# guanlongzhao/fac-via-ppg

Measured on AMD Instinct MI355X. Metric: 22.05 kHz audio samples/sec end-to-end PPG→wav; real-time factor at batch=1, higher is better.
Workload: dtype f32

## Files before the change

### fac-via-ppg_amd/common/stft.py

```python
import numpy as np
import torch
from scipy.signal import get_window

from common.audio_processing import _center_pad, squared_window
from facppg import lib as _lib


def dft_bases(filter_length, hop_length, win_length, window):
    n = filter_length
    cutoff = n // 2 + 1
    ang = 2.0 * np.pi * np.outer(np.arange(cutoff), np.arange(n)) / n
    fwd = np.vstack([np.cos(ang), -np.sin(ang)])
    wc = np.full(cutoff, 2.0)
    wc[0] = 1.0
    if n % 2 == 0:
        wc[-1] = 1.0
    scale = n / hop_length
    inv = np.vstack([np.cos(ang) * wc[:, None], -np.sin(ang) * wc[:, None]]) / (n * scale)
    fwd32, inv32 = fwd.astype(np.float32), inv.astype(np.float32)
    if window is not None:
        assert filter_length >= win_length
        win = _center_pad(get_window(window, win_length, fftbins=True), n).astype(np.float32)
        fwd32, inv32 = fwd32 * win, inv32 * win
    return fwd32, inv32


class STFT(torch.nn.Module):

    def __init__(self, filter_length=800, hop_length=200, win_length=800, window='hann', mel_basis=None):
        super(STFT, self).__init__()
        self.filter_length = filter_length
        self.hop_length = hop_length
        self.win_length = win_length
        self.window = window
        self.forward_transform = None
        fwd, inv = dft_bases(filter_length, hop_length, win_length, window)
        self.register_buffer('forward_basis', torch.from_numpy(fwd[:, None, :]).float())
        self.register_buffer('inverse_basis', torch.from_numpy(inv[:, None, :]).float())
        wsq = squared_window(window, win_length, filter_length) if window is not None else \
            np.zeros(filter_length)
        self.register_buffer('_win_sq', torch.from_numpy(wsq.astype(np.float32)), persistent=False)
        self._mel_basis_np = mel_basis

    def _handle(self, dev):
        h = self.__dict__.get("_facppg_handle")
        if h is not None and h[1] == dev:
            return h[0]
        self._release()
        L = _lib.load()
        fwd = self.forward_basis.squeeze(1).to(dev).contiguous()
        inv_t = self.inverse_basis.squeeze(1).t().to(dev).contiguous()
        wsq = self._win_sq.to(dev).contiguous()
        mel = None if self._mel_basis_np is None else torch.as_tensor(self._mel_basis_np, dtype=torch.float32).to(dev).contiguous()
        out = _lib.ctypes.c_void_p()
        with torch.cuda.device(dev):
            _lib.check(L.facppg_stft_create(self.filter_length, self.hop_length, _lib.ptr(fwd), _lib.ptr(inv_t), _lib.ptr(wsq),
                                            _lib.ptr(mel), 0 if mel is None else mel.shape[0], dev.index,
                                            _lib.current_stream(dev), _lib.ctypes.byref(out)))
        self.__dict__["_facppg_handle"] = (out, dev)
        return out

    def _release(self):
        h = self.__dict__.pop("_facppg_handle", None)
        if h is not None:
            _lib.load().facppg_stft_destroy(h[0])
        self.__dict__.pop("_facppg_ws", None)

    def __del__(self):
        try:
            self._release()
        except Exception:
            pass

    def __getstate__(self):
        d = dict(self.__dict__)
        d.pop("_facppg_handle", None)
        d.pop("_facppg_ws", None)
        return d

    def _workspace(self, h, dev, B, N):
        nbytes = _lib.load().facppg_stft_workspace_bytes(h, B, N)
        ws = self.__dict__.get("_facppg_ws")
        if ws is None or ws.numel() < nbytes or ws.device != dev:
            ws = torch.empty(nbytes, dtype=torch.uint8, device=dev)
            self.__dict__["_facppg_ws"] = ws
        return ws

    @staticmethod
    def _lengths(lengths, B, N, dev):
        if lengths is None:
            return None
        if torch.is_tensor(lengths):
            lt = lengths.to(device=dev, dtype=torch.int32).contiguous()
            if lt.numel() != B or int(lt.max()) > N:
                raise _lib.FacppgError("lengths must be B sample counts <= N")
            return lt
        if len(lengths) != B or max(int(n) for n in lengths) > N:
            raise _lib.FacppgError("lengths must be B sample counts <= N")
        return _lib.upload([int(n) for n in lengths], torch.int32, dev)

    def transform(self, input_data, lengths=None):
        _lib.require_cuda(input_data, "STFT.transform: input_data")
        x = input_data.float().contiguous()
        B, N = x.shape
        self.num_samples = N
        dev = x.device
        h = self._handle(dev)
        ws = self._workspace(h, dev, B, N)
        F = N // self.hop_length + 1
        cutoff = self.filter_length // 2 + 1
        mag = torch.zeros(B, cutoff, F, device=dev) if lengths is not None else torch.empty(B, cutoff, F, device=dev)
        phase = torch.zeros_like(mag) if lengths is not None else torch.empty_like(mag)
        with torch.cuda.device(dev):
            _lib.check(_lib.load().facppg_stft_transform(h, _lib.ptr(x), _lib.ptr(self._lengths(lengths, B, N, dev)), B, N,
                                                         _lib.ptr(mag), _lib.ptr(phase), _lib.ptr(ws), ws.numel(),
                                                         _lib.current_stream(dev)))
        return mag, phase

    def inverse(self, magnitude, phase):
        _lib.require_cuda(magnitude, "STFT.inverse: magnitude")
        mag = magnitude.float().contiguous()
        ph = phase.to(mag.device).float().contiguous()
        B, _, F = mag.shape
        dev = mag.device
        h = self._handle(dev)
        ws = self._workspace(h, dev, B, (F - 1) * self.hop_length)
        out = torch.empty(B, 1, self.hop_length * (F - 1), device=dev)
        with torch.cuda.device(dev):
            _lib.check(_lib.load().facppg_stft_inverse(h, _lib.ptr(mag), _lib.ptr(ph), B, F, _lib.ptr(out), _lib.ptr(ws),
                                                       ws.numel(), _lib.current_stream(dev)))
        return out

    def forward(self, input_data):
        self.magnitude, self.phase = self.transform(input_data)
        return self.inverse(self.magnitude, self.phase)

    def mel(self, y, lengths=None):
        _lib.require_cuda(y, "mel_spectrogram: y")
# ... 29 lines not shown
```

### fac-via-ppg_amd/csrc/facppg_dsp.hip

```cpp
#include <cstring>
#include <new>

#include "facppg_gemm.h"

using namespace facppg;

struct facppg_stft {
  int fl, hop, cutoff, n_mel, device;
  char* arena;
  float4 *fwd, *inv_t, *melb;
  float* win_sq;
};

namespace {

__global__ void k_frames(const float* __restrict__ x, float* __restrict__ X, const int* __restrict__ n_valid, int N, int fl,
                         int hop, int F, int* __restrict__ f_valid) {
  const int b = blockIdx.z, k = blockIdx.y;
  const int Nb = n_valid ? n_valid[b] : N;
  const int Fb = Nb / hop + 1;
  if (f_valid && blockIdx.x == 0 && k == 0 && threadIdx.x == 0) f_valid[b] = Fb;
  const int f = blockIdx.x * blockDim.x + threadIdx.x;
  if (f >= Fb) return;
  int j = f * hop + k - fl / 2;
// ... 12 lines not shown
  if (phase) phase[o] = atan2f(im, re);
}

__global__ void k_recombine(const float* __restrict__ mag, const float* __restrict__ phase, float* __restrict__ R,
                            const int* __restrict__ f_valid, int cutoff, int F) {
  const int b = blockIdx.z, c = blockIdx.y, f = blockIdx.x * blockDim.x + threadIdx.x;
  if (f >= (f_valid ? f_valid[b] : F)) return;
  const size_t o = ((size_t)b * cutoff + c) * F + f;
  float sn, cs;
  sincosf(phase[o], &sn, &cs);
  R[((size_t)b * 2 * cutoff + c) * F + f] = mag[o] * cs;
  R[((size_t)b * 2 * cutoff + cutoff + c) * F + f] = mag[o] * sn;
}

__global__ void k_spectral_subtract(float* __restrict__ S, const float* __restrict__ bias, float strength,
                                    const int* __restrict__ f_valid, int cutoff, int F) {
  const int b = blockIdx.z, c = blockIdx.y, f = blockIdx.x * blockDim.x + threadIdx.x;
  if (f >= (f_valid ? f_valid[b] : F)) return;
  const size_t ore = ((size_t)b * 2 * cutoff + c) * F + f, oim = ore + (size_t)cutoff * F;
  const float re = S[ore], im = S[oim];
  const float mag = sqrtf(re * re + im * im);
  const float m2 = fmaxf(mag - bias[c] * strength, 0.0f);
  if (mag > 0.0f) {
    const float sc = m2 / mag;
    S[ore] = re * sc; S[oim] = im * sc;
  } else {
    S[ore] = m2; S[oim] = 0.0f;
  }
}

__global__ void k_overlap_add(const float* __restrict__ Zt, const float* __restrict__ win_sq, float* __restrict__ y,
                              const int* __restrict__ f_valid, int fl, int hop, int F, long y_bs) {
  const int b = blockIdx.y;
  const int Fb = f_valid ? f_valid[b] : F;
  const int i = blockIdx.x * blockDim.x + threadIdx.x;
  if (i >= hop * (Fb - 1)) return;
  const int n = i + fl / 2;
  int f_hi = n / hop;
  if (f_hi > Fb - 1) f_hi = Fb - 1;
  int f_lo = (n - fl + hop) / hop;
  if (f_lo < 0) f_lo = 0;
  float acc = 0.0f, ws = 0.0f;
  for (int f = f_lo; f <= f_hi; ++f) {
    const int k = n - f * hop;
    acc += Zt[((size_t)b * F + f) * fl + k];
    ws += win_sq[k];
  }
  if (ws > 1.17549435e-38f) acc /= ws;
  y[(size_t)b * y_bs + i] = acc * ((float)fl / (float)hop);
}

struct Ws {
  int F;
  size_t X, S, Z, fv, sk, sk_bytes, total;
};
Ws ws_layout(const facppg_stft* h, int B, int N) {
  Ws w;
  w.F = N / h->hop + 1;
  size_t off = 0;
  auto take = [&](size_t bytes) { size_t o = off; off += (bytes + 255) / 256 * 256; return o; };
  w.X = take((size_t)B * (h->fl + 2) * w.F * 4);
  w.S = take((size_t)B * (h->fl + 2) * w.F * 4);
  w.Z = take((size_t)B * w.F * h->fl * 4);
  w.fv = take((size_t)B * 4);
  w.sk_bytes = (size_t)4 * B * (h->fl + 2) * w.F * 4;
  w.sk = take(w.sk_bytes);
  w.total = off;
  return w;
}

int run_forward(facppg_stft* h, const float* audio, const int* n_valid, int B, int N, char* ws, const Ws& w, hipStream_t s) {
  float* X = (float*)(ws + w.X);
  float* S = (float*)(ws + w.S);
  int* fv = (int*)(ws + w.fv);
  dim3 g((w.F + 255) / 256, h->fl, B);
  k_frames<<<g, 256, 0, s>>>(audio, X, n_valid, N, h->fl, h->hop, w.F, fv);
  GemmArgs a;
  a.A = h->fwd; a.M = 2 * h->cutoff; a.Cin = h->fl; a.X = X; a.x_bs = (long)h->fl * w.F; a.ldx = w.F; a.N = w.F;
  a.n_valid = fv; a.C = S; a.c_bs = (long)2 * h->cutoff * w.F; a.ldc = w.F; a.B = B;
  a.splitk_ws = (float*)(ws + w.sk); a.splitk_ws_bytes = w.sk_bytes;
  return gemm_launch(a, s);
}

int run_inverse(facppg_stft* h, const float* R, int B, char* ws, const Ws& w, const int* fv, float* out, long out_bs, hipStream_t s) {
  float* Z = (float*)(ws + w.Z);
  GemmArgs a;
  a.A = h->inv_t; a.M = h->fl; a.Cin = 2 * h->cutoff; a.X = R; a.x_bs = (long)2 * h->cutoff * w.F; a.ldx = w.F; a.N = w.F;
  a.n_valid = fv; a.C = Z; a.c_bs = (long)w.F * h->fl; a.ldc = h->fl; a.c_transposed = 1; a.B = B;
  a.splitk_ws = (float*)(ws + w.sk); a.splitk_ws_bytes = w.sk_bytes;
  if (int rc = gemm_launch(a, s)) return rc;
  const int n_out = h->hop * (w.F - 1);
  if (n_out > 0) {
    dim3 g((n_out + 255) / 256, B);
    k_overlap_add<<<g, 256, 0, s>>>(Z, h->win_sq, out, fv, h->fl, h->hop, w.F, out_bs);
  }
  FACPPG_HIP_CHECK(hipGetLastError());
  return FACPPG_OK;
}

int check_common(const facppg_stft* h, const void* a, const void* b, const void* ws, int B, int N, size_t ws_bytes, Ws* w) {
  FACPPG_REQUIRE(h && a && b && ws, FACPPG_EINVAL, "NULL argument");
  FACPPG_REQUIRE(B > 0 && N > h->fl / 2, FACPPG_EINVAL, "need B > 0 and N > filter_length/2 (reflect padding), got B=%d N=%d", B, N);
  *w = ws_layout(h, B, N);
  FACPPG_REQUIRE(ws_bytes >= w->total, FACPPG_EWORKSPACE, "workspace has %zu bytes, need %zu", ws_bytes, w->total);
  return FACPPG_OK;
}

}

extern "C" int facppg_stft_create(int filter_length, int hop_length, const float* fwd_basis_dev, const float* inv_basis_t_dev,
                                  const float* win_sq_dev, const float* mel_basis_dev, int n_mel, int device, void* stream_,
                                  facppg_stft** out) {
  FACPPG_REQUIRE(fwd_basis_dev && inv_basis_t_dev && win_sq_dev && out, FACPPG_EINVAL, "NULL argument");
  FACPPG_REQUIRE(filter_length >= 16 && filter_length % 2 == 0 && hop_length > 0 && hop_length <= filter_length, FACPPG_EINVAL,
                 "bad filter_length/hop_length %d/%d", filter_length, hop_length);
  FACPPG_REQUIRE(!mel_basis_dev || n_mel > 0, FACPPG_EINVAL, "n_mel must be positive with a mel basis");
  hipStream_t s = (hipStream_t)stream_;
  FACPPG_HIP_CHECK(hipSetDevice(device));
  facppg_stft* h = new (std::nothrow) facppg_stft();
  FACPPG_REQUIRE(h, FACPPG_EINVAL, "out of host memory");
  h->fl = filter_length; h->hop = hop_length; h->cutoff = filter_length / 2 + 1; h->n_mel = mel_basis_dev ? n_mel : 0;
  h->device = device;
  const int R = 2 * h->cutoff;
  size_t off = 0;
  auto take = [&](size_t bytes) { size_t o = off; off += (bytes + 255) / 256 * 256; return o; };
  const size_t o_fwd = take(packed_a_float4s(R, h->fl) * 16), o_inv = take(packed_a_float4s(h->fl, R) * 16);
  const size_t o_mel = take(h->n_mel ? packed_a_float4s(h->n_mel, h->cutoff) * 16 : 16), o_win = take((size_t)h->fl * 4);
  if (hipMalloc((void**)&h->arena, off) != hipSuccess) {
    set_error("hipMalloc(%zu) failed", off);
    delete h;
    return FACPPG_EHIP;
  }
  h->fwd = (float4*)(h->arena + o_fwd); h->inv_t = (float4*)(h->arena + o_inv); h->melb = (float4*)(h->arena + o_mel);
  h->win_sq = (float*)(h->arena + o_win);
  int rc = pack_a(fwd_basis_dev, R, h->fl, 1, h->fwd, s);
  if (!rc) rc = pack_a(inv_basis_t_dev, h->fl, R, 1, h->inv_t, s);
  if (!rc && h->n_mel) rc = pack_a(mel_basis_dev, h->n_mel, h->cutoff, 1, h->melb, s);
  if (!rc && hipMemcpyAsync(h->win_sq, win_sq_dev, (size_t)h->fl * 4, hipMemcpyDeviceToDevice, s) != hipSuccess) rc = FACPPG_EHIP;
  if (!rc && hipStreamSynchronize(s) != hipSuccess) rc = FACPPG_EHIP;
  if (rc) {
    (void)hipFree(h->arena);
    delete h;
    return rc;
  }
  *out = h;
  return FACPPG_OK;
}

extern "C" void facppg_stft_destroy(facppg_stft* h) {
  if (!h) return;
  (void)hipFree(h->arena);
  delete h;
}

extern "C" size_t facppg_stft_workspace_bytes(const facppg_stft* h, int B, int N) {
  if (!h || B <= 0 || N <= 0) return 0;
  return ws_layout(h, B, N).total;
}

extern "C" int facppg_stft_transform(facppg_stft* h, const float* audio_dev, const int32_t* n_valid_dev, int B, int N,
                                     float* mag_dev, float* phase_dev, void* ws_, size_t ws_bytes, void* stream_) {
  Ws w;
  if (int rc = check_common(h, audio_dev, mag_dev, ws_, B, N, ws_bytes, &w)) return rc;
  hipStream_t s = (hipStream_t)stream_;
  char* ws = (char*)ws_;
  if (int rc = run_forward(h, audio_dev, n_valid_dev, B, N, ws, w, s)) return rc;
  dim3 g((w.F + 255) / 256, h->cutoff, B);
  k_magphase<<<g, 256, 0, s>>>((float*)(ws + w.S), mag_dev, phase_dev, (int*)(ws + w.fv), h->cutoff, w.F);
  FACPPG_HIP_CHECK(hipGetLastError());
  return FACPPG_OK;
}

extern "C" int facppg_stft_inverse(facppg_stft* h, const float* mag_dev, const float* phase_dev, int B, int F, float* out_dev,
                                   void* ws_, size_t ws_bytes, void* stream_) {
  FACPPG_REQUIRE(h && mag_dev && phase_dev && out_dev && ws_, FACPPG_EINVAL, "NULL argument");
  FACPPG_REQUIRE(B > 0 && F > 1, FACPPG_EINVAL, "need B > 0 and at least 2 frames");
  const int N = (F - 1) * h->hop;
  const Ws w = ws_layout(h, B, N);
  FACPPG_REQUIRE(ws_bytes >= w.total, FACPPG_EWORKSPACE, "workspace has %zu bytes, need %zu", ws_bytes, w.total);
  hipStream_t s = (hipStream_t)stream_;
  char* ws = (char*)ws_;
  float* R = (float*)(ws + w.X);
  dim3 g((F + 255) / 256, h->cutoff, B);
  k_recombine<<<g, 256, 0, s>>>(mag_dev, phase_dev, R, nullptr, h->cutoff, F);
  return run_inverse(h, R, B, ws, w, nullptr, out_dev, (long)h->hop * (F - 1), s);
}

extern "C" int facppg_stft_mel(facppg_stft* h, const float* audio_dev, const int32_t* n_valid_dev, int B, int N, float* mel_dev,
                               void* ws_, size_t ws_bytes, void* stream_) {
  Ws w;
  if (int rc = check_common(h, audio_dev, mel_dev, ws_, B, N, ws_bytes, &w)) return rc;
  FACPPG_REQUIRE(h->n_mel > 0, FACPPG_EINVAL, "handle was created without a mel basis");
  hipStream_t s = (hipStream_t)stream_;
  char* ws = (char*)ws_;
  if (int rc = run_forward(h, audio_dev, n_valid_dev, B, N, ws, w, s)) return rc;
  float* mag = (float*)(ws + w.X);
  int* fv = (int*)(ws + w.fv);
  dim3 g((w.F + 255) / 256, h->cutoff, B);
  k_magphase<<<g, 256, 0, s>>>((float*)(ws + w.S), mag, nullptr, fv, h->cutoff, w.F);
  GemmArgs a;
  a.A = h->melb; a.M = h->n_mel; a.Cin = h->cutoff; a.X = mag; a.x_bs = (long)h->cutoff * w.F; a.ldx = w.F; a.N = w.F;
  a.n_valid = fv; a.act = ACT_LOG_CLAMP; a.C = mel_dev; a.c_bs = (long)h->n_mel * w.F; a.ldc = w.F; a.B = B;
  return gemm_launch(a, s);
}

extern "C" int facppg_denoise(facppg_stft* h, const float* audio_dev, const int32_t* n_valid_dev, const float* bias_spec_dev,
                              float strength, int B, int N, float* out_dev, void* ws_, size_t ws_bytes, void* stream_) {
  Ws w;
  if (int rc = check_common(h, audio_dev, out_dev, ws_, B, N, ws_bytes, &w)) return rc;
  FACPPG_REQUIRE(bias_spec_dev, FACPPG_EINVAL, "bias_spec is NULL");
  hipStream_t s = (hipStream_t)stream_;
  char* ws = (char*)ws_;
  if (int rc = run_forward(h, audio_dev, n_valid_dev, B, N, ws, w, s)) return rc;
  float* S = (float*)(ws + w.S);
  int* fv = (int*)(ws + w.fv);
  dim3 g((w.F + 255) / 256, h->cutoff, B);
  k_spectral_subtract<<<g, 256, 0, s>>>(S, bias_spec_dev, strength, fv, h->cutoff, w.F);
  return run_inverse(h, S, B, ws, w, fv, out_dev, (long)h->hop * (w.F - 1), s);
}
```

### fac-via-ppg_amd/csrc/facppg_gemm.h

```cpp
#pragma once
#include "facppg_common.h"

namespace facppg {

enum GemmAct { ACT_NONE = 0, ACT_RELU = 1, ACT_TANH = 2, ACT_LOG_CLAMP = 3  };

inline int gemm_kpad(int K) { return round_up(K, 64); }
inline size_t packed_a_float4s(int M, int K) { return (size_t)(round_up(M, 32) / 32) * (gemm_kpad(K) / 8 + 1) * 64 + 3 * 64; }

int pack_a(const float* src, int M, int Cin, int taps, float4* dst, hipStream_t s);
int pack_a_strided(const float* src, int M, int Cin, int taps, long sm, long sc, long st, long off, float4* dst, hipStream_t s);

struct GemmArgs {
  const float4* A = nullptr;
  int M = 0;
  int Cin = 0, taps = 1, dil = 1, pad = 0;
  const float* X = nullptr;
  long x_bs = 0;
  int ldx = 0;
  int N = 0;
  int col0 = 0;
  int src_hi = 0;
  const int* skip = nullptr;
  const int* n_valid = nullptr;
  int n_valid_mul = 1;
  int n_valid_add = 0;
  const float* bias = nullptr;
  const float* scale = nullptr;
  const float* shift = nullptr;
  int act = ACT_NONE;
  const uint8_t* mask = nullptr;
  long mask_bs = 0;
  int ldmask = 0;
  const float* res = nullptr;
  long res_bs = 0;
  int ldres = 0;
  float* C = nullptr;
  long c_bs = 0;
  int ldc = 0;
  int c_transposed = 0;
  const float* gate_ts = nullptr;
  long gate_bs = 0;
  int ldgate = 0;
  int B = 1;
  float* splitk_ws = nullptr;
  size_t splitk_ws_bytes = 0;
};

int gemm_launch(const GemmArgs& a, hipStream_t s);

}
```

### fac-via-ppg_amd/csrc/facppg_gemm.hip

```cpp
#include "facppg_gemm.h"

namespace facppg {
namespace {

constexpr int TN = 64, KCH = 64;

__global__ void k_pack_a(const float* __restrict__ src, float4* __restrict__ dst, int M, int Cin, int taps, int KG, long sm,
                         long sc, long st, long off) {
  const int idx = blockIdx.x * blockDim.x + threadIdx.x;
  const int MB = (M + 31) / 32;
  if (idx >= MB * (KG + 1) * 64) return;
  const int lane = idx & 63, g = (idx >> 6) % (KG + 1), mb = (idx >> 6) / (KG + 1);
  const int m = mb * 32 + (lane & 31), K = Cin * taps;
  float v[4];
  for (int s = 0; s < 4; ++s) {
    const int k = 8 * g + 4 * (lane >> 5) + s;
    const int tap = k / Cin, c = k - tap * Cin;
    v[s] = (m < M && k < K && g < KG) ? src[off + m * sm + c * sc + tap * st] : 0.0f;
  }
  dst[idx] = make_float4(v[0], v[1], v[2], v[3]);
}

struct KArgs {
  GemmArgs g;
  int KG;
  int sk;
};

__device__ __forceinline__ void gemm_epilogue(const GemmArgs& p, int b, int m, int n, float v) {
  if (p.bias) v += p.bias[m];
  if (p.scale) v = v * p.scale[m] + p.shift[m];
  if (p.act == ACT_RELU) v = fmaxf(v, 0.0f);
  else if (p.act == ACT_TANH) v = tanhf(v);
  else if (p.act == ACT_LOG_CLAMP) v = logf(fmaxf(v, 1e-5f));
  if (p.mask) v = v * (float)p.mask[(size_t)b * p.mask_bs + (size_t)m * p.ldmask + n] * 2.0f;
  if (p.res) v += p.res[(size_t)b * p.res_bs + (size_t)m * p.ldres + n];
  if (p.gate_ts) {
    const float T = p.gate_ts[(size_t)b * p.gate_bs + (size_t)m * p.ldgate + n];
    const float S = p.gate_ts[(size_t)b * p.gate_bs + (size_t)(p.M + m) * p.ldgate + n];
    p.C[(size_t)b * p.c_bs + (size_t)m * p.ldc + n] = v * S * (1.0f - T * T);
    p.C[(size_t)b * p.c_bs + (size_t)(p.M + m) * p.ldc + n] = v * T * S * (1.0f - S);
  } else if (p.c_transposed) p.C[(size_t)b * p.c_bs + (size_t)n * p.ldc + m] = v;
  else p.C[(size_t)b * p.c_bs + (size_t)m * p.ldc + n] = v;
}

__global__ __launch_bounds__(256) void k_gemm(KArgs ka) {
  const GemmArgs& p = ka.g;
  __shared__ __attribute__((aligned(16))) float smem[2 * KCH * TN];
  const int tid = threadIdx.x, lane = tid & 63, w = tid >> 6, li = lane & 31, kh = lane >> 5;
  const int b = blockIdx.z / ka.sk, ks = blockIdx.z % ka.sk, n0 = p.col0 + blockIdx.x * TN;
  const int Nb = p.n_valid ? min(p.N, p.n_valid[b] * p.n_valid_mul + p.n_valid_add) : p.N;
  if (n0 >= Nb) return;
  if (p.skip && *p.skip) return;
// ... 4 lines not shown
  const int K = p.Cin * p.taps;
  const int nch_all = ka.KG / 8;
  const int c_lo = ks * nch_all / ka.sk, c_hi = (ks + 1) * nch_all / ka.sk;

  f32x16 acc[2];
#pragma unroll
  for (int r = 0; r < 16; ++r) { acc[0][r] = 0.0f; acc[1][r] = 0.0f; }

  const float* xb = p.X + (size_t)b * p.x_bs;
  const int col = n0 + lane;
  float stg[16];
  auto stage_load = [&](int c) {
#pragma unroll
    for (int j = 0; j < 16; ++j) {
      const int kk = c * KCH + w * 16 + j;
      const int tap = kk / p.Cin, ch = kk - tap * p.Cin;
      const int sc = col + (tap - p.pad) * p.dil;
      stg[j] = (kk < K && sc >= 0 && sc < Ns) ? xb[(size_t)ch * p.ldx + sc] : 0.0f;
    }
  };
  auto stage_write = [&](int buf) {
    float* dst = smem + buf * (KCH * TN) + (w * 16) * TN + lane;
#pragma unroll
    for (int j = 0; j < 16; ++j) dst[j * TN] = stg[j];
  };

  const float4* ap = p.A + (size_t)(active ? mb : 0) * (ka.KG + 1) * 64 + lane;
  constexpr int RING = 4;
  float4 ar[RING];
  stage_load(c_lo);
#pragma unroll
  for (int i = 0; i < RING - 1; ++i) ar[i] = ap[(size_t)(c_lo * 8 + i) * 64];
  stage_write(c_lo & 1);
  __syncthreads();
  for (int c = c_lo; c < c_hi; ++c) {
    stage_load(c + 1 < c_hi ? c + 1 : c);
    const float* lb = smem + (c & 1) * (KCH * TN) + (4 * kh) * TN + li;
    const int G = c * 8;
#pragma unroll
    for (int g = 0; g < 8; ++g) {
      ar[(g + RING - 1) % RING] = ap[(size_t)(G + g + RING - 1) * 64];
      __builtin_amdgcn_sched_barrier(0);
      const float4 a0 = ar[g % RING];
#pragma unroll
      for (int s = 0; s < 4; ++s) {
        const float av = s == 0 ? a0.x : s == 1 ? a0.y : s == 2 ? a0.z : a0.w;
        acc[0] = mfma32x32x2(av, lb[(8 * g + s) * TN], acc[0]);
        acc[1] = mfma32x32x2(av, lb[(8 * g + s) * TN + 32], acc[1]);
      }
    }
    stage_write((c + 1) & 1);
    __syncthreads();
  }
  if (!active) return;
#pragma unroll
  for (int cb = 0; cb < 2; ++cb) {
    const int n = n0 + cb * 32 + li;
    if (n >= Nb) continue;
#pragma unroll
    for (int r = 0; r < 16; ++r) {
      const int m = mb * 32 + 8 * (r >> 2) + (r & 3) + 4 * kh;
      if (m >= p.M) continue;
      if (ka.sk > 1) p.splitk_ws[(((size_t)ks * p.B + b) * p.M + m) * p.N + n] = acc[cb][r];
      else gemm_epilogue(p, b, m, n, acc[cb][r]);
    }
  }
}

__global__ void k_gemm_reduce(KArgs ka) {
  const GemmArgs& p = ka.g;
  const int n = p.col0 + blockIdx.x * blockDim.x + threadIdx.x, m = blockIdx.y, b = blockIdx.z;
  const int Nb = p.n_valid ? min(p.N, p.n_valid[b] * p.n_valid_mul + p.n_valid_add) : p.N;
  if (n >= Nb) return;
  if (p.skip && *p.skip) return;
  float v = 0.0f;
  for (int ks = 0; ks < ka.sk; ++ks) v += p.splitk_ws[(((size_t)ks * p.B + b) * p.M + m) * p.N + n];
  gemm_epilogue(p, b, m, n, v);
}

}

int pack_a_strided(const float* src, int M, int Cin, int taps, long sm, long sc, long st, long off, float4* dst, hipStream_t s) {
  const int KG = gemm_kpad(Cin * taps) / 8;
  const int total = (round_up(M, 32) / 32) * (KG + 1) * 64;
  k_pack_a<<<(total + 255) / 256, 256, 0, s>>>(src, dst, M, Cin, taps, KG, sm, sc, st, off);
  FACPPG_HIP_CHECK(hipGetLastError());
  return FACPPG_OK;
}

int pack_a(const float* src, int M, int Cin, int taps, float4* dst, hipStream_t s) {
  return pack_a_strided(src, M, Cin, taps, (long)Cin * taps, taps, 1, 0, dst, s);
}

int gemm_launch(const GemmArgs& a, hipStream_t s) {
  FACPPG_REQUIRE(a.A && a.X && a.C && a.M > 0 && a.N > 0 && a.Cin > 0 && a.taps > 0 && a.B > 0 && a.col0 >= 0 && a.col0 < a.N, FACPPG_EINVAL,
                 "gemm_launch: bad arguments");
  KArgs ka;
  ka.g = a;
  ka.KG = gemm_kpad(a.Cin * a.taps) / 8;
  ka.sk = 1;
  dim3 grid((a.N - a.col0 + TN - 1) / TN, (round_up(a.M, 32) / 32 + 3) / 4, a.B);
  const int nch = ka.KG / 8;
  if (a.splitk_ws && nch >= 8) {
    const int sk = nch / 4 < 16 ? nch / 4 : 16;
    const size_t need = (size_t)sk * a.B * a.M * a.N * sizeof(float);
    FACPPG_REQUIRE(need <= a.splitk_ws_bytes, FACPPG_EWORKSPACE, "gemm_launch: split-K buffer has %zu bytes, needs %zu",
                   a.splitk_ws_bytes, need);
    ka.sk = sk;
  }
  grid.z = a.B * ka.sk;
  k_gemm<<<grid, 256, 0, s>>>(ka);
  if (ka.sk > 1) k_gemm_reduce<<<dim3((a.N - a.col0 + 255) / 256, a.M, a.B), 256, 0, s>>>(ka);
  FACPPG_HIP_CHECK(hipGetLastError());
  return FACPPG_OK;
}

}
```

### fac-via-ppg_amd/csrc/facppg_taco.hip

```cpp

#include <algorithm>
#include <cstdlib>
#include <cstring>
#include <mutex>
#include <new>

#include "facppg_gemm.h"

using namespace facppg;

struct facppg_taco {
  facppg_taco_config c;
  int device;
  int coop_limit;
  int wall_khz;
  char* arena;
  float4 *pre0, *pre1, *conv[8], *wih;
  float *conv_b[8], *conv_scale[8], *conv_shift[8];
  float *whh_t[2], *lstm_b;
  float4* mem_w;
  float *dp0_t, *dp1_t, *att_t, *att_b, *dec_t, *dec_b, *q_t, *proj_t, *proj_b;
  float *loc_conv, *loc_dense, *v;
  float *att_coop[5], *dec_coop[5];
  int coop_U[5], coop_nwg[5];
// ... 1332 lines not shown
      forced_att_slice<NTC>(att_slice, xrow, p.E + p.A, p.U, p.A, unit0, L.in_att + p.P, L.part, c_state, out, (unsigned)(tf + 1), tid);
    }
    __syncthreads();
  };
  att_step(0);
  long long tk = clock64();
#define PROF(slot)                                                        \
  if (p.prof && leader && b == 0 && tid == 0) {                           \
    const long long now = clock64();                                      \
    p.prof[slot] += now - tk;                                             \
    tk = now;                                                             \
  }
  for (int t = 0; t < T; ++t) {
    unsigned long long* xt = xb + (size_t)t * fw;
    int lo, hi;
    attn_window_range(p.window, t, len, &lo, &hi);
    attn_features<NTC>(p, L, lo, min(64, hi - lo + 1), tid);
    __syncthreads();
    attn_energy_pre<NTC>(p, L, pm, lo, min(64, hi - lo + 1), tid, stash);
    PROF(0)
    coop_gather<NTC>(xt, (unsigned)(t + 1), p.A, ah, L.in_dec, tid);
    PROF(1)
    dec_attention<NTC, 0, true>(p, L, mem, pm, len, t, b, tid, leader, true, NoQueryRegs().w, stash);
    if (leader)
      for (int i = tid; i < p.E; i += NTC) xpub(xt + p.A + i, L.in_proj[p.D + i], (unsigned)(t + 1));
    PROF(2)
    if (t + 1 < T) att_step(t + 1);
    PROF(3)
  }
#undef PROF
}

__global__ void k_forced_inputs(const float* __restrict__ tgt, float* __restrict__ x, size_t rows, int T) {
  const size_t i = (size_t)blockIdx.x * blockDim.x + threadIdx.x;
  if (i >= rows * T) return;
  const int t = (int)(i % T);
  x[i] = t ? tgt[i - 1] : 0.0f;
}
__global__ void k_forced_outputs(const float* __restrict__ mg, float* __restrict__ mel, float* __restrict__ gate, int B, int NF, int T) {
  const size_t i = (size_t)blockIdx.x * blockDim.x + threadIdx.x;
  if (i >= (size_t)B * (NF + 1) * T) return;
  const int t = (int)(i % T), r = (int)(i / T % (NF + 1)), b = (int)(i / T / (NF + 1));
  if (r < NF) mel[((size_t)b * NF + r) * T + t] = mg[i];
  else gate[(size_t)b * T + t] = mg[i];
}
__global__ void k_random_mask_forced_utt(uint8_t* __restrict__ out, const uint64_t* __restrict__ seeds, int B, int P, int T) {
  const size_t i = (size_t)blockIdx.x * blockDim.x + threadIdx.x;
  if (i >= (size_t)2 * B * P * T) return;
  const int t = (int)(i % T), u = (int)(i / T % P), b = (int)(i / T / P % B), j = (int)(i / T / P / B);
  out[i] = mask_bit(seeds[b] ^ 0xD1B54A32D192ED03ull, ((uint64_t)t << 32) | (uint32_t)(j * P + u));
}

struct TWs {
  size_t a0, a1, xproj, mem_cm, mask, xchg, splitk, splitk_bytes, total;
};
TWs tws_layout(const facppg_taco_config& c, int B, int Tin) {
  TWs w;
  size_t off = 0;
  auto take = [&](size_t bytes) { size_t o = off; off += (bytes + 255) / 256 * 256; return o; };
  const size_t E = c.encoder_embedding_dim > c.symbols_embedding_dim ? c.encoder_embedding_dim : c.symbols_embedding_dim;
  w.a0 = take((size_t)B * E * Tin * 4);
  w.a1 = take((size_t)B * E * Tin * 4);
  w.xproj = take((size_t)B * Tin * 4 * c.encoder_embedding_dim * 4);
  w.mem_cm = take((size_t)B * c.encoder_embedding_dim * Tin * 4);
  w.mask = take((size_t)2 * B * c.symbols_embedding_dim * Tin);
  w.xchg = take((size_t)B * 2 * 2 * (c.encoder_embedding_dim / 2) * 8);
  const size_t mx = c.encoder_embedding_dim > c.symbols_embedding_dim ? c.encoder_embedding_dim : c.symbols_embedding_dim;
  w.splitk_bytes = (size_t)16 * B * mx * Tin * 4;
  w.splitk = take(w.splitk_bytes);
  w.total = off;
  return w;
}

}

static int taco_check(const facppg_taco_config* c) {
  FACPPG_REQUIRE(c, FACPPG_EINVAL, "config is NULL");
  FACPPG_REQUIRE(c->n_symbols > 0 && c->symbols_embedding_dim > 0 && c->encoder_embedding_dim > 0 && c->encoder_embedding_dim % 2 == 0,
                 FACPPG_EINVAL, "bad encoder dims");
  FACPPG_REQUIRE(c->symbols_embedding_dim == c->encoder_embedding_dim, FACPPG_EUNSUPPORTED,
                 "symbols_embedding_dim must equal encoder_embedding_dim (prenet feeds the conv bank)");
  FACPPG_REQUIRE(c->encoder_n_convolutions >= 0 && c->encoder_n_convolutions <= 8 && c->postnet_n_convolutions >= 2 &&
                     c->postnet_n_convolutions <= 8 && c->encoder_kernel_size % 2 == 1 && c->postnet_kernel_size % 2 == 1,
                 FACPPG_EUNSUPPORTED, "conv stack sizes out of range");
  FACPPG_REQUIRE(c->attention_rnn_dim == c->decoder_rnn_dim && c->attention_rnn_dim % 4 == 0 && 4 * c->attention_rnn_dim <= 4096,
                 FACPPG_EUNSUPPORTED, "attention_rnn_dim must equal decoder_rnn_dim, be a multiple of 4 and <= 1024");
  FACPPG_REQUIRE(c->attention_location_n_filters >= 1 && c->attention_location_n_filters <= 32 && c->attention_dim >= 1 &&
                     c->attention_dim <= 256,
                 FACPPG_EUNSUPPORTED, "attention_location_n_filters must be <= 32 and attention_dim <= 256 (one MFMA pass each)");
  FACPPG_REQUIRE(c->encoder_embedding_dim <= 768 && c->prenet_dim <= NTC && c->attention_dim <= NTC && c->n_acoustic_feat_dims < NTC &&
                     (2 * c->encoder_embedding_dim) % 4 == 0,
                 FACPPG_EUNSUPPORTED, "decoder dims exceed the 512-thread cooperative workgroup");
  FACPPG_REQUIRE(c->attention_location_kernel_size % 2 == 1 && c->attention_location_n_filters > 0, FACPPG_EUNSUPPORTED,
                 "attention_location_kernel_size must be odd");
  return FACPPG_OK;
}

static size_t taco_count(const facppg_taco_config* c) {
  const size_t S = c->symbols_embedding_dim, E = c->encoder_embedding_dim, H = E / 2, K = c->encoder_kernel_size;
  const size_t P = c->prenet_dim, A = c->attention_rnn_dim, D = c->decoder_rnn_dim, AD = c->attention_dim, NF = c->n_acoustic_feat_dims;
  size_t n = S * c->n_symbols + S * S;
  n += (size_t)c->encoder_n_convolutions * (E * E * K + 5 * E);
  n += 2 * (4 * H * E + 4 * H * H + 8 * H);
  n += P * NF + P * P;
  n += 4 * A * (P + E) + 4 * A * A + 8 * A;
  n += AD * A + AD * E + AD + (size_t)c->attention_location_n_filters * 2 * c->attention_location_kernel_size +
       AD * c->attention_location_n_filters;
  n += 4 * D * (A + E) + 4 * D * D + 8 * D;
  n += NF * (D + E) + NF + (D + E) + 1;
  const size_t PE = c->postnet_embedding_dim, PK = c->postnet_kernel_size;
  for (int j = 0; j < c->postnet_n_convolutions; ++j) {
    const size_t ci = j == 0 ? NF : PE, co = j == c->postnet_n_convolutions - 1 ? NF : PE;
    n += co * ci * PK + 5 * co;
  }
  return n;
}

extern "C" size_t facppg_taco_weight_count(const facppg_taco_config* c) {
  if (taco_check(c) != FACPPG_OK) return 0;
// ... 182 lines not shown
    const int n = (D + E + 1) * Pp;
    k_fold_prenet<<<(n + 255) / 256, 256, 0, s>>>(h->proj_t, h->proj_b, h->dp0_t, h->w1p_t, h->b1p, D + E, NF, NFp, Pp);
    if (!rc) rc = pack_a_strided(h->proj_t, NF + 1, D + E, 1, 1, NFp, 0, 0, h->tf_proj, s);
  }
  for (int j = 0; j < c.postnet_n_convolutions; ++j) {
    const int ci = j == 0 ? NF : PE, co = j == c.postnet_n_convolutions - 1 ? NF : PE;
    h->post[j] = F4(o.post[j]); h->post_b[j] = F(o.post_b[j]); h->post_scale[j] = F(o.post_sc[j]); h->post_shift[j] = F(o.post_sh[j]);
    if (!rc) rc = pack_a(src, co, ci, PK, h->post[j], s); src += (size_t)co * ci * PK;
    cpy(h->post_b[j], src, co); src += co;
    bn(src, co, h->post_scale[j], h->post_shift[j]);
  }
  hipok(hipGetLastError());
  hipok(hipStreamSynchronize(s));
  if (!rc && (size_t)(src - wsrc) != n_floats) { set_error("internal: consumed %zu of %zu weights", (size_t)(src - wsrc), n_floats); rc = FACPPG_EINVAL; }
  if (rc) return rc;
  guard.h = nullptr;
  *out = h;
  return FACPPG_OK;
}

extern "C" void facppg_taco_destroy(facppg_taco* h) {
  if (!h) return;
  (void)hipFree(h->arena);
  delete h;
}

extern "C" size_t facppg_taco_workspace_bytes(const facppg_taco* h, int B, int Tin) {
  if (!h || B <= 0 || Tin <= 0) return 0;
  return tws_layout(h->c, B, Tin).total;
}

static int taco_encode_impl(const facppg_taco* h, const float* ppg_dev, const int32_t* lengths_dev, const uint8_t* masks_dev,
                            uint64_t seed, int B, int Tin, float* memory_dev, float* pm_dev, void* ws_, size_t ws_bytes,
                            void* stream_, bool padded_batch) {
  FACPPG_REQUIRE(h && ppg_dev && memory_dev && pm_dev && ws_, FACPPG_EINVAL, "NULL argument");
  FACPPG_REQUIRE(B > 0 && Tin > 0 && B <= 65535, FACPPG_EINVAL, "bad B/Tin");
  const facppg_taco_config& c = h->c;
  const TWs w = tws_layout(c, B, Tin);
  FACPPG_REQUIRE(ws_bytes >= w.total, FACPPG_EWORKSPACE, "workspace has %zu bytes, need %zu", ws_bytes, w.total);
  hipStream_t s = (hipStream_t)stream_;
  char* ws = (char*)ws_;
  float* a0 = (float*)(ws + w.a0);
  float* a1 = (float*)(ws + w.a1);
  float* xproj = (float*)(ws + w.xproj);
  float* mem_cm = (float*)(ws + w.mem_cm);
  const int S = c.symbols_embedding_dim, E = c.encoder_embedding_dim, H = E / 2;
  const uint8_t* masks = masks_dev;
  if (!masks) {
    uint8_t* m = (uint8_t*)(ws + w.mask);
    const size_t n = (size_t)2 * B * S * Tin;
    k_random_mask<<<(unsigned)((n + 255) / 256), 256, 0, s>>>(m, n, seed);
    masks = m;
  }
  GemmArgs g;
  g.B = B; g.N = Tin; g.n_valid = padded_batch ? nullptr : lengths_dev;
  g.splitk_ws = (float*)(ws + w.splitk); g.splitk_ws_bytes = w.splitk_bytes;
  g.A = h->pre0; g.M = S; g.Cin = c.n_symbols; g.X = ppg_dev; g.x_bs = (long)c.n_symbols * Tin; g.ldx = Tin; g.act = ACT_RELU;
  g.mask = masks; g.mask_bs = (long)S * Tin; g.ldmask = Tin; g.C = a0; g.c_bs = (long)S * Tin; g.ldc = Tin;
  if (int rc = gemm_launch(g, s)) return rc;
  g.A = h->pre1; g.Cin = S; g.X = a0; g.x_bs = (long)S * Tin; g.mask = masks + (size_t)B * S * Tin; g.C = a1;
  if (int rc = gemm_launch(g, s)) return rc;
  float* cur = a1;
  float* nxt = a0;
  g.mask = nullptr;
  for (int j = 0; j < c.encoder_n_convolutions; ++j) {
    g.A = h->conv[j]; g.M = E; g.Cin = E; g.taps = c.encoder_kernel_size; g.pad = (c.encoder_kernel_size - 1) / 2; g.X = cur;
    g.x_bs = (long)E * Tin; g.bias = h->conv_b[j]; g.scale = h->conv_scale[j]; g.shift = h->conv_shift[j]; g.C = nxt;
    g.c_bs = (long)E * Tin;
    if (int rc = gemm_launch(g, s)) return rc;
    float* t = cur; cur = nxt; nxt = t;
  }
  GemmArgs p;
  p.splitk_ws = g.splitk_ws; p.splitk_ws_bytes = g.splitk_ws_bytes;
  p.B = B; p.N = Tin; p.n_valid = lengths_dev; p.A = h->wih; p.M = 8 * H; p.Cin = E; p.X = cur; p.x_bs = (long)E * Tin; p.ldx = Tin;
  p.bias = h->lstm_b; p.C = xproj; p.c_bs = (long)Tin * 8 * H; p.ldc = 8 * H; p.c_transposed = 1;
  if (int rc = gemm_launch(p, s)) return rc;
  const char* bilstm_mode = getenv("FACPPG_BILSTM_MODE");
  const bool no_coop = bilstm_mode && !strcmp(bilstm_mode, "single");
  const bool fit32 = (long)B * 2 * ((H + 31) / 32) <= h->coop_limit && (H + 3) / 4 <= 96 && !(bilstm_mode && !strcmp(bilstm_mode, "wide"));
  const bool fit64 = (long)B * 2 * ((H + 63) / 64) <= h->coop_limit && (H + 1) / 2 <= 152;
  if (!no_coop && (fit32 || fit64)) {
    unsigned long long* xchg = (unsigned long long*)(ws + w.xchg);
    FACPPG_HIP_CHECK(hipMemsetAsync(xchg, 0, (size_t)B * 2 * 2 * H * 8, s));
    const float *w0 = h->whh_t[0], *w1 = h->whh_t[1];
    const float* xp = xproj;
    int Tin_ = Tin, H_ = H;
    void* args[] = {(void*)&xp, (void*)&w0, (void*)&w1, (void*)&lengths_dev, (void*)&Tin_, (void*)&H_, (void*)&xchg,
                    (void*)&memory_dev, (void*)&mem_cm};
    if (fit32) FACPPG_HIP_CHECK(launch_coop((const void*)k_bilstm_coop<32, 96>, dim3((H + 31) / 32, 2, B), dim3(NTC), args, 0, s));
    else FACPPG_HIP_CHECK(launch_coop((const void*)k_bilstm_coop<64, 152>, dim3((H + 63) / 64, 2, B), dim3(NTC), args, 0, s));
  } else {
    const int KS = NT / H < H ? NT / H : H;
    const size_t smem = (size_t)(2 * H + (KS > 0 ? KS : 1) * 4 * H) * 4;
    k_bilstm<<<dim3(2, B), NT, smem, s>>>(xproj, h->whh_t[0], h->whh_t[1], lengths_dev, Tin, H, memory_dev, mem_cm);
  }
  GemmArgs m;
  m.splitk_ws = g.splitk_ws; m.splitk_ws_bytes = g.splitk_ws_bytes;
  m.B = B; m.N = Tin; m.n_valid = lengths_dev; m.A = h->mem_w; m.M = c.attention_dim; m.Cin = E; m.X = mem_cm; m.x_bs = (long)E * Tin;
  m.ldx = Tin; m.C = pm_dev; m.c_bs = (long)Tin * c.attention_dim; m.ldc = Tin;
  if (int rc = gemm_launch(m, s)) return rc;
  FACPPG_HIP_CHECK(hipGetLastError());
  return FACPPG_OK;
}

extern "C" int facppg_taco_encode(const facppg_taco* h, const float* ppg_dev, const int32_t* lengths_dev, const uint8_t* masks_dev,
                                  uint64_t seed, int B, int Tin, float* memory_dev, float* pm_dev, void* ws_, size_t ws_bytes,
                                  void* stream_) {
  return taco_encode_impl(h, ppg_dev, lengths_dev, masks_dev, seed, B, Tin, memory_dev, pm_dev, ws_, ws_bytes, stream_, false);
}

extern "C" int facppg_taco_encode_padded(const facppg_taco* h, const float* ppg_dev, const int32_t* lengths_dev,
                                         const int32_t* lengths_host, const uint8_t* masks_dev, uint64_t seed, int B, int Tin,
                                         float* memory_dev, float* pm_dev, void* ws_, size_t ws_bytes, void* stream_) {
  FACPPG_REQUIRE(h && memory_dev && pm_dev, FACPPG_EINVAL, "NULL argument");
  FACPPG_REQUIRE(B > 0 && Tin > 0, FACPPG_EINVAL, "bad B/Tin");
  FACPPG_REQUIRE((lengths_dev == nullptr) == (lengths_host == nullptr), FACPPG_EINVAL, "lengths_dev and lengths_host go together");
  for (int b = 0; lengths_host && b < B; ++b) {
    FACPPG_REQUIRE(lengths_host[b] >= 1 && lengths_host[b] <= Tin, FACPPG_EINVAL, "lengths[%d] = %d is outside [1, Tin = %d]", b,
                   lengths_host[b], Tin);
    FACPPG_REQUIRE(b == 0 || lengths_host[b] <= lengths_host[b - 1], FACPPG_EINVAL,
                   "lengths must be sorted in descending order (pack_padded_sequence, model.py:226): lengths[%d] = %d > lengths[%d] = %d",
                   b, lengths_host[b], b - 1, lengths_host[b - 1]);
  }
  hipStream_t s = (hipStream_t)stream_;
  FACPPG_HIP_CHECK(hipMemsetAsync(memory_dev, 0, (size_t)B * Tin * h->c.encoder_embedding_dim * 4, s));
  FACPPG_HIP_CHECK(hipMemsetAsync(pm_dev, 0, (size_t)B * Tin * h->c.attention_dim * 4, s));
  return taco_encode_impl(h, ppg_dev, lengths_dev, masks_dev, seed, B, Tin, memory_dev, pm_dev, ws_, ws_bytes, stream_, true);
}

namespace {
struct DecWs { size_t mask, xchg, prof, xsplit, total; };
DecWs dec_ws(const facppg_taco_config& c, int B, int max_steps) {
  DecWs w;
  size_t off = 0;
  auto take = [&](size_t bytes) { size_t o = off; off += (bytes + 255) / 256 * 256; return o; };
  w.mask = take((size_t)max_steps * 2 * B * c.prenet_dim);
  w.xchg = take((size_t)B * 2 * c.attention_rnn_dim * 8);
  w.prof = take(32 * 8);
  w.xsplit = take((size_t)B * (c.n_acoustic_feat_dims + 1 + 2 * c.prenet_dim + c.attention_rnn_dim + c.encoder_embedding_dim + c.decoder_rnn_dim + 8) * 8);
  w.total = off;
  return w;
}
}

extern "C" int facppg_taco_draw_dropout(const facppg_taco* h, const uint64_t* seeds_dev, int B, int Tin, int max_steps,
                                        uint8_t* enc_masks_dev, uint8_t* dec_masks_dev, void* stream_) {
  FACPPG_REQUIRE(h && seeds_dev, FACPPG_EINVAL, "NULL argument");
  FACPPG_REQUIRE(B > 0 && Tin > 0 && max_steps > 0, FACPPG_EINVAL, "bad B/Tin/max_steps");
  hipStream_t s = (hipStream_t)stream_;
  const int S = h->c.symbols_embedding_dim, P = h->c.prenet_dim;
  if (enc_masks_dev) {
    const size_t n = (size_t)2 * B * S * Tin;
// ... 98 lines not shown
                   : NU == 3 ? (const void*)k_decoder_split<3> : (const void*)k_decoder_split<4>;
    FACPPG_HIP_CHECK(hipFuncSetAttribute(fn, hipFuncAttributeMaxDynamicSharedMemorySize, (int)ssm));
    void* args[] = {(void*)&a};
    const int groups = (B + NU - 1) / NU;
    a.nwk = h->split_nwk;
    unsigned long long* words = opts ? (unsigned long long*)opts->frame_words_dev : nullptr;
    a.melx = (B == 1 && words && opts->frame_words_frames >= max_steps) ? words : nullptr;
    a.dbg_flags = getenv("FACPPG_DECODER_NO_ROWS") ? 1 : 0;
    FACPPG_HIP_CHECK(launch_coop(fn, dim3(h->split_nwk + NU, groups), dim3(NTC), args, ssm, s));
    launch_mode = 2; launch_wgs = (h->split_nwk + NU) * groups;
    if (a.prof) {
      long long pr[32];
      FACPPG_HIP_CHECK(hipMemcpyAsync(pr, a.prof, sizeof(pr), hipMemcpyDeviceToHost, s));
      FACPPG_HIP_CHECK(hipStreamSynchronize(s));
      fprintf(stderr, "[facppg split decoder prof (main), shader cycles] location features %lld energy_pre %lld entering row %lld query weights requested %lld wait_gate %lld wait_ah %lld attention %lld | att: query %lld energy %lld softmax %lld update %lld context %lld\n",
              pr[6], pr[7], pr[14], pr[2], pr[0], pr[3], pr[5], pr[8], pr[10], pr[11], pr[12], pr[13]);
      fprintf(stderr, "[facppg split decoder prof (worker 0), shader cycles] proj+prenet1 %lld | gather gate,X1 %lld | prenet2 %lld | gather X2 %lld | "
              "att LSTM %lld | gather AH %lld | gather CTX %lld | dec LSTM + gather DH %lld | barrier %lld\n",
              pr[16], pr[17], pr[18], pr[19], pr[20], pr[21], pr[22], pr[23], pr[24]);
    }
  } else
  if (coop) {
    FACPPG_HIP_CHECK(hipMemsetAsync(ws + w.xchg, 0, w.total - w.xchg, s));
    const void* fn = (const void*)k_decoder_coop;
    FACPPG_HIP_CHECK(hipFuncSetAttribute(fn, hipFuncAttributeMaxDynamicSharedMemorySize, (int)smem));
    for (int b0 = 0; b0 < B; b0 += chunk) {
      const int nb = B - b0 < chunk ? B - b0 : chunk;
      int cv = variant;
      if (!force_u)
        for (int v = 0; v < variant; ++v)
          if ((long)nb * h->coop_nwg[v] <= wg_limit) { cv = v; break; }
      a.b0 = b0; a.att_coop = h->att_coop[cv]; a.dec_coop = h->dec_coop[cv]; a.U = h->coop_U[cv];
      void* args[] = {(void*)&a};
      FACPPG_HIP_CHECK(launch_coop(fn, dim3(h->coop_nwg[cv], nb), dim3(NTC), args, smem, s));
      launch_mode = 1; launch_wgs = h->coop_nwg[cv] * nb;
    }
    if (a.prof) {
      long long pr[16];
      FACPPG_HIP_CHECK(hipMemcpyAsync(pr, a.prof, sizeof(pr), hipMemcpyDeviceToHost, s));
      FACPPG_HIP_CHECK(hipStreamSynchronize(s));
      fprintf(stderr, "[facppg decoder prof, shader cycles] project %lld prenet %lld att_slice %lld sync1 %lld gather %lld attention %lld dec_slice %lld sync2 %lld | att: query %lld feat %lld energy %lld softmax %lld update %lld context %lld\n",
              pr[0], pr[1], pr[2], pr[3], pr[4], pr[5], pr[6], pr[7], pr[8], pr[9], pr[10], pr[11], pr[12], pr[13]);
    }
  } else {
    FACPPG_HIP_CHECK(hipFuncSetAttribute((const void*)k_decoder, hipFuncAttributeMaxDynamicSharedMemorySize, (int)smem));
    k_decoder<<<B, NT, smem, s>>>(a);
  }
  FACPPG_HIP_CHECK(hipGetLastError());
  if (opts) { opts->mode = launch_mode; opts->workgroups = launch_wgs; opts->streamed = a.melx != nullptr; }
  return FACPPG_OK;
}

namespace {
struct ForcedWs { size_t x0, p1, p2, xa, hc, mg, mask, xchg, prof, splitk, splitk_bytes, total; };
ForcedWs forced_ws(const facppg_taco_config& c, int B, int T) {
  ForcedWs w;
  size_t off = 0;
  auto take = [&](size_t bytes) { size_t o = off; off += (bytes + 255) / 256 * 256; return o; };
  const size_t BT = (size_t)B * T;
  w.x0 = take(BT * c.n_acoustic_feat_dims * 4);
  w.p1 = take(BT * c.prenet_dim * 4);
  w.p2 = take(BT * c.prenet_dim * 4);
  w.xa = take(BT * 4 * c.attention_rnn_dim * 4);
  w.hc = take(BT * (c.decoder_rnn_dim + c.encoder_embedding_dim) * 4);
  w.mg = take(BT * (c.n_acoustic_feat_dims + 1) * 4);
  w.mask = take(2 * BT * c.prenet_dim);
  w.xchg = take(BT * (c.attention_rnn_dim + c.encoder_embedding_dim + c.decoder_rnn_dim) * 8);
  w.prof = take(32 * 8);
  w.splitk_bytes = 16 * BT * (c.n_acoustic_feat_dims + 1) * 4;
  w.splitk = take(w.splitk_bytes);
  w.total = off;
  return w;
}
}

extern "C" size_t facppg_taco_decode_forced_workspace_bytes(const facppg_taco* h, int B, int T_out) {
  if (!h || B <= 0 || T_out <= 0) return 0;
  return forced_ws(h->c, B, T_out).total;
}

extern "C" int facppg_taco_draw_dropout_forced(const facppg_taco* h, const uint64_t* seeds_dev, int B, int T_out,
                                               uint8_t* dec_masks_dev, void* stream_) {
  FACPPG_REQUIRE(h && seeds_dev && dec_masks_dev, FACPPG_EINVAL, "NULL argument");
  FACPPG_REQUIRE(B > 0 && T_out > 0, FACPPG_EINVAL, "bad B/T_out");
  const size_t n = (size_t)2 * B * h->c.prenet_dim * T_out;
  k_random_mask_forced_utt<<<(unsigned)((n + 255) / 256), 256, 0, (hipStream_t)stream_>>>(dec_masks_dev, seeds_dev, B, h->c.prenet_dim, T_out);
  FACPPG_HIP_CHECK(hipGetLastError());
  return FACPPG_OK;
}

extern "C" int facppg_taco_decode_forced(const facppg_taco* h, const float* memory_dev, const float* pm_dev, const int32_t* lengths_dev,
                                         const float* targets_dev, const uint8_t* masks_dev, uint64_t seed, int B, int Tin, int T_out,
                                         float* mel_dev, float* gate_dev, float* align_dev, void* ws_, size_t ws_bytes,
                                         facppg_taco_decode_opts* opts, void* stream_) {
  FACPPG_REQUIRE(h && memory_dev && pm_dev && targets_dev && mel_dev && gate_dev && ws_, FACPPG_EINVAL, "NULL argument");
  FACPPG_REQUIRE(B > 0 && Tin > 0 && T_out > 0 && B <= 65535, FACPPG_EINVAL, "bad B/Tin/T_out");
  FACPPG_REQUIRE(!opts || opts->max_workgroups >= 0, FACPPG_EINVAL, "negative max_workgroups");
  FACPPG_REQUIRE(Tin <= 8192, FACPPG_EUNSUPPORTED, "Tin > 8192 does not fit the decoder's LDS state");
  const facppg_taco_config& c = h->c;
  hipStream_t s = (hipStream_t)stream_;
  const ForcedWs w = forced_ws(c, B, T_out);
  FACPPG_REQUIRE(ws_bytes >= w.total, FACPPG_EWORKSPACE, "teacher-forced decode workspace has %zu bytes, need %zu", ws_bytes, w.total);
  char* ws = (char*)ws_;
  const int P = c.prenet_dim, E = c.encoder_embedding_dim, A = c.attention_rnn_dim, D = c.decoder_rnn_dim, NF = c.n_acoustic_feat_dims;
  const int T = T_out, G = 4 * A, KP = D + E;
  float *x0 = (float*)(ws + w.x0), *p1 = (float*)(ws + w.p1), *p2 = (float*)(ws + w.p2), *xa = (float*)(ws + w.xa);
  float *hc = (float*)(ws + w.hc), *mg = (float*)(ws + w.mg);
  const uint8_t* masks = masks_dev;
  const size_t nmask = (size_t)2 * B * P * T;
  if (!masks) {
    k_random_mask<<<(unsigned)((nmask + 255) / 256), 256, 0, s>>>((uint8_t*)(ws + w.mask), nmask, seed ^ 0xD1B54A32D192ED03ull);
    masks = (const uint8_t*)(ws + w.mask);
  }
  {
    const size_t n = (size_t)B * NF * T;
    k_forced_inputs<<<(unsigned)((n + 255) / 256), 256, 0, s>>>(targets_dev, x0, (size_t)B * NF, T);
  }
  GemmArgs g;
  g.B = B; g.N = T; g.A = h->tf_dp0; g.M = P; g.Cin = NF; g.X = x0; g.x_bs = (long)NF * T; g.ldx = T; g.act = ACT_RELU;
  g.mask = masks; g.mask_bs = (long)P * T; g.ldmask = T; g.C = p1; g.c_bs = (long)P * T; g.ldc = T;
  if (int rc = gemm_launch(g, s)) return rc;
  g.A = h->tf_dp1; g.Cin = P; g.X = p1; g.x_bs = (long)P * T; g.mask = masks + (size_t)B * P * T; g.C = p2;
  if (int rc = gemm_launch(g, s)) return rc;
  GemmArgs x;
  x.B = B; x.N = T; x.A = h->tf_attx; x.M = G; x.Cin = P; x.X = p2; x.x_bs = (long)P * T; x.ldx = T; x.bias = h->att_b;
  x.C = xa; x.c_bs = (long)T * G; x.ldc = G; x.c_transposed = 1;
  if (int rc = gemm_launch(x, s)) return rc;
  DecArgs a = {};
  a.dec_b = h->dec_b; a.q_t = h->q_t; a.loc_conv = h->loc_conv; a.loc_dense = h->loc_dense; a.v = h->v;
  a.memory = memory_dev; a.pm = pm_dev; a.lengths = lengths_dev; a.align = align_dev;
  a.B = B; a.Tin = Tin; a.E = E; a.P = P; a.A = A; a.D = D; a.AD = c.attention_dim; a.NF = NF;
  a.NFIL = c.attention_location_n_filters; a.KSZ = c.attention_location_kernel_size; a.window = c.attention_window_size;
  a.max_steps = T; a.gate_thr = c.gate_threshold;
  const size_t smem = (round_up((int)dec_lds_floats(a.P, a.E, a.A, a.D, a.NF, a.AD, a.NFIL, a.KSZ, Tin), 4) + (size_t)8 * NTC * 4) * 4;
  FACPPG_REQUIRE(smem <= 160 * 1024 - 1024, FACPPG_EUNSUPPORTED, "decoder state (%zu bytes) exceeds LDS", smem);
  const int max_wgs = opts ? opts->max_workgroups : 0;
  const int wg_limit = max_wgs > 0 && max_wgs < h->coop_limit ? max_wgs : h->coop_limit;
  FACPPG_REQUIRE(wg_limit >= 2 * h->coop_nwg[4], FACPPG_EUNSUPPORTED, "the teacher-forced decoder needs %d co-resident workgroups, %d allowed",
                 2 * h->coop_nwg[4], wg_limit);
  const char* force_u = getenv("FACPPG_DECODER_COOP_U");
  auto pick = [&](int nb, int* vc, int* vd) {
    for (int c2 = 0; c2 < 5; ++c2) {
      if (force_u && atoi(force_u) != h->coop_U[c2]) continue;
      for (int d2 = c2; d2 <= (force_u ? c2 : std::min(c2 + 1, 4)); ++d2)
        if ((long)nb * (h->coop_nwg[c2] + h->coop_nwg[d2]) <= wg_limit) { *vc = c2; *vd = d2; return true; }
    }
    return false;
  };
  const bool regw = !force_u && !getenv("FACPPG_FORCED_NO_REGW") && (long)B * (h->split_nwk + h->coop_nwg[0]) <= wg_limit &&
                    E + A <= SKP * SKR_FA && A <= h->split_nwk * SU;
  int vc = 4, vd = 4, chunk = B;
  if (regw) { vc = vd = 0; }
  else if (!pick(B, &vc, &vd)) {
    FACPPG_REQUIRE(!force_u, FACPPG_EUNSUPPORTED, "FACPPG_DECODER_COOP_U=%s does not fit B = %d", force_u, B);
    vc = vd = 4; chunk = wg_limit / (2 * h->coop_nwg[4]);
  }
  unsigned long long* xw = (unsigned long long*)(ws + w.xchg);
  FACPPG_HIP_CHECK(hipMemsetAsync(xw, 0, w.prof + 32 * 8 - w.xchg, s));
  a.prof = getenv("FACPPG_DECODER_PROF") ? (long long*)(ws + w.prof) : nullptr;
  const void* fn = regw ? (const void*)k_decoder_forced<true> : (const void*)k_decoder_forced<false>;
  FACPPG_HIP_CHECK(hipFuncSetAttribute(fn, hipFuncAttributeMaxDynamicSharedMemorySize, (int)smem));
  a.att_w4 = h->att_w4;
  int launch_wgs = 0;
  for (int b0 = 0; b0 < B; b0 += chunk) {
    const int nb = B - b0 < chunk ? B - b0 : chunk;
    int cv = vc, dv = vd;
    if (nb < chunk && !force_u && !regw) pick(nb, &cv, &dv);
    a.b0 = b0; a.att_coop = h->att_coop[cv]; a.dec_coop = h->dec_coop[dv]; a.U = h->coop_U[cv];
    const float* xa_c = xa;
    int NA = regw ? h->split_nwk : h->coop_nwg[cv], UD = h->coop_U[dv];
    void* args[] = {(void*)&a, (void*)&xa_c, (void*)&hc, (void*)&xw, (void*)&NA, (void*)&UD};
    FACPPG_HIP_CHECK(launch_coop(fn, dim3(NA + h->coop_nwg[dv], nb), dim3(NTC), args, smem, s));
    launch_wgs = (NA + h->coop_nwg[dv]) * nb;
  }
  if (a.prof) {
    long long pr[16];
    FACPPG_HIP_CHECK(hipMemcpyAsync(pr, a.prof, sizeof(pr), hipMemcpyDeviceToHost, s));
    FACPPG_HIP_CHECK(hipStreamSynchronize(s));
    fprintf(stderr, "[facppg teacher-forced decoder prof (chain workgroup 0), shader cycles] features+energy_pre %lld gather_ah %lld attention %lld att_slice %lld | att: query %lld feat %lld energy %lld softmax %lld update %lld context %lld\n",
            pr[0], pr[1], pr[2], pr[3], pr[8], pr[9], pr[10], pr[11], pr[12], pr[13]);
  }
  GemmArgs q;
  q.splitk_ws = (float*)(ws + w.splitk); q.splitk_ws_bytes = w.splitk_bytes;
  q.B = B; q.N = T; q.A = h->tf_proj; q.M = NF + 1; q.Cin = KP; q.X = hc; q.x_bs = (long)KP * T; q.ldx = T; q.bias = h->proj_b;
  q.C = mg; q.c_bs = (long)(NF + 1) * T; q.ldc = T;
  if (int rc = gemm_launch(q, s)) return rc;
  {
    const size_t n = (size_t)B * (NF + 1) * T;
    k_forced_outputs<<<(unsigned)((n + 255) / 256), 256, 0, s>>>(mg, mel_dev, gate_dev, B, NF, T);
  }
  FACPPG_HIP_CHECK(hipGetLastError());
  if (opts) { opts->mode = 1; opts->workgroups = launch_wgs; opts->streamed = 0; }
  return FACPPG_OK;
}

__global__ void k_forced_state(const unsigned long long* __restrict__ xw, float* __restrict__ ah, float* __restrict__ dh, size_t BT,
                               int A, int E, int D) {
  const size_t i = (size_t)blockIdx.x * blockDim.x + threadIdx.x;
  if (i >= BT * (A + D)) return;
  const size_t r = i / (A + D);
  const int k = (int)(i % (A + D));
  const float v = __uint_as_float((unsigned)xw[r * (A + E + D) + (k < A ? k : k + E)]);
  if (k < A) ah[r * A + k] = v;
  else dh[r * D + k - A] = v;
}

extern "C" int facppg_taco_decode_forced_state(const facppg_taco* h, const void* ws_, size_t ws_bytes, int B, int T_out, float* ah_dev,
                                               float* dh_dev, uint8_t* masks_dev, void* stream_) {
  FACPPG_REQUIRE(h && ws_ && ah_dev && dh_dev, FACPPG_EINVAL, "NULL argument");
  FACPPG_REQUIRE(B > 0 && T_out > 0, FACPPG_EINVAL, "bad B/T_out");
  const facppg_taco_config& c = h->c;
  const ForcedWs w = forced_ws(c, B, T_out);
  FACPPG_REQUIRE(ws_bytes >= w.total, FACPPG_EWORKSPACE, "teacher-forced decode workspace has %zu bytes, need %zu", ws_bytes, w.total);
  hipStream_t s = (hipStream_t)stream_;
  const char* ws = (const char*)ws_;
  const size_t BT = (size_t)B * T_out, n = BT * (c.attention_rnn_dim + c.decoder_rnn_dim);
  k_forced_state<<<(unsigned)((n + 255) / 256), 256, 0, s>>>((const unsigned long long*)(ws + w.xchg), ah_dev, dh_dev, BT,
                                                             c.attention_rnn_dim, c.encoder_embedding_dim, c.decoder_rnn_dim);
  FACPPG_HIP_CHECK(hipGetLastError());
  if (masks_dev) FACPPG_HIP_CHECK(hipMemcpyAsync(masks_dev, ws + w.mask, 2 * BT * c.prenet_dim, hipMemcpyDeviceToDevice, s));
  return FACPPG_OK;
}

extern "C" int facppg_taco_encode_state(const facppg_taco* h, const void* ws_, size_t ws_bytes, int B, int Tin, uint8_t* masks_dev,
                                        void* stream_) {
  FACPPG_REQUIRE(h && ws_ && masks_dev, FACPPG_EINVAL, "NULL argument");
  FACPPG_REQUIRE(B > 0 && Tin > 0, FACPPG_EINVAL, "bad B/Tin");
  const TWs w = tws_layout(h->c, B, Tin);
  FACPPG_REQUIRE(ws_bytes >= w.total, FACPPG_EWORKSPACE, "encoder workspace has %zu bytes, need %zu", ws_bytes, w.total);
  FACPPG_HIP_CHECK(hipMemcpyAsync(masks_dev, (const char*)ws_ + w.mask, (size_t)2 * B * h->c.symbols_embedding_dim * Tin,
                                  hipMemcpyDeviceToDevice, (hipStream_t)stream_));
  return FACPPG_OK;
}

extern "C" int facppg_taco_postnet(const facppg_taco* h, const float* mel_dev, const int32_t* out_lengths_dev, int B, int T, int ld,
                                   float* mel_post_dev, void* ws_, size_t ws_bytes, void* stream_) {
  FACPPG_REQUIRE(h && mel_dev && mel_post_dev && ws_, FACPPG_EINVAL, "NULL argument");
  FACPPG_REQUIRE(B > 0 && T > 0 && ld >= T, FACPPG_EINVAL, "bad B/T/ld");
  const facppg_taco_config& c = h->c;
  const int PE = c.postnet_embedding_dim, NF = c.n_acoustic_feat_dims, n = c.postnet_n_convolutions;
  const size_t need = facppg_taco_postnet_workspace_bytes(h, B, T);
  FACPPG_REQUIRE(ws_bytes >= need, FACPPG_EWORKSPACE, "workspace has %zu bytes, need %zu", ws_bytes, need);
  hipStream_t s = (hipStream_t)stream_;
  float* buf[2] = {(float*)ws_, (float*)ws_ + (size_t)B * PE * T};
  float* skws = (float*)ws_ + (size_t)2 * B * PE * T;
  const size_t skws_bytes = need - (size_t)2 * B * PE * T * 4;
  const float* cur = mel_dev;
  long cur_bs = (long)NF * ld;
  int cur_ld = ld;
  for (int j = 0; j < n; ++j) {
    const int ci = j == 0 ? NF : PE, co = j == n - 1 ? NF : PE;
    GemmArgs g;
    g.splitk_ws = skws; g.splitk_ws_bytes = skws_bytes;
    g.B = B; g.N = T; g.n_valid = out_lengths_dev; g.A = h->post[j]; g.M = co; g.Cin = ci; g.taps = c.postnet_kernel_size;
    g.pad = (c.postnet_kernel_size - 1) / 2; g.X = cur; g.x_bs = cur_bs; g.ldx = cur_ld; g.bias = h->post_b[j];
    g.scale = h->post_scale[j]; g.shift = h->post_shift[j];
    if (j < n - 1) {
      g.act = ACT_TANH; g.C = buf[j & 1]; g.c_bs = (long)PE * T; g.ldc = T;
    } else {
      g.res = mel_dev; g.res_bs = (long)NF * ld; g.ldres = ld; g.C = mel_post_dev; g.c_bs = (long)NF * ld; g.ldc = ld;
    }
    if (int rc = gemm_launch(g, s)) return rc;
    cur = g.C; cur_bs = g.c_bs; cur_ld = g.ldc;
  }
  return FACPPG_OK;
}

extern "C" size_t facppg_taco_postnet_workspace_bytes(const facppg_taco* h, int B, int T) {
  if (!h || B <= 0 || T <= 0) return 0;
  const size_t sk = (size_t)16 * B * h->c.postnet_embedding_dim * T * 4;
  return (size_t)2 * B * h->c.postnet_embedding_dim * T * 4 + sk;
}

namespace {
__global__ __launch_bounds__(256) void k_collect_frames(const unsigned long long* __restrict__ melx, const int* __restrict__ out_len,
                                                        int NF, int fa, int fb, float* __restrict__ dst, int ld, int* void_flag,
                                                        const int* prev_flag, unsigned long long limit) {
  if (prev_flag && __hip_atomic_load(prev_flag, __ATOMIC_RELAXED, __HIP_MEMORY_SCOPE_AGENT)) {
    if (void_flag) __hip_atomic_store(void_flag, 1, __ATOMIC_RELAXED, __HIP_MEMORY_SCOPE_AGENT);
    return;
  }
  const int n = (fb - fa) * NF;
  for (int i = blockIdx.x * blockDim.x + threadIdx.x; i < n; i += gridDim.x * blockDim.x) {
    const int f = fa + i / NF, row = i - (f - fa) * NF;
    const unsigned long long* w = melx + (size_t)f * NF + row;
    unsigned long long v, t0 = 0;
    unsigned spins = 0;
    for (;;) {
      v = __hip_atomic_load(w, __ATOMIC_RELAXED, __HIP_MEMORY_SCOPE_AGENT);
      if ((unsigned)(v >> 32) == (unsigned)(f + 1)) break;
      const int ol = __hip_atomic_load(out_len, __ATOMIC_RELAXED, __HIP_MEMORY_SCOPE_AGENT);
      if (ol > 0 && f >= ol) {
        if (void_flag) __hip_atomic_store(void_flag, 1, __ATOMIC_RELAXED, __HIP_MEMORY_SCOPE_AGENT);
        return;
      }
      __builtin_amdgcn_s_sleep(32);
      if ((++spins & 255u) == 0 && limit) {
        const unsigned long long now = wall_clock64();
        if (!t0) t0 = now;
        else if (now - t0 > limit) {
          if (void_flag) __hip_atomic_store(void_flag, 1, __ATOMIC_RELAXED, __HIP_MEMORY_SCOPE_AGENT);
          return;
        }
      }
    }
    dst[(size_t)row * ld + f] = __uint_as_float((unsigned)v);
  }
}
}

extern "C" int facppg_taco_collect_frames(const facppg_taco* h, const void* words_dev, const int32_t* out_length_dev, int frame_a,
                                          int frame_b, float* mel_dev, int ld, int32_t* void_flag_dev, const int32_t* prev_flag_dev,
                                          void* stream_) {
  FACPPG_REQUIRE(h && words_dev && out_length_dev && mel_dev, FACPPG_EINVAL, "NULL argument");
  FACPPG_REQUIRE(frame_a >= 0 && frame_b > frame_a && frame_b <= ld, FACPPG_EINVAL, "frames [%d, %d) with ld %d", frame_a, frame_b, ld);
  const int n = (frame_b - frame_a) * h->c.n_acoustic_feat_dims;
  const char* wait_env = getenv("FACPPG_STREAM_WAIT_MS");
  const double wait_ms = wait_env ? strtod(wait_env, nullptr) : 100.0;
  const unsigned long long limit = void_flag_dev && wait_ms > 0 && h->wall_khz > 0 ? (unsigned long long)(wait_ms * h->wall_khz) : 0ull;
  k_collect_frames<<<(n + 255) / 256 < 8 ? (n + 255) / 256 : 8, 256, 0, (hipStream_t)stream_>>>(
      (const unsigned long long*)words_dev, out_length_dev, h->c.n_acoustic_feat_dims, frame_a, frame_b, mel_dev, ld, void_flag_dev,
      prev_flag_dev, limit);
  FACPPG_HIP_CHECK(hipGetLastError());
  return FACPPG_OK;
}

extern "C" size_t facppg_taco_postnet_stream_workspace_bytes(const facppg_taco* h, int max_frames) {
  if (!h || max_frames <= 0) return 0;
  const size_t PE = h->c.postnet_embedding_dim, n = h->c.postnet_n_convolutions;
  return (n - 1) * PE * max_frames * 4 + (size_t)16 * PE * max_frames * 4;
}

extern "C" int facppg_taco_postnet_range(const facppg_taco* h, const float* mel_dev, int ld, int f_prev, int f_new, int final_T,
                                         float* mel_post_dev, int ld_post, void* ws_, size_t ws_bytes, int max_frames,
                                         const int32_t* skip_dev, void* stream_) {
  FACPPG_REQUIRE(h && mel_dev && mel_post_dev && ws_, FACPPG_EINVAL, "NULL argument");
  const facppg_taco_config& c = h->c;
  const int PE = c.postnet_embedding_dim, NF = c.n_acoustic_feat_dims, n = c.postnet_n_convolutions, pad = (c.postnet_kernel_size - 1) / 2;
  FACPPG_REQUIRE(f_prev >= 0 && f_new >= f_prev && f_new <= max_frames && max_frames <= ld && final_T <= max_frames, FACPPG_EINVAL,
                 "bad frame range [%d, %d) / final %d / max %d", f_prev, f_new, final_T, max_frames);
  FACPPG_REQUIRE(final_T == 0 || final_T == f_new, FACPPG_EINVAL, "a final call covers exactly the utterance's frames");
  const size_t need = facppg_taco_postnet_stream_workspace_bytes(h, max_frames);
  FACPPG_REQUIRE(ws_bytes >= need, FACPPG_EWORKSPACE, "workspace has %zu bytes, need %zu", ws_bytes, need);
  hipStream_t s = (hipStream_t)stream_;
  float* bufs = (float*)ws_;
  float* skws = bufs + (size_t)(n - 1) * PE * max_frames;
  const size_t skws_bytes = (size_t)16 * PE * max_frames * 4;
  int src_hi = f_new;
  for (int j = 0; j < n; ++j) {
    const int lag = pad * (j + 1);
    const int lo = f_prev - lag > 0 ? f_prev - lag : 0;
    const int hi = final_T > 0 ? final_T : f_new - lag;
    if (hi > lo) {
      const int ci = j == 0 ? NF : PE, co = j == n - 1 ? NF : PE;
      GemmArgs g;
      g.splitk_ws = skws; g.splitk_ws_bytes = skws_bytes;
      g.B = 1; g.N = hi; g.col0 = lo; g.src_hi = src_hi; g.skip = skip_dev;
      g.A = h->post[j]; g.M = co; g.Cin = ci; g.taps = c.postnet_kernel_size; g.pad = pad;
      g.X = j == 0 ? mel_dev : bufs + (size_t)(j - 1) * PE * max_frames; g.ldx = j == 0 ? ld : max_frames;
      g.bias = h->post_b[j]; g.scale = h->post_scale[j]; g.shift = h->post_shift[j];
      if (j < n - 1) { g.act = ACT_TANH; g.C = bufs + (size_t)j * PE * max_frames; g.ldc = max_frames; }
      else { g.res = mel_dev; g.ldres = ld; g.C = mel_post_dev; g.ldc = ld_post; }
      if (int rc = gemm_launch(g, s)) return rc;
    }
    src_hi = hi > 0 ? hi : 0;
    if (src_hi == 0) break;
  }
  return FACPPG_OK;
}

extern "C" size_t facppg_taco_decode_workspace_bytes(const facppg_taco* h, int B, int max_steps) {
  if (!h || B <= 0 || max_steps <= 0) return 0;
  return dec_ws(h->c, B, max_steps).total;
}
```

### fac-via-ppg_amd/csrc/facppg_tdnn.hip

```cpp
#include <cmath>
#include <new>
#include <vector>

#include "facppg_gemm.h"

using namespace facppg;

struct facppg_tdnn {
  int device = 0;
  int n_layers = 0, final_op = 0, in_dim = 0, out_dim = 0, left = 0, right = 0, max_dim = 0;
  std::vector<facppg_tdnn_layer> layers;
  std::vector<float4*> A;
  std::vector<float*> bias;
  float* arena = nullptr;
};

namespace {

__global__ void k_tdnn_input(const float* __restrict__ feats, float* __restrict__ x0, int T, int D, int L, int Tp) {
  const int j = blockIdx.x * blockDim.x + threadIdx.x, c = blockIdx.y;
  if (j >= Tp) return;
  const int t = min(max(j - L, 0), T - 1);
  x0[(size_t)c * Tp + j] = feats[(size_t)t * D + c];
}

__global__ void k_tdnn_renorm(float* __restrict__ x, int C, int Tp, float target_rms) {
  const int j = blockIdx.x * blockDim.x + threadIdx.x;
  if (j >= Tp) return;
  float ss = 0.0f;
  for (int c = 0; c < C; ++c) { const float v = x[(size_t)c * Tp + j]; ss = fmaf(v, v, ss); }
  const float floor_ = 1.3552527156068805e-20f;
  const float scale = 1.0f / sqrtf(fmaxf(ss / ((float)C * target_rms * target_rms), floor_));
  for (int c = 0; c < C; ++c) x[(size_t)c * Tp + j] *= scale;
}

__global__ void k_tdnn_output(const float* __restrict__ y, int M, int Tp, int T, int final_op, float* __restrict__ out) {
  const int t = blockIdx.x * blockDim.x + threadIdx.x;
  if (t >= T) return;
  float mx = -INFINITY, sum = 0.0f;
  if (final_op != 0) {
    for (int m = 0; m < M; ++m) mx = fmaxf(mx, y[(size_t)m * Tp + t]);
    for (int m = 0; m < M; ++m) sum += expf(y[(size_t)m * Tp + t] - mx);
  }
  const float lse = logf(sum);
  for (int m = 0; m < M; ++m) {
    const float v = y[(size_t)m * Tp + t];
    out[(size_t)t * M + m] = final_op == 0 ? v : final_op == 1 ? expf(v - mx) / sum : v - mx - lse;
  }
}

struct TdnnWs { size_t x[2], splitk, splitk_bytes, total; int Tp; };
TdnnWs tdnn_ws(const facppg_tdnn* h, int T) {
  TdnnWs w;
  w.Tp = h->left + T + h->right;
  size_t off = 0;
  auto take = [&](size_t bytes) { size_t o = off; off += (bytes + 255) / 256 * 256; return o; };
  w.x[0] = take((size_t)h->max_dim * w.Tp * 4);
  w.x[1] = take((size_t)h->max_dim * w.Tp * 4);
  w.splitk_bytes = (size_t)16 * h->max_dim * w.Tp * 4;
  w.splitk = take(w.splitk_bytes);
  w.total = off;
  return w;
}

}

extern "C" size_t facppg_tdnn_weight_count(const facppg_tdnn_layer* layers, int n_layers) {
  if (!layers || n_layers <= 0) return 0;
  size_t n = 0;
  for (int i = 0; i < n_layers; ++i) {
    const facppg_tdnn_layer& l = layers[i];
    if (l.out_dim <= 0 || l.in_dim <= 0 || l.taps <= 0 || l.dil <= 0) return 0;
    n += (size_t)l.out_dim * l.taps * l.in_dim + l.out_dim;
  }
  return n;
}

extern "C" int facppg_tdnn_create(const facppg_tdnn_layer* layers, int n_layers, int final_op, const float* weights_dev,
                                  size_t n_weights, int device, void* stream_, facppg_tdnn** out) {
  FACPPG_REQUIRE(layers && weights_dev && out && n_layers > 0, FACPPG_EINVAL, "NULL argument");
  FACPPG_REQUIRE(final_op >= 0 && final_op <= 2, FACPPG_EINVAL, "final_op must be 0 (none), 1 (softmax) or 2 (log-softmax)");
  FACPPG_REQUIRE(n_weights == facppg_tdnn_weight_count(layers, n_layers) && n_weights > 0, FACPPG_EINVAL,
                 "weight blob has %zu values, the layer table needs %zu", n_weights, facppg_tdnn_weight_count(layers, n_layers));
  hipStream_t s = (hipStream_t)stream_;
  facppg_tdnn* h = new (std::nothrow) facppg_tdnn;
  FACPPG_REQUIRE(h, FACPPG_EHIP, "out of host memory");
  h->device = device; h->n_layers = n_layers; h->final_op = final_op;
  h->layers.assign(layers, layers + n_layers);
  h->in_dim = layers[0].in_dim; h->out_dim = layers[n_layers - 1].out_dim; h->max_dim = h->in_dim;
  size_t a_f4 = 0, b_f = 0;
  for (int i = 0; i < n_layers; ++i) {
    const facppg_tdnn_layer& l = layers[i];
    if (i > 0 && l.in_dim != layers[i - 1].out_dim) {
      set_error("layer %d reads %d channels, layer %d writes %d", i, l.in_dim, i - 1, layers[i - 1].out_dim);
      delete h;
      return FACPPG_EINVAL;
    }
    h->left += l.first < 0 ? -l.first : 0;
    const int hi = l.first + (l.taps - 1) * l.dil;
    h->right += hi > 0 ? hi : 0;
    if (l.first > 0 || hi < 0) {
      set_error("layer %d: a splice that excludes the current frame's side (first %d, last %d) is not supported", i, l.first, hi);
      delete h;
      return FACPPG_EUNSUPPORTED;
    }
    h->max_dim = l.out_dim > h->max_dim ? l.out_dim : h->max_dim;
    a_f4 += packed_a_float4s(l.out_dim, l.in_dim * l.taps);
    b_f += (size_t)round_up(l.out_dim, 64);
  }
  if (hipMalloc(&h->arena, a_f4 * 16 + b_f * 4) != hipSuccess) {
    set_error("hipMalloc of %zu bytes of packed TDNN weights failed", a_f4 * 16 + b_f * 4);
// ... 6 lines not shown
  for (int i = 0; i < n_layers; ++i) {
    const facppg_tdnn_layer& l = layers[i];
    const int K = l.taps * l.in_dim;
    const int rc = pack_a_strided(src, l.out_dim, l.in_dim, l.taps, K, 1, l.in_dim, 0, ap, s);
    if (rc != FACPPG_OK || hipMemcpyAsync(bp, src + (size_t)l.out_dim * K, (size_t)l.out_dim * 4, hipMemcpyDeviceToDevice, s) != hipSuccess) {
      if (rc == FACPPG_OK) set_error("copy of the layer-%d bias failed", i);
      (void)hipFree(h->arena);
      delete h;
      return FACPPG_EHIP;
    }
    h->A.push_back(ap);
    h->bias.push_back(bp);
    ap += packed_a_float4s(l.out_dim, K);
    bp += round_up(l.out_dim, 64);
    src += (size_t)l.out_dim * K + l.out_dim;
  }
  if (hipStreamSynchronize(s) != hipSuccess) {
    set_error("packing the TDNN weights failed");
    (void)hipFree(h->arena);
    delete h;
    return FACPPG_EHIP;
  }
  *out = h;
  return FACPPG_OK;
}

extern "C" void facppg_tdnn_destroy(facppg_tdnn* h) {
  if (!h) return;
  if (h->arena) (void)hipFree(h->arena);
  delete h;
}

extern "C" int facppg_tdnn_context(const facppg_tdnn* h, int* left, int* right) {
  FACPPG_REQUIRE(h && left && right, FACPPG_EINVAL, "NULL argument");
  *left = h->left; *right = h->right;
  return FACPPG_OK;
}

extern "C" size_t facppg_tdnn_workspace_bytes(const facppg_tdnn* h, int T) {
  if (!h || T <= 0) return 0;
  return tdnn_ws(h, T).total;
}

extern "C" int facppg_tdnn_forward(facppg_tdnn* h, const float* feats_dev, int T, float* out_dev, void* ws_, size_t ws_bytes,
                                   void* stream_) {
  FACPPG_REQUIRE(h && feats_dev && out_dev && ws_, FACPPG_EINVAL, "NULL argument");
  FACPPG_REQUIRE(T > 0, FACPPG_EINVAL, "T must be positive (got %d)", T);
  const TdnnWs w = tdnn_ws(h, T);
  FACPPG_REQUIRE(ws_bytes >= w.total, FACPPG_EWORKSPACE, "workspace has %zu bytes, need %zu", ws_bytes, w.total);
  hipStream_t s = (hipStream_t)stream_;
  char* ws = (char*)ws_;
  float* x[2] = {(float*)(ws + w.x[0]), (float*)(ws + w.x[1])};
  const int Tp = w.Tp;
  k_tdnn_input<<<dim3((Tp + 255) / 256, h->in_dim), 256, 0, s>>>(feats_dev, x[0], T, h->in_dim, h->left, Tp);
  int cur = 0;
  for (int i = 0; i < h->n_layers; ++i) {
    const facppg_tdnn_layer& l = h->layers[i];
    GemmArgs g;
    g.A = h->A[i]; g.M = l.out_dim; g.Cin = l.in_dim; g.taps = l.taps; g.dil = l.dil; g.pad = 0;
    g.X = x[cur]; g.ldx = Tp; g.N = Tp; g.bias = h->bias[i]; g.act = l.relu ? ACT_RELU : ACT_NONE;
    g.C = x[cur ^ 1]; g.ldc = Tp; g.B = 1;
    g.splitk_ws = (float*)(ws + w.splitk); g.splitk_ws_bytes = w.splitk_bytes;
    const int rc = gemm_launch(g, s);
    if (rc != FACPPG_OK) return rc;
    cur ^= 1;
    if (l.renorm_target_rms > 0.0f) k_tdnn_renorm<<<(Tp + 255) / 256, 256, 0, s>>>(x[cur], l.out_dim, Tp, l.renorm_target_rms);
  }
  k_tdnn_output<<<(T + 63) / 64, 64, 0, s>>>(x[cur], h->out_dim, Tp, T, h->final_op, out_dev);
  FACPPG_HIP_CHECK(hipGetLastError());
  return FACPPG_OK;
}
```

### fac-via-ppg_amd/csrc/facppg_wg.hip

```cpp
#include <algorithm>
#include <cmath>
#include <cstdlib>
#include <cstring>
#include <new>
#include <type_traits>
#include <vector>

#include "facppg_gemm.h"
#include "facppg_wg_internal.h"

namespace facppg {

thread_local char g_err[512] = "";
void set_error(const char* fmt, ...) {
  va_list ap;
  va_start(ap, fmt);
  vsnprintf(g_err, sizeof(g_err), fmt, ap);
  va_end(ap);
}

namespace {

constexpr int TN = 64;
constexpr int HALO = 128;
// ... 171 lines not shown
}

__global__ void k_fold_first(const float* __restrict__ in_w,
                             const float* __restrict__ start_w,
                             const float* __restrict__ start_b,
                             float* __restrict__ F0, int hh) {
  const int idx = blockIdx.x * blockDim.x + threadIdx.x;
  if (idx >= 2 * C * 64) return;
  const int o = idx >> 6, kk = idx & 63, tap = kk >> 3, ch = kk & 7;
  double v = 0.0;
  if (tap < 3 && ch <= hh)
    for (int c = 0; c < C; ++c) v += (double)in_w[((size_t)o * C + c) * 3 + tap] * (double)(ch < hh ? start_w[c * hh + ch] : start_b[c]);
  F0[idx] = (float)v;
}

__global__ void k_copy_rows(const float* __restrict__ src, float* __restrict__ dst, int n) {
  const int i = blockIdx.x * blockDim.x + threadIdx.x;
  if (i < n) dst[i] = src[i];
}

__global__ __launch_bounds__(1024) void k_group_offsets(const int* __restrict__ t_valid, int B, int* __restrict__ off) {
  __shared__ int part[1024];
  const int t = threadIdx.x, per = (B + 1023) / 1024, b0 = t * per, b1 = min(B, b0 + per);
  int sum = 0;
  for (int b = b0; b < b1; ++b) sum += (t_valid[b] + 3) / 4;
  part[t] = sum;
  __syncthreads();
  for (int d = 1; d < 1024; d <<= 1) {
    const int v = t >= d ? part[t - d] : 0;
    __syncthreads();
    part[t] += v;
    __syncthreads();
  }
  int run = part[t] - sum;
  for (int b = b0; b < b1; ++b) { off[b] = run; run += (t_valid[b] + 3) / 4; }
  if (t == 1023) off[B] = part[1023];
}

__global__ void k_group_table(const int* __restrict__ t_valid, const int* __restrict__ off, int B, int4* __restrict__ table, int n) {
  const int g = blockIdx.x * blockDim.x + threadIdx.x;
  if (g >= n) return;
  int4 e = make_int4(0, 0, 0, 0);
  if (g < off[B]) {
    int lo = 0, hi = B - 1;
    while (lo < hi) {
      const int mid = (lo + hi + 1) >> 1;
      if (off[mid] <= g) lo = mid; else hi = mid - 1;
    }
    const int q = 4 * (g - off[lo]);
    e = make_int4(lo, q, t_valid[lo] - q, 0);
  }
  table[g] = e;
}

struct WnArgs {
  const float* h_in;
  float* h_out;
  const float* spect;
  float* skip;
  const float4* w1;
  const float* b1;
  const float4* w2;
  const float* b2;
  const int* t_valid;
  int T, hop8, Lp, Lr, dil, first;
  float* save_ts;
  const float* melp;
  const float4* wc;
  int P, Tr, Tqp, ntq, nt, nch, ngc, kc, xcd_map;
  int hop, ksize;
  int flat_cols;
  const int4* groups;
  const float* xa;
  const float* we;
  const float* endb;
  int nconv;
  const float4* seed;
  int seed_nt;
};

typedef float f4u __attribute__((ext_vector_type(4), aligned(4)));

template <int NRB>
__device__ __forceinline__ void load_a(float4 (&a)[4], const float4* __restrict__ p, int rb_stride, int g) {
#pragma unroll
  for (int rb = 0; rb < NRB; ++rb) a[rb] = p[rb * rb_stride + g * 64];
}

template <int NCB, bool K4 = false>
__device__ __forceinline__ void load_b(float (&bv)[4][NCB], const float* lb, int g) {
  if constexpr (K4) {
#pragma unroll
    for (int cb = 0; cb < NCB; ++cb) {
      const float4 v = *reinterpret_cast<const float4*>(lb + ((2 * g) * (32 * NCB) + 32 * cb) * 4);
      bv[0][cb] = v.x; bv[1][cb] = v.y; bv[2][cb] = v.z; bv[3][cb] = v.w;
    }
  } else {
#pragma unroll
    for (int s = 0; s < 4; ++s)
#pragma unroll
      for (int cb = 0; cb < NCB; ++cb) bv[s][cb] = lb[(8 * g + s) * (32 * NCB) + 32 * cb];
  }
}

__device__ __forceinline__ int k4_index(int k, int col, int tnt) { return ((k >> 2) * tnt + col) * 4 + (k & 3); }

template <int NRB, int NCB>
__device__ __forceinline__ void mfma_group(f32x16 (&acc)[4][NCB], const float4 (&a)[4], const float (&bv)[4][NCB]) {
#pragma unroll
  for (int s = 0; s < 4; ++s) {
#pragma unroll
    for (int rb = 0; rb < NRB; ++rb) {
      const float av = s == 0 ? a[rb].x : s == 1 ? a[rb].y : s == 2 ? a[rb].z : a[rb].w;
#pragma unroll
      for (int cb = 0; cb < NCB; ++cb) acc[rb][cb] = mfma32x32x2(av, bv[s][cb], acc[rb][cb]);
    }
  }
}

__device__ __forceinline__ int pm_chunks(const WnArgs& p, int ph) {
  const int nj = (p.ksize - 1 - 8 * ph) / p.hop + 1;
  return min(p.nch, p.nconv + (nj * NMEL + KCH - 1) / KCH);
}

template <bool LAST, int NCB, bool SAVE = false, bool PM = false, bool EF = false>
__global__ __launch_bounds__(256, 2) void k_wn_layer(WnArgs p) {
  static_assert(!EF || PM, "folded flow edges exist on the phase-major layout only");
  extern __shared__ __attribute__((aligned(16))) float smem[];
  constexpr int TNt = 32 * NCB;
  constexpr int RPL = 64 / TNt;
  constexpr int NSTG = 16 / RPL;
// ... 358 lines not shown
#pragma unroll
  for (int rb = 0; rb < NRB2; ++rb) {
    const bool is_res = !LAST && rb < 2;
    const int chb = w * 64 + (rb & 1) * 32 + 4 * kh;
#pragma unroll
    for (int cb = 0; cb < NCB; ++cb) {
      const int col = cb * 32 + li;
      if (col < nvalid) {
#pragma unroll
        for (int r = 0; r < 16; ++r) {
          const int ch = chb + 8 * (r >> 2) + (r & 3);
          if (is_res) {
            const size_t o = ((size_t)b * C + ch) * p.Lp + in_off + col;
            p.h_out[o] = acc[rb][cb][r];
          } else {
            const size_t o = ((size_t)b * C + ch) * p.Lr + sk_off + col;
            p.skip[o] = (p.first ? 0.0f : p.skip[o]) + acc[rb][cb][r];
          }
        }
      }
    }
  }
}

#ifdef FACPPG_WN8_PROF
__device__ unsigned long long g_wn8_prof[12];
#define WN8_STAMP_DECL long long wn8_t = clock64()
#define WN8_STAMP(i)                                                                           \
  do {                                                                                         \
    const long long now__ = clock64();                                                         \
    if (blockIdx.x == 0 && threadIdx.x == 0) { atomicAdd(&g_wn8_prof[i], (unsigned long long)(now__ - wn8_t)); if ((i) == 5) atomicAdd(&g_wn8_prof[6], 1ull); } \
    wn8_t = now__;                                                                             \
  } while (0)
#else
#define WN8_STAMP_DECL
#define WN8_STAMP(i)
#endif

typedef float f32x4s __attribute__((ext_vector_type(4)));
#define FACPPG_AS1 __attribute__((address_space(1)))
typedef float f32x4s __attribute__((ext_vector_type(4)));
__device__ __forceinline__ float4 gld(const float4* q) {
  const f32x4s v = *(const FACPPG_AS1 f32x4s*)q;
  return make_float4(v.x, v.y, v.z, v.w);
}
__device__ __forceinline__ f4u gld(const f4u* q) { return *(const FACPPG_AS1 f4u*)q; }
__device__ __forceinline__ float gld(const float* q) { return *(const FACPPG_AS1 float*)q; }
__device__ __forceinline__ void store_f4(float* g, const float4 v) {
  const f32x4s x = {v.x, v.y, v.z, v.w};
  *(FACPPG_AS1 f32x4s*)g = x;
}
__device__ __forceinline__ void store_f1(float* g, const float v) { *(__attribute__((address_space(1))) float*)g = v; }

template <bool LAST, int NCB, bool EF, bool SEED = false>
__device__ __forceinline__ void wn_layer8_tile(const WnArgs& p, const int lin, float* __restrict__ smem) {
  static_assert(!SEED || NCB == 1, "seeded tiles: 32 frames");
  constexpr int TNt = 32 * NCB;
  WN8_STAMP_DECL;
  const int tid = threadIdx.x, lane = tid & 63, w8 = tid >> 6, wq = w8 >> 1, sub = w8 & 1;
  const int li = lane & 31, kh = lane >> 5;
  const int chb = wq * 64 + sub * 32;
  int b, nvalid, ph, in_off, sk_off, tap0, tap1, tap2, lane_q;
  int tile;
  {
    if (p.xcd_map == 1) { const int r = lin >> 3; ph = (r / p.nt) * 8 + (lin & 7); tile = r % p.nt; }
    else { ph = lin / p.nt; tile = lin % p.nt; }
    if (ph >= p.P) return;
    int qcol;
    if (p.groups) {
      const int4 e = p.groups[tile * (TNt / 4) + lane % (TNt / 4)];
      if (__builtin_amdgcn_readfirstlane(e.z) <= 0) return;
      b = e.x; qcol = e.y; nvalid = e.z;
    } else if (p.flat_cols > 0) {
      const int c0 = tile * TNt + (lane % (TNt / 4)) * 4;
      const int cl = min(c0, p.flat_cols - 4);
      b = cl / p.T; qcol = cl - b * p.T; nvalid = p.flat_cols - c0;
    } else {
      b = tile / p.ntq;
      const int q0 = (tile % p.ntq) * TNt, Tb = p.t_valid ? p.t_valid[b] : p.T;
      if (q0 >= Tb) return;
      qcol = q0 + (lane % (TNt / 4)) * 4; nvalid = Tb - qcol;
    }
    in_off = ph * p.Tqp + HQ + qcol;
    sk_off = ph * p.Tr + qcol;
    lane_q = HQ + qcol;
    {
      const int pm = ph - p.dil, qm = pm >= 0 ? pm / p.P : -((p.P - 1 - pm) / p.P);
      const int pq = ph + p.dil, qp = pq / p.P;
      tap0 = (pm - qm * p.P) * p.Tqp + qm;
      tap1 = ph * p.Tqp;
      tap2 = (pq - qp * p.P) * p.Tqp + qp;
    }
  }
  f32x16 acc[2][NCB];
  const float4* wave_a = p.w1 + (wq * 4 + sub) * 64 + lane;
  const float4* wave_c = p.wc + (size_t)ph * p.ngc * 1024 + (wq * 4 + sub) * 64 + lane;
  const int nch = SEED ? p.nconv : pm_chunks(p, ph);
  const int ncc = SEED ? 0 : nch - p.nconv;
  constexpr int F4R = TNt / 4, RPL4 = 64 / F4R, NSTG4 = 8 / RPL4;
  const int srow4 = lane / F4R, scol4 = (lane % F4R) * 4;
  const bool folded_first = EF && p.nconv == 1;
  const float* hb4 = folded_first ? p.xa + (size_t)b * 8 * p.Lp : p.h_in + (size_t)b * C * p.Lp;
  const float* sb4 = p.melp + (size_t)b * NMEL * p.Tqp + in_off - ph * p.Tqp;
  float4 stg[NSTG4];
  auto stage_load = [&](int c) __attribute__((always_inline)) {
    const bool conv = c >= ncc;
// ... 43 lines not shown
#pragma unroll
        for (int cb = 0; cb < NCB; ++cb) acc[rb][cb] = mfma32x32x2(av, bv[s][cb], acc[rb][cb]);
      }
  };
  constexpr int RING = 4;
  float4 ar[RING][2];
  stage_load(0);
#pragma unroll
  for (int i = 0; i < RING - 1; ++i) load_a1(ar[i], i);
  const float4* seedp = SEED ? p.seed + ((((size_t)ph * p.seed_nt + tile) * 8 + w8) * 8) * 64 + lane : nullptr;
#pragma unroll
  for (int rb = 0; rb < 2; ++rb) {
#pragma unroll
    for (int q = 0; q < 4; ++q) {
      const float4 bv = SEED ? gld(seedp + (rb * 4 + q) * 64) : gld(reinterpret_cast<const float4*>(p.b1 + rb * C + chb + 4 * kh + 8 * q));
      acc[rb][0][4 * q + 0] = bv.x; acc[rb][0][4 * q + 1] = bv.y; acc[rb][0][4 * q + 2] = bv.z; acc[rb][0][4 * q + 3] = bv.w;
    }
#pragma unroll
    for (int cb = 1; cb < NCB; ++cb) acc[rb][cb] = acc[rb][0];
  }
  stage_write(0);
  __syncthreads();
  WN8_STAMP(0);
  for (int c = 0; c < nch; ++c) {
    stage_load(c + 1 < nch ? c + 1 : c);
    const float* lb = smem + (c & 1) * (KCH * TNt) + (kh * TNt + li) * 4;
#pragma unroll
    for (int g = 0; g < 8; ++g) {
      load_a1(ar[(g + RING - 1) % RING], c * 8 + g + RING - 1);
      __builtin_amdgcn_sched_barrier(0);
      float bq[4][NCB];
      load_b<NCB, true>(bq, lb, g);
      mfma2(ar[g % RING], bq, 2);
    }
    stage_write((c + 1) & 1);
    __syncthreads();
  }
  WN8_STAMP(1);
#pragma unroll
  for (int cb = 0; cb < NCB; ++cb)
#pragma unroll
    for (int r = 0; r < 16; ++r)
      smem[k4_index(chb + 8 * (r >> 2) + (r & 3) + 4 * kh, cb * 32 + li, TNt)] = gate_tanh_sigmoid(acc[0][cb][r], acc[1][cb][r]);
  __syncthreads();
  WN8_STAMP(2);
  constexpr int NRB2 = EF ? (LAST ? 0 : 1) : LAST ? 1 : 2;
  constexpr bool ROWS256 = LAST || EF;
  constexpr bool ESPLIT = EF && NCB == 1;
  float4 es0, es1;
  if constexpr (ESPLIT) {
    const float4* wimg = reinterpret_cast<const float4*>(p.we) + w8 * 128 + lane * 2;
    es0 = gld(wimg); es1 = gld(wimg + 1);
  }
  constexpr bool HPRE = !LAST && NCB == 1;
  float4 hpre[HPRE ? 32 / RPL4 : 1];
  if constexpr (HPRE) {
    if (nvalid >= 4) {
      const float* rb0 = p.h_in + (size_t)b * C * p.Lp + in_off;
#pragma unroll
      for (int i = 0; i < 32 / RPL4; ++i) hpre[i] = gld(reinterpret_cast<const float4*>(rb0 + (size_t)(chb + i * RPL4 + srow4) * p.Lp));
    }
  }
#pragma unroll
  for (int rb = 0; rb < NRB2; ++rb) {
#pragma unroll
    for (int q = 0; q < 4; ++q) {
      const float4 bv = gld(reinterpret_cast<const float4*>(p.b2 + (ROWS256 ? 0 : rb * C) + chb + 4 * kh + 8 * q));
      acc[rb][0][4 * q + 0] = bv.x; acc[rb][0][4 * q + 1] = bv.y; acc[rb][0][4 * q + 2] = bv.z; acc[rb][0][4 * q + 3] = bv.w;
    }
#pragma unroll
    for (int cb = 1; cb < NCB; ++cb) acc[rb][cb] = acc[rb][0];
  }
  if constexpr (NRB2 > 0) {
    const float4* ap2 = p.w2 + (size_t)(ROWS256 ? wq * 2 + sub : wq * 4 + sub) * NG2 * 64 + lane;
    const float* lb = smem + (kh * TNt + li) * 4;
    auto load_a2 = [&](float4 (&a)[2], int g) __attribute__((always_inline)) {
      a[0] = gld(ap2 + g * 64);
      if constexpr (!ROWS256) a[1] = gld(ap2 + (size_t)2 * NG2 * 64 + g * 64);
    };
#pragma unroll
    for (int i = 0; i < RING - 1; ++i) load_a2(ar[i], i);
    for (int c = 0; c < NG2 / 8; ++c) {
#pragma unroll
      for (int g = 0; g < 8; ++g) {
        load_a2(ar[(g + RING - 1) % RING], c * 8 + g + RING - 1);
        __builtin_amdgcn_sched_barrier(0);
        float bq[4][NCB];
        load_b<NCB, true>(bq, lb, c * 8 + g);
        mfma2(ar[g % RING], bq, NRB2);
      }
    }
  }
  WN8_STAMP(3);
  if constexpr (ESPLIT) {
    const int pl = lane & 15, kq = lane >> 4;
    const float av[8] = {es0.x, es0.y, es0.z, es0.w, es1.x, es1.y, es1.z, es1.w};
#pragma unroll
    for (int blk = 0; blk < TNt / 16; ++blk) {
      const float* gb = smem + (16 * blk + pl) * 4 + kq + (8 * w8) * TNt * 4;
      f32x4 e = {0.f, 0.f, 0.f, 0.f};
#pragma unroll
      for (int g = 0; g < 8; ++g) e = mfma16x16x4(av[g], gb[g * TNt * 4], e);
      if (kq < 2) {
        float* part = smem + C * TNt + (w8 * 8 + 4 * kq) * TNt + 16 * blk + pl;
#pragma unroll
        for (int r = 0; r < 4; ++r) part[r * TNt] = e[r];
      }
    }
  } else if constexpr (EF) {
    if (w8 < TNt / 16) {
      const int pl = lane & 15, kq = lane >> 4;
      const float4* wimg = reinterpret_cast<const float4*>(p.we) + lane * 2;
      const float* gb = smem + (16 * w8 + pl) * 4 + kq;
      float4 a0[8], a1[8];
#pragma unroll
      for (int sl = 0; sl < 8; ++sl) { a0[sl] = gld(wimg + sl * 128); a1[sl] = gld(wimg + sl * 128 + 1); }
      f32x4 tot = {0.f, 0.f, 0.f, 0.f};
#pragma unroll
      for (int sl = 0; sl < 8; ++sl) {
        const float av[8] = {a0[sl].x, a0[sl].y, a0[sl].z, a0[sl].w, a1[sl].x, a1[sl].y, a1[sl].z, a1[sl].w};
        f32x4 e = {0.f, 0.f, 0.f, 0.f};
#pragma unroll
        for (int g = 0; g < 8; ++g) e = mfma16x16x4(av[g], gb[(8 * sl + g) * TNt * 4], e);
        if (sl == 0) tot = e;
        else { tot[0] += e[0]; tot[1] += e[1]; tot[2] += e[2]; tot[3] += e[3]; }
      }
      if (kq < 2) {
        float* endl = smem + C * TNt + (4 * kq) * TNt + 16 * w8 + pl;
#pragma unroll
        for (int r = 0; r < 4; ++r) endl[r * TNt] = tot[r];
      }
    }
  }
  __syncthreads();
  WN8_STAMP(4);
  if constexpr (EF) {
    const int row = w8 * RPL4 + srow4;
    if (row < 8 && nvalid > 0) {
      float4 v4 = *reinterpret_cast<const float4*>(smem + C * TNt + row * TNt + scol4);
      if constexpr (ESPLIT) {
#pragma unroll
        for (int sl = 1; sl < 8; ++sl) {
          const float4 x = *reinterpret_cast<const float4*>(smem + C * TNt + (sl * 8 + row) * TNt + scol4);
          v4.x += x.x; v4.y += x.y; v4.z += x.z; v4.w += x.w;
        }
      }
      float* g = p.skip + ((size_t)b * 8 + row) * p.Lr + sk_off;
      const float bias = p.endb[row];
      const float vv[4] = {v4.x, v4.y, v4.z, v4.w};
      if (nvalid >= 4) {
        float4 x = make_float4(bias, bias, bias, bias);
        if (!p.first) x = *reinterpret_cast<const float4*>(g);
        store_f4(g, make_float4(x.x + vv[0], x.y + vv[1], x.z + vv[2], x.w + vv[3]));
      } else {
        for (int k = 0; k < nvalid; ++k) store_f1(g + k, (p.first ? bias : g[k]) + vv[k]);
      }
    }
  }
  float* slab = smem + w8 * (32 * TNt);
#pragma unroll
  for (int half = 0; half < NRB2; ++half) {
    const bool is_res = EF || (!LAST && half == 0);
#pragma unroll
    for (int cb = 0; cb < NCB; ++cb)
#pragma unroll
      for (int r = 0; r < 16; ++r) slab[(8 * (r >> 2) + (r & 3) + 4 * kh) * TNt + cb * 32 + li] = acc[half][cb][r];
    const int nv = nvalid;
    if (nv <= 0) continue;
    float* gbase = is_res ? p.h_out + (size_t)b * C * p.Lp + in_off : p.skip + (size_t)b * C * p.Lr + sk_off;
    const float* rbase = is_res ? p.h_in + (size_t)b * C * p.Lp + in_off : gbase;
    const int pitch = is_res ? p.Lp : p.Lr;
    const bool add = is_res || !p.first;
#pragma unroll
    for (int i = 0; i < 32 / RPL4; ++i) {
      const int row = i * RPL4 + srow4;
      const size_t o = (size_t)(chb + row) * pitch;
      float4 v = *reinterpret_cast<const float4*>(slab + row * TNt + scol4);
      if (nv >= 4) {
        if (add) {
          float4 x;
          if (HPRE && is_res) x = hpre[i];
          else x = gld(reinterpret_cast<const float4*>(rbase + o));
          v.x += x.x; v.y += x.y; v.z += x.z; v.w += x.w;
        }
        store_f4(gbase + o, v);
      } else {
        const float vv[4] = {v.x, v.y, v.z, v.w};
        for (int k = 0; k < nv; ++k) store_f1(gbase + o + k, vv[k] + (add ? gld(rbase + o + k) : 0.0f));
      }
    }
  }
  WN8_STAMP(5);
}

template <bool LAST, int NCB, bool EF = false, bool SEED = false>
__global__ __launch_bounds__(512, NCB == 4 ? 2 : 4) void k_wn_layer8(WnArgs p) {
  extern __shared__ __attribute__((aligned(16))) float smem[];
  wn_layer8_tile<LAST, NCB, EF, SEED>(p, (int)blockIdx.x, smem);
}


struct WnLayerPtrs {
  const float4* w1;
  const float4* wc;
  const float* b1;
  const float4* w2;
  const float* b2;
  const float* we;
};
// ... 231 lines not shown
          acc[rbl] = mfma16x16x4(s == 0 ? a4.x : s == 1 ? a4.y : s == 2 ? a4.z : a4.w, bq[s], acc[rbl]);
        }
    }
    stage_write((c + 1) & 1);
    __syncthreads();
  }
#pragma unroll
  for (int rbl = 0; rbl < 2; ++rbl)
#pragma unroll
    for (int r = 0; r < 4; ++r)
      smem[(((2 * w8 + rbl) * 4 + 2 * (r & 1) + (kq & 1)) * TN16 + pl) * 4 + 2 * (kq >> 1) + ((r >> 1) & 1)] = gate_tanh_sigmoid(acc[rbl][r], acc[rbl + 2][r]);
  __syncthreads();
  constexpr int NB2 = EF ? (LAST ? 0 : 2) : LAST ? 2 : 4;
  constexpr bool ROWS256 = LAST || EF;
  float4 hpre[2];
  if constexpr (!LAST) {
    if (nvalid - (lane & 3) * 4 >= 4) {
#pragma unroll
      for (int it = 0; it < 2; ++it)
        hpre[it] = *reinterpret_cast<const float4*>(p.h_in + ((size_t)b * C + chb + it * 16 + (lane >> 2)) * p.Lp + in_off + (lane & 3) * 4);
    }
  }
#pragma unroll
  for (int rbl = 0; rbl < NB2; ++rbl) {
    const float4 bv = *reinterpret_cast<const float4*>(p.b2 + (ROWS256 ? 0 : (rbl >> 1) * C) + chb + (rbl & 1) * 16 + 4 * kq);
    acc[rbl][0] = bv.x; acc[rbl][1] = bv.y; acc[rbl][2] = bv.z; acc[rbl][3] = bv.w;
  }
  if constexpr (NB2 > 0) {
    const float4* ap2 = p.w2 + (w8 * NB2) * 64 + lane;
    const float* lb = smem + (kq * TN16 + pl) * 4;
    auto load_a2 = [&](float4 (&a)[4], int g) __attribute__((always_inline)) {
#pragma unroll
      for (int rbl = 0; rbl < NB2; ++rbl) a[rbl] = ap2[(size_t)g * (NB2 * 8 * 64) + rbl * 64];
    };
#pragma unroll
    for (int i = 0; i < RING - 1; ++i) load_a2(ar[i], i);
    for (int c = 0; c < C / 64; ++c) {
#pragma unroll
      for (int g = 0; g < 4; ++g) {
        load_a2(ar[(g + RING - 1) % RING], c * 4 + g + RING - 1);
        __builtin_amdgcn_sched_barrier(0);
        const float4 b4 = *reinterpret_cast<const float4*>(lb + (4 * c + g) * (4 * TN16 * 4));
        const float bq[4] = {b4.x, b4.y, b4.z, b4.w};
#pragma unroll
        for (int s = 0; s < 4; ++s)
#pragma unroll
          for (int rbl = 0; rbl < NB2; ++rbl) {
            const float4& a4 = ar[g % RING][rbl];
            acc[rbl] = mfma16x16x4(s == 0 ? a4.x : s == 1 ? a4.y : s == 2 ? a4.z : a4.w, bq[s], acc[rbl]);
          }
      }
    }
  }
  if constexpr (EF) {
    const float4* wimg = reinterpret_cast<const float4*>(p.we) + w8 * 128 + lane * 2;
    const float4 a0 = wimg[0], a1 = wimg[1];
    const float av[8] = {a0.x, a0.y, a0.z, a0.w, a1.x, a1.y, a1.z, a1.w};
    f32x4 e = {0.f, 0.f, 0.f, 0.f};
#pragma unroll
    for (int g = 0; g < 8; ++g)
      e = mfma16x16x4(av[g], smem[(((2 * w8 + (g >> 2)) * 4 + 2 * (kq & 1) + (g & 1)) * TN16 + pl) * 4 + 2 * ((g & 3) >> 1) + (kq >> 1)], e);
    if (kq < 2) {
      float* part = smem + C * TN16 + (w8 * 8 + 4 * kq) * TN16 + pl;
#pragma unroll
      for (int r = 0; r < 4; ++r) part[r * TN16] = e[r];
    }
  }
  __syncthreads();
  if constexpr (EF) {
    if (tid < 32) {
      const int row = tid >> 2, c4 = (tid & 3) * 4, nv = nvalid - c4;
      if (nv > 0) {
        const float* part = smem + C * TN16 + row * TN16 + c4;
        float4 t = *reinterpret_cast<const float4*>(part);
#pragma unroll
        for (int sl = 1; sl < 8; ++sl) {
          const float4 x = *reinterpret_cast<const float4*>(part + sl * 8 * TN16);
          t.x += x.x; t.y += x.y; t.z += x.z; t.w += x.w;
        }
        float* g = p.skip + ((size_t)b * 8 + row) * p.Lr + sk_off + c4;
        const float bias = p.endb[row];
        const float vv[4] = {t.x, t.y, t.z, t.w};
        if (nv >= 4) {
          float4 x = make_float4(bias, bias, bias, bias);
          if (!p.first) x = *reinterpret_cast<const float4*>(g);
          *reinterpret_cast<float4*>(g) = make_float4(x.x + vv[0], x.y + vv[1], x.z + vv[2], x.w + vv[3]);
        } else {
          for (int k = 0; k < nv; ++k) g[k] = (p.first ? bias : g[k]) + vv[k];
        }
      }
    }
  }
  float* slab = smem + w8 * (32 * TN16);
  const int erow = lane >> 2, ecol = (lane & 3) * 4;
#pragma unroll
  for (int half = 0; half < NB2 / 2; ++half) {
    const bool is_res = EF || (!LAST && half == 0);
#pragma unroll
    for (int rbl = 0; rbl < 2; ++rbl)
#pragma unroll
      for (int r = 0; r < 4; ++r) slab[(16 * rbl + 4 * kq + r) * TN16 + pl] = acc[half * 2 + rbl][r];
    const int nv = nvalid - ecol;
    if (nv <= 0) continue;
    float* gbase = is_res ? p.h_out + (size_t)b * C * p.Lp + in_off + ecol : p.skip + (size_t)b * C * p.Lr + sk_off + ecol;
    const float* rbase = is_res ? p.h_in + (size_t)b * C * p.Lp + in_off + ecol : gbase;
    const int pitch = is_res ? p.Lp : p.Lr;
    const bool add = is_res || !p.first;
#pragma unroll
    for (int it = 0; it < 2; ++it) {
      const int row = it * 16 + erow;
      const size_t o = (size_t)(chb + row) * pitch;
      float4 v = *reinterpret_cast<const float4*>(slab + row * TN16 + ecol);
      if (nv >= 4) {
        if (add) {
          float4 x;
          if (!LAST && is_res) x = hpre[it];
          else x = *reinterpret_cast<const float4*>(rbase + o);
          v.x += x.x; v.y += x.y; v.z += x.z; v.w += x.w;
        }
        *reinterpret_cast<float4*>(gbase + o) = v;
      } else {
        const float vv[4] = {v.x, v.y, v.z, v.w};
        for (int k = 0; k < nv; ++k) gbase[o + k] = vv[k] + (add ? rbase[o + k] : 0.0f);
      }
    }
  }
}

template <bool LAST, bool EF = false>
__global__ __launch_bounds__(512, 4) void k_wn_layer16(WnArgs p) {
  extern __shared__ __attribute__((aligned(16))) float smem[];
  int ph, tile;
  {
    const int lin = blockIdx.x;
    if (p.xcd_map == 1) { const int r = lin >> 3; ph = (r / p.nt) * 8 + (lin & 7); tile = r % p.nt; }
    else { ph = lin / p.nt; tile = lin % p.nt; }
    if (ph >= p.P) return;
  }
  wn_layer16_tile<LAST, EF>(p, ph, tile / p.ntq, (tile % p.ntq) * TN16, smem);
}

template <bool LAST>
__global__ __launch_bounds__(512, 4) void k_wn_layer_mixed(WnArgs p32, WnArgs p16, int n32) {
// ... 56 lines not shown
  for (int r = 0; r < 10; ++r) {
    const uint64_t p0 = (uint64_t)0xD2511F53u * c0, p1 = (uint64_t)0xCD9E8D57u * c2;
    const uint32_t n0 = (uint32_t)(p1 >> 32) ^ c1 ^ k0, n2 = (uint32_t)(p0 >> 32) ^ c3 ^ k1;
    c1 = (uint32_t)p1; c3 = (uint32_t)p0; c0 = n0; c2 = n2;
    k0 += 0x9E3779B9u; k1 += 0xBB67AE85u;
  }
  out[0] = c0; out[1] = c1; out[2] = c2; out[3] = c3;
}

__device__ __forceinline__ void normal4(const uint32_t (&r)[4], float (&o)[4]) {
#pragma unroll
  for (int h = 0; h < 2; ++h) {
    const float u1 = ((float)(r[2 * h] >> 8) + 0.5f) * (1.0f / 16777216.0f);
    const float u2 = ((float)(r[2 * h + 1] >> 8) + 0.5f) * (1.0f / 16777216.0f);
    const float rad = sqrtf(-2.0f * logf(u1));
    float sn, cs;
    sincosf(6.28318530717958647692f * u2, &sn, &cs);
    o[2 * h] = rad * cs; o[2 * h + 1] = rad * sn;
  }
}

__global__ void k_noise(float* __restrict__ z, size_t n, uint64_t seed) {
  const size_t i = (size_t)blockIdx.x * blockDim.x + threadIdx.x;
  if (4 * i >= n) return;
  uint32_t r[4];
  philox4x32_10((uint32_t)i, (uint32_t)(i >> 32), 0u, 0u, (uint32_t)seed, (uint32_t)(seed >> 32), r);
  float o[4];
  normal4(r, o);
  for (int j = 0; j < 4; ++j)
    if (4 * i + j < n) z[4 * i + j] = o[j];
}

__global__ void k_noise_utt(float* __restrict__ z, const uint64_t* __restrict__ seeds, int B, int L, int n_first, int n_early,
                            int n_seg) {
  const int l4 = blockIdx.x * blockDim.x + threadIdx.x, b = blockIdx.y;
  if (4 * l4 >= L) return;
  const uint64_t seed = seeds[b];
  size_t seg_off = 0;
  for (int sg = 0; sg < n_seg; ++sg) {
    const int nch = sg == 0 ? n_first : n_early;
    for (int ch = 0; ch < nch; ++ch) {
      uint32_t r[4];
      philox4x32_10((uint32_t)l4, (uint32_t)ch, (uint32_t)sg, 0x7A5Eu, (uint32_t)seed, (uint32_t)(seed >> 32), r);
      float o[4];
      normal4(r, o);
      float* dst = z + seg_off + ((size_t)b * nch + ch) * L + 4 * l4;
      for (int j = 0; j < 4; ++j)
        if (4 * l4 + j < L) dst[j] = o[j];
    }
    seg_off += (size_t)B * nch * L;
  }
}

struct EdgeArgs {
  const float* skip;
  const float* aud_in;
  float* aud_out;
  float* h_out;
  float* final_audio;
  const float* z0;
  const float* z_early;
  const float* end_w;
  const float* end_b;
  const float* winv;
  const float* start_w;
  const float* start_b;
  const int* t_valid;
  float sigma;
  int T, hop8, Lp, Lr, L, n_early, final_flow;
  int swap, swap_next;
  int La;
  int P, Tr, Tqp;
  int folded;
  float* xa_out;
};

template <int HN>
__device__ __forceinline__ void write_xa(const EdgeArgs& p, int b, int h_off, const float* a0) {
  float* dst = p.xa_out + (size_t)b * 8 * p.Lp + h_off;
#pragma unroll
  for (int j = 0; j < 8; ++j) dst[(size_t)j * p.Lp] = j < HN ? a0[j] : j == HN ? 1.0f : 0.0f;
}

__device__ __forceinline__ bool edge_pos(const EdgeArgs& p, int b, int x, int& pos, int& h_off, int& sk_off) {
  const int Tb = p.t_valid ? p.t_valid[b] : p.T;
  if (p.P > 0) {
    const int ph = blockIdx.z;
    if (x >= Tb) return false;
    pos = x * p.P + ph; h_off = ph * p.Tqp + HQ + x; sk_off = ph * p.Tr + x;
  } else {
    if (x >= Tb * p.hop8) return false;
    pos = x; h_off = HALO + x; sk_off = x;
  }
  return true;
}

template <int HN>
__device__ __forceinline__ void start_conv(const EdgeArgs& p, int b, int h_off, const float* a0, int ch0 = 0, int nch = C) {
  float* dst = p.h_out + (size_t)b * C * p.Lp + h_off;
  for (int ch = ch0; ch < ch0 + nch; ++ch) {
    float v = p.start_b[ch];
#pragma unroll
    for (int j = 0; j < HN; ++j) v = fmaf(p.start_w[ch * HN + j], a0[j], v);
    dst[(size_t)ch * p.Lp] = v;
  }
}

template <int HN, bool QS = false>
__global__ __launch_bounds__(256) void k_begin(EdgeArgs p) {
  const int b = blockIdx.y;
  const int pl = QS ? (int)(threadIdx.x & 63) : (int)threadIdx.x, wq = QS ? (int)(threadIdx.x >> 6) : 0;
  int pos, h_off, sk_off;
  if (!edge_pos(p, b, blockIdx.x * (QS ? 64 : 256) + pl, pos, h_off, sk_off)) return;
  float a[2 * HN];
#pragma unroll
  for (int j = 0; j < 2 * HN; ++j) {
    a[j] = p.sigma * p.z0[((size_t)b * 2 * HN + j) * p.L + pos];
    if (wq == 0) p.aud_out[((size_t)b * 8 + j) * p.La + pos] = a[j];
  }
  if constexpr (QS) start_conv<HN>(p, b, h_off, a + (p.swap_next ? HN : 0), 64 * wq, 64);
  else start_conv<HN>(p, b, h_off, a + (p.swap_next ? HN : 0));
  if (p.folded && wq == 0) write_xa<HN>(p, b, h_off, a + (p.swap_next ? HN : 0));
}

template <int H, bool EARLY, bool QS>
__global__ __launch_bounds__(256) void k_flow_end(EdgeArgs p) {
  constexpr int CC = 2 * H;
  __shared__ float red[QS ? 4 : 1][CC][QS ? 64 : 1];
  const int b = blockIdx.y, pl = QS ? (threadIdx.x & 63) : threadIdx.x, qtr = QS ? (threadIdx.x >> 6) : 0;
  constexpr int CQ = QS ? C / 4 : C;
  int pos = 0, h_off = 0, sk_off = 0;
  const bool valid = edge_pos(p, b, blockIdx.x * (QS ? 64 : 256) + pl, pos, h_off, sk_off);
  float o[CC];
  const float* sk = p.skip + (size_t)b * C * p.Lr + sk_off;
  auto quarter = [&](int q, float (&acc)[CC]) __attribute__((always_inline)) {
#pragma unroll
    for (int j = 0; j < CC; ++j) acc[j] = 0.0f;
    for (int c0 = q * 64; c0 < q * 64 + 64; c0 += 16) {
      float v[16];
#pragma unroll
      for (int u = 0; u < 16; ++u) v[u] = sk[(size_t)(c0 + u) * p.Lr];
#pragma unroll
      for (int u = 0; u < 16; ++u)
#pragma unroll
        for (int j = 0; j < CC; ++j) acc[j] = fmaf(p.end_w[j * C + c0 + u], v[u], acc[j]);
    }
  };
  if (p.folded) {
    if (!valid) return;
#pragma unroll
    for (int j = 0; j < CC; ++j) o[j] = p.skip[((size_t)b * 8 + j) * p.Lr + sk_off];
  } else if constexpr (QS) {
#pragma unroll
    for (int j = 0; j < CC; ++j) o[j] = 0.0f;
    if (valid) quarter(qtr, o);
#pragma unroll
    for (int j = 0; j < CC; ++j) red[qtr][j][pl] = o[j];
    __syncthreads();
    if (!valid) return;
#pragma unroll
    for (int j = 0; j < CC; ++j) o[j] = p.end_b[j] + red[0][j][pl] + red[1][j][pl] + red[2][j][pl] + red[3][j][pl];
  } else {
    if (!valid) return;
#pragma unroll
    for (int j = 0; j < CC; ++j) o[j] = p.end_b[j];
    for (int q = 0; q < 4; ++q) {
      float acc[CC];
      quarter(q, acc);
#pragma unroll
      for (int j = 0; j < CC; ++j) o[j] += acc[j];
    }
  }
  float a[CC];
#pragma unroll
  for (int j = 0; j < CC; ++j) a[j] = p.aud_in[((size_t)b * 8 + j) * p.La + pos];
  {
    const int tr = p.swap ? 0 : H;
#pragma unroll
    for (int j = 0; j < H; ++j) a[tr + j] = (a[tr + j] - o[j]) / expf(o[H + j]);
  }
  constexpr int CN = EARLY ? CC + 2 : CC;
  float y[CN];
  if (EARLY) {
#pragma unroll
    for (int j = 0; j < 2; ++j) y[j] = p.sigma * p.z_early[((size_t)b * 2 + j) * p.L + pos];
  }
#pragma unroll
  for (int i = 0; i < CC; ++i) {
    float v = 0.0f;
#pragma unroll
    for (int j = 0; j < CC; ++j) v = fmaf(p.winv[i * CC + j], a[j], v);
    y[(EARLY ? 2 : 0) + i] = v;
  }
  if (p.final_flow) {
    if (qtr == 0) {
      float* dst = p.final_audio + (size_t)b * p.T * p.hop8 * 8 + (size_t)pos * CN;
#pragma unroll
      for (int j = 0; j < CN; ++j) dst[j] = y[j];
    }
  } else {
    if (qtr == 0) {
#pragma unroll
      for (int j = 0; j < CN; ++j) p.aud_out[((size_t)b * 8 + j) * p.La + pos] = y[j];
    }
    start_conv<CN / 2>(p, b, h_off, y + (p.swap_next ? CN / 2 : 0), qtr * CQ, CQ);
    if (p.folded && qtr == 0) write_xa<CN / 2>(p, b, h_off, y + (p.swap_next ? CN / 2 : 0));
  }
}


template <int H, bool EARLY>
__global__ __launch_bounds__(256) void k_flow_end4(EdgeArgs p) {
  constexpr int CC = 2 * H, CN = EARLY ? CC + 2 : CC, HN = CN / 2;
  const int b = blockIdx.y, ph = blockIdx.z, x0 = 4 * (blockIdx.x * blockDim.x + threadIdx.x);
  const int Tb = p.t_valid ? p.t_valid[b] : p.T;
  if (x0 >= Tb) return;
  const int nv = min(4, Tb - x0);
  const int h_off = ph * p.Tqp + HQ + x0, sk_off = ph * p.Tr + x0;
  const float* sk = p.skip + (size_t)b * C * p.Lr + sk_off;
  float o[4][CC];
#pragma unroll
  for (int e = 0; e < 4; ++e)
#pragma unroll
    for (int j = 0; j < CC; ++j) o[e][j] = p.end_b[j];
  if (p.folded) {
#pragma unroll
    for (int j = 0; j < CC; ++j) {
      const float4 v = *reinterpret_cast<const float4*>(p.skip + ((size_t)b * 8 + j) * p.Lr + sk_off);
      o[0][j] = v.x; o[1][j] = v.y; o[2][j] = v.z; o[3][j] = v.w;
    }
  }
  for (int q = 0; q < (p.folded ? 0 : 4); ++q) {
    float acc[4][CC];
#pragma unroll
    for (int e = 0; e < 4; ++e)
#pragma unroll
      for (int j = 0; j < CC; ++j) acc[e][j] = 0.0f;
    for (int c0 = q * 64; c0 < q * 64 + 64; c0 += 8) {
      float4 v[8];
#pragma unroll
      for (int u = 0; u < 8; ++u) v[u] = *reinterpret_cast<const float4*>(sk + (size_t)(c0 + u) * p.Lr);
#pragma unroll
      for (int u = 0; u < 8; ++u)
#pragma unroll
        for (int j = 0; j < CC; ++j) {
          const float wv = p.end_w[j * C + c0 + u];
          acc[0][j] = fmaf(wv, v[u].x, acc[0][j]); acc[1][j] = fmaf(wv, v[u].y, acc[1][j]);
          acc[2][j] = fmaf(wv, v[u].z, acc[2][j]); acc[3][j] = fmaf(wv, v[u].w, acc[3][j]);
        }
    }
#pragma unroll
    for (int e = 0; e < 4; ++e)
#pragma unroll
      for (int j = 0; j < CC; ++j) o[e][j] += acc[e][j];
  }
  float y[4][CN];
#pragma unroll
  for (int e = 0; e < 4; ++e) {
    const int pos = (x0 + (e < nv ? e : 0)) * p.P + ph;
    float a[CC];
#pragma unroll
    for (int j = 0; j < CC; ++j) a[j] = p.aud_in[((size_t)b * 8 + j) * p.La + pos];
    const int tr = p.swap ? 0 : H;
#pragma unroll
    for (int j = 0; j < H; ++j) a[tr + j] = (a[tr + j] - o[e][j]) / expf(o[e][H + j]);
    if (EARLY) {
#pragma unroll
      for (int j = 0; j < 2; ++j) y[e][j] = p.sigma * p.z_early[((size_t)b * 2 + j) * p.L + pos];
    }
#pragma unroll
    for (int i = 0; i < CC; ++i) {
      float v = 0.0f;
#pragma unroll
      for (int j = 0; j < CC; ++j) v = fmaf(p.winv[i * CC + j], a[j], v);
      y[e][(EARLY ? 2 : 0) + i] = v;
    }
    if (e < nv) {
      if (p.final_flow) {
        float* dst = p.final_audio + (size_t)b * p.T * p.hop8 * 8 + (size_t)pos * CN;
#pragma unroll
        for (int j = 0; j < CN; ++j) dst[j] = y[e][j];
      } else {
#pragma unroll
        for (int j = 0; j < CN; ++j) p.aud_out[((size_t)b * 8 + j) * p.La + pos] = y[e][j];
      }
    }
  }
  if (p.final_flow) return;
  const int a0 = p.swap_next ? HN : 0;
  float* dst = p.h_out + (size_t)b * C * p.Lp + h_off;
  for (int ch = 0; ch < C; ++ch) {
    float v[4];
#pragma unroll
    for (int e = 0; e < 4; ++e) {
      v[e] = p.start_b[ch];
#pragma unroll
      for (int j = 0; j < HN; ++j) v[e] = fmaf(p.start_w[ch * HN + j], y[e][a0 + j], v[e]);
    }
    float* d = dst + (size_t)ch * p.Lp;
    if (nv == 4) *reinterpret_cast<float4*>(d) = make_float4(v[0], v[1], v[2], v[3]);
    else for (int e = 0; e < nv; ++e) d[e] = v[e];
  }
  if (p.folded) {
    float* xd = p.xa_out + (size_t)b * 8 * p.Lp + h_off;
#pragma unroll
    for (int j = 0; j < 8; ++j) {
      float v[4];
#pragma unroll
      for (int e = 0; e < 4; ++e) v[e] = j < HN ? y[e][a0 + j] : j == HN ? 1.0f : 0.0f;
      float* d = xd + (size_t)j * p.Lp;
      if (nv == 4) *reinterpret_cast<float4*>(d) = make_float4(v[0], v[1], v[2], v[3]);
      else for (int e = 0; e < nv; ++e) d[e] = v[e];
    }
  }
}

struct FwdArgs {
  const float* skip;
  const float* aud_in;
  float* aud_out;
  float* h_out;
  const float* audio;
  float* z_out;
  float* log_s_out;
  const float* end_w;
  const float* end_b;
  const float* w_next;
  const float* start_w;
  const float* start_b;
// ... 553 lines not shown
  }
  auto launch_cost = [](long tiles, int full, int half) {
    const long rem = tiles % 512;
    return (tiles / 512) * full + (rem == 0 ? 0 : rem <= 256 ? half : full);
  };
  const bool uniform = !T_valid_dev && T % 4 == 0;
  const long cols = (long)B * T;
  const long tiles_w = uniform ? (long)w.P * ((cols + 63) / 64) : (long)w.P * B * ((T + 63) / 64);
  const long tiles_n = uniform ? (long)w.P * ((cols + 31) / 32) : (long)w.P * B * ((T + 31) / 32);
  const long tiles_16 = (long)w.P * B * ((T + 15) / 16);
  const long cost_w = launch_cost(tiles_w, 331, 185), cost_n = launch_cost(tiles_n, 181, 94);
  const long cost_16 = launch_cost(tiles_16, FACPPG_COST16_FULL, FACPPG_COST16_HALF);
  int tn = cost_16 < cost_w && cost_16 < cost_n ? TN16 : cost_n < cost_w ? 32 : TN;
  if (const char* tile_env = getenv("FACPPG_WN_TILE")) {
    const int v = atoi(tile_env);
    FACPPG_REQUIRE(v == 16 || v == 32 || v == 64 || (v == 128 && fold), FACPPG_EINVAL,
                   "FACPPG_WN_TILE=%s: expected 16, 32, 64 or (with folded flow edges) 128", tile_env);
    tn = v;
  }
  if (seeds) {
    FACPPG_REQUIRE(B == 1 && !T_valid_dev && fold, FACPPG_EUNSUPPORTED, "seeded inference: one utterance, folded flow edges");
    FACPPG_REQUIRE(seeded_frames % 32 == 0 && seeded_frames > 0, FACPPG_EUNSUPPORTED,
                   "seeded inference: %d seeded frames, expected a positive multiple of 32", seeded_frames);
    tn = 32;
  }
  const int n32 = seeds && seeded_frames < T ? seeded_frames / 32 : 0;
  const int n16 = n32 ? (T - seeded_frames + TN16 - 1) / TN16 : 0;
  const bool tile16 = tn == TN16, narrow = tn == 32, wide128 = tn == 128;
  WnArgs a;
  memset(&a, 0, sizeof(a));
  a.melp = melp; a.skip = skip; a.t_valid = T_valid_dev; a.T = T; a.hop8 = w.P; a.Lp = w.P * w.Tqp; a.Lr = w.P * w.Tr;
  a.P = w.P; a.Tr = w.Tr; a.Tqp = w.Tqp; a.ntq = (T + tn - 1) / tn; a.nt = a.ntq * B;
  const char* no_flat = getenv("FACPPG_WN_NO_FLAT");
  if (!T_valid_dev && T % 4 == 0 && !no_flat && !tile16) { a.flat_cols = B * T; a.nt = (B * T + tn - 1) / tn; }
  if (T_valid_dev && B > 1 && !no_flat && !tile16) {
    int* goff = (int*)(ws + w.goff);
    int4* gtab = (int4*)(ws + w.gtab);
    k_group_offsets<<<1, 1024, 0, s>>>(T_valid_dev, B, goff);
    k_group_table<<<(w.ngroups + 255) / 256, 256, 0, s>>>(T_valid_dev, goff, B, gtab, w.ngroups);
    a.groups = gtab; a.nt = w.ngroups * 4 / tn;
  }
  a.ngc = h->kcp / 8; a.kc = h->kc; a.hop = c.hop_length; a.ksize = c.upsample_kernel;
  a.xa = xa;
  const char* no_xcd = getenv("FACPPG_WN_NO_XCD_MAP");
  a.xcd_map = ((w.P % 8 == 0) && !no_xcd) ? 1 : 0;
  if (n32) a.nt = n32 + n16;
  const unsigned lgrid = (unsigned)(w.P * a.nt);
  const char* w8env = getenv("FACPPG_WN_8W");
  const int w8mode = seeds ? 1 : w8env ? atoi(w8env) : 1;
  a.seed_nt = w.Tr / 32;
  h->last_tile = tn; h->last_tiles = (int)lgrid;
  h->last_waves = (wide128 || tile16 || (narrow && w8mode != 0) || (!narrow && w8mode == 2)) ? 8 : 4;
  h->ev_layers = c.wn_layers;
  for (int k = nf - 1; k >= 0; --k) {
    if (flow_events && flow_events[k]) FACPPG_HIP_CHECK(hipStreamWaitEvent(s, (hipEvent_t)flow_events[k], 0));
    for (int i = 0; i < c.wn_layers; ++i) {
      a.h_in = hbuf[hi]; a.h_out = hbuf[hi ^ 1];
      a.w1 = h->w1pm[k][i]; a.wc = h->wcpm[k][i]; a.b1 = h->b1pm[k][i]; a.w2 = h->w2[k][i]; a.b2 = h->b2[k][i];
      if (tile16) { a.w1 = h->w1_16[k][i]; a.wc = h->wc_16[k][i]; a.w2 = h->w2_16[k][i]; }
      a.dil = 1 << i; a.first = (i == 0);
      const bool last = i == c.wn_layers - 1;
      a.nconv = NCHH;
      if (fold) {
        a.we = h->we[k][i]; a.endb = h->endb[k];
        a.w2 = tile16 ? h->w2r_16[k][i] : h->w2r[k][i];
        if (i == 0) { a.nconv = 1; a.w1 = tile16 ? h->w1f_16[k] : h->w1f[k]; }
      }
      a.nch = a.nconv + h->kcp / KCH;
      if (h->profiling && i == 0) FACPPG_HIP_CHECK(hipEventRecord(h->ev[h->ev_used++], s));
#define WN_LAUNCH(KERNEL_LAST, KERNEL_MID, THREADS, LDS)              \
  do {                                                                 \
    if (last) KERNEL_LAST<<<lgrid, THREADS, LDS, s>>>(a);              \
    else KERNEL_MID<<<lgrid, THREADS, LDS, s>>>(a);                    \
  } while (0)
      if (fold) {
        if (wide128) WN_LAUNCH((k_wn_layer8<true, 4, true>), (k_wn_layer8<false, 4, true>), 512, 131072 + 4096);
        else if (tile16) WN_LAUNCH((k_wn_layer16<true, true>), (k_wn_layer16<false, true>), 512, 16384 + 4096);
        else if (narrow) {
          if (seeds) {
            a.seed = seeds + (size_t)(k * c.wn_layers + i) * w.P * a.seed_nt * 8 * 8 * 64;
            if (n32) {
              WnArgs a16 = a;
              a16.w1 = i == 0 ? h->w1f_16[k] : h->w1_16[k][i]; a16.wc = h->wc_16[k][i]; a16.w2 = last ? h->w2_16[k][i] : h->w2r_16[k][i];
              a16.flat_cols = 0; a16.groups = nullptr;
              if (last) k_wn_layer_mixed<true><<<lgrid, 512, 32768 + 8 * 1024, s>>>(a, a16, n32);
              else k_wn_layer_mixed<false><<<lgrid, 512, 32768 + 8 * 1024, s>>>(a, a16, n32);
            } else WN_LAUNCH((k_wn_layer8<true, 1, true, true>), (k_wn_layer8<false, 1, true, true>), 512, 32768 + 8 * 1024);
          } else if (w8mode == 0) WN_LAUNCH((k_wn_layer<true, 1, false, true, true>), (k_wn_layer<false, 1, false, true, true>), 256, 32768 + 1024);
          else WN_LAUNCH((k_wn_layer8<true, 1, true>), (k_wn_layer8<false, 1, true>), 512, 32768 + 8 * 1024);
        } else if (w8mode == 2) WN_LAUNCH((k_wn_layer8<true, 2, true>), (k_wn_layer8<false, 2, true>), 512, 65536 + 2048);
        else WN_LAUNCH((k_wn_layer<true, 2, false, true, true>), (k_wn_layer<false, 2, false, true, true>), 256, 65536 + 2048);
      } else {
        if (tile16) WN_LAUNCH((k_wn_layer16<true>), (k_wn_layer16<false>), 512, 16384);
        else if (narrow) {
          if (w8mode == 0) WN_LAUNCH((k_wn_layer<true, 1, false, true>), (k_wn_layer<false, 1, false, true>), 256, 32768);
          else WN_LAUNCH((k_wn_layer8<true, 1>), (k_wn_layer8<false, 1>), 512, 32768);
        } else if (w8mode == 2) WN_LAUNCH((k_wn_layer8<true, 2>), (k_wn_layer8<false, 2>), 512, 65536);
        else WN_LAUNCH((k_wn_layer<true, 2, false, true>), (k_wn_layer<false, 2, false, true>), 256, 65536);
      }
#undef WN_LAUNCH
      if (!last) hi ^= 1;
      if (h->profiling && last) FACPPG_HIP_CHECK(hipEventRecord(h->ev[h->ev_used++], s));
    }
    e.aud_in = aud[ai]; e.aud_out = aud[ai ^ 1]; e.h_out = hbuf[hi];
    e.end_w = h->end_w[k]; e.end_b = h->end_b[k]; e.winv = h->winv[k];
    e.final_flow = (k == 0);
    e.swap = c.alternate_halves && (k & 1);
    e.swap_next = c.alternate_halves && k > 0 && ((k - 1) & 1);
    e.z_early = nullptr;
    if (h->early[k]) { e.z_early = z + z_off; z_off += (size_t)B * c.n_early_size * w.L; }
    if (k > 0) { e.start_w = h->start_w[k - 1]; e.start_b = h->start_b[k - 1]; }
    const int cn = 2 * h->n_half[k] + (h->early[k] ? 2 : 0);
    if (k > 0) FACPPG_REQUIRE(cn == 2 * h->n_half[k - 1], FACPPG_EUNSUPPORTED, "flow %d channel mismatch", k);
    else FACPPG_REQUIRE(cn == 8, FACPPG_EUNSUPPORTED, "final flow must yield n_group channels");
    switch (h->n_half[k]) {
      case 1: launch_flow_end<1>(h->early[k], fqs, fgrid, s, e); break;
      case 2: launch_flow_end<2>(h->early[k], fqs, fgrid, s, e); break;
      case 3: launch_flow_end<3>(h->early[k], fqs, fgrid, s, e); break;
      case 4: launch_flow_end<4>(h->early[k], fqs, fgrid, s, e); break;
      default: FACPPG_REQUIRE(false, FACPPG_EUNSUPPORTED, "n_half %d", h->n_half[k]);
    }
    ai ^= 1;
  }
  FACPPG_HIP_CHECK(hipGetLastError());
  return FACPPG_OK;
}

extern "C" int facppg_wg_infer(facppg_wg* h, const float* mel_dev, const int32_t* T_valid_dev, const float* z_dev,
                               uint64_t seed, float sigma, int B, int T, float* audio_dev, void* ws_, size_t ws_bytes,
                               void* stream_) {
  WG_REQUIRE_FP32(h, "facppg_wg_infer");
  FACPPG_REQUIRE(h && mel_dev && audio_dev && ws_, FACPPG_EINVAL, "NULL argument");
  FACPPG_REQUIRE(B > 0 && T > 0, FACPPG_EINVAL, "B and T must be positive (got %d, %d)", B, T);
  const facppg_wg_config& c = h->cfg;
  const WsLayout w = ws_layout(c, B, T);
  {
    const size_t need = facppg_wg_workspace_bytes(h, B, T);
    FACPPG_REQUIRE(ws_bytes >= need, FACPPG_EWORKSPACE, "workspace has %zu bytes, need %zu", ws_bytes, need);
  }
  FACPPG_REQUIRE(B <= 65535, FACPPG_EINVAL, "B too large");
  {
    int tot = h->n_rem[c.n_flows - 1];
    for (int k = 0; k < c.n_flows; ++k) tot += h->early[k] ? c.n_early_size : 0;
    FACPPG_REQUIRE(tot == 8, FACPPG_EUNSUPPORTED, "noise channel count %d != n_group", tot);
  }
  const char* unfolded = getenv("FACPPG_WG_UNFOLDED");
  if (!unfolded || atoi(unfolded) == 0)
    return wg_infer_pm(h, mel_dev, T_valid_dev, z_dev, seed, sigma, B, T, audio_dev, (char*)ws_, (hipStream_t)stream_);
  hipStream_t s = (hipStream_t)stream_;
  char* ws = (char*)ws_;
  float* hbuf[2] = {(float*)(ws + w.h0), (float*)(ws + w.h1)};
  float* spect = (float*)(ws + w.spect);
  float* skip = (float*)(ws + w.skip);
  float* aud[2] = {(float*)(ws + w.aud0), (float*)(ws + w.aud1)};
  float* zbuf = (float*)(ws + w.z);
  const int hop8 = c.hop_length / 8;
  const int nf = c.n_flows;

  FACPPG_HIP_CHECK(hipMemsetAsync(ws + w.h0, 0, (size_t)B * C * w.Lp * 4 * 2, s));
  if (w.Lr != w.L || T_valid_dev) FACPPG_HIP_CHECK(hipMemsetAsync(spect, 0, (size_t)B * NCOND * w.Lr * 4, s));

  const float* z = z_dev;
  const size_t zn = (size_t)B * 8 * w.L;
  if (!z) {
    k_noise<<<(unsigned)((zn / 4 + 255) / 256 + 1), 256, 0, s>>>(zbuf, zn, seed);
    z = zbuf;
  }
  {
    dim3 g((T + UP_QB - 1) / UP_QB, c.n_mel_channels, B);
    const size_t sm = (size_t)c.n_mel_channels * (UP_QB + UP_MAXJ) * 4;
    k_upsample<<<g, 256, sm, s>>>(mel_dev, h->up_w, h->up_b, spect, T_valid_dev, T, c.n_mel_channels, c.hop_length,
                                  c.upsample_kernel, w.Lr, T * c.hop_length);
  }
// ... 521 lines not shown
```

### fac-via-ppg_amd/waveglow/glow.py

```python
import os

import torch

from facppg import lib as _lib


def fused_add_tanh_sigmoid_multiply(input_a, input_b, n_channels):
    n = int(n_channels[0])
    in_act = input_a + input_b
    return torch.tanh(in_act[:, :n, :]) * torch.sigmoid(in_act[:, n:, :])


def _sum_segment(t):
    if t.dim() == 0 or t.is_contiguous():
        return 1, 0, t.numel()
    if t.dim() == 3 and t.stride(2) == 1 and t.stride(1) == t.size(2):
        return t.size(0), t.stride(0), t.size(1) * t.size(2)
    return None


class _GlowLossFunction(torch.autograd.Function):

    @staticmethod
    def forward(ctx, sigma, n_log_s, z, *rest):
        L = _lib.load()
        dev = z.device
        log_s, log_det = rest[:n_log_s], rest[n_log_s:]
        tensors = [z] + list(log_s)
        segs = (_lib.SumSegment * len(tensors))()
        for i, t in enumerate(tensors):
            outer, stride, inner = _sum_segment(t)
            segs[i] = _lib.SumSegment(t.data_ptr(), stride, outer, inner, 1 if i == 0 else 0)
        ws = torch.empty(len(tensors) * 64, dtype=torch.float64, device=dev)
        sums = torch.empty(len(tensors), dtype=torch.float32, device=dev)
        with torch.cuda.device(dev):
            _lib.check(L.facppg_segment_sums(segs, len(tensors), _lib.ptr(ws), ws.numel() * 8, _lib.ptr(sums), _lib.current_stream(dev)))
        n = z.numel()
        total = sums[0] * (0.5 / (sigma * sigma)) - sums[1:].sum()
        if log_det:
            total = total - torch.stack([t.reshape(()) for t in log_det]).sum()
        ctx.save_for_backward(z)
        ctx.sigma, ctx.n = float(sigma), n
        ctx.shapes = [t.shape for t in rest]
        return total / n

    @staticmethod
    def backward(ctx, g):
        (z,) = ctx.saved_tensors
        c = g / ctx.n
        neg = -c
        return (None, None, z * (c * (1.0 / (ctx.sigma * ctx.sigma)))) + tuple(neg.expand(sh) for sh in ctx.shapes)


# ... 923 lines not shown
        best = None
        for frames, full, half in self._ROUND_COSTS:
            cols = sum(-(-int(n) // 4) * 4 for n in lengths)
            tiles = P * -(-cols // frames)
            rem = tiles % 512
            cost = (tiles // 512) * full + (0 if rem == 0 else half if rem <= 256 else full)
            if best is None or cost < best[0]:
                best = (cost, tiles / 512.0 * full, tiles)
        return 1.0 - best[1] / best[0] if best[0] and best[2] > 512 else 0.0

    def _infer_two_groups(self, spect, sigma, zt, lengths, seed, utterance_seeds):
        dev, hop, g8 = spect.device, self.upsample.stride[0], self.n_group
        B, _, T = spect.shape
        order = sorted(range(B), key=lambda i: (-int(lengths[i]), i))
        side = _infer_side_stream(dev)
        cur = torch.cuda.current_stream(dev)
        out = torch.zeros(B, T * hop, dtype=torch.float32, device=dev)
        Lfull = T * hop // g8
        segs = None
        if zt is not None:
            chans = [self.n_remaining_channels] + [self.n_early_size] * ((g8 - self.n_remaining_channels) // self.n_early_size)
            segs, off = [], 0
            for c in chans:
                segs.append(zt[off:off + B * c * Lfull].view(B, c, Lfull))
                off += B * c * Lfull
        sel = _lib.upload(order[0::2] + order[1::2] + [int(lengths[i]) for i in order[0::2] + order[1::2]], torch.int64, dev)
        parts, n0 = [], len(order[0::2])
        for gi, idx in enumerate((order[0::2], order[1::2])):
            it = sel[:n0] if gi == 0 else sel[n0:B]
            lt = (sel[B:B + n0] if gi == 0 else sel[B + n0:]).to(torch.int32)
            Tg = max(int(lengths[i]) for i in idx)
            mel_g = spect.index_select(0, it)[:, :, :Tg].contiguous()
            if utterance_seeds is not None:
                z_g = self.draw_noise([utterance_seeds[i] for i in idx], Tg, dev)
            elif segs is not None:
                z_g = torch.cat([sg.index_select(0, it)[:, :, :Tg * hop // g8].reshape(-1) for sg in segs])
            else:
                z_g = None
            a = torch.zeros(len(idx), Tg * hop, dtype=torch.float32, device=dev)
            ws = self._infer_workspace(len(idx), Tg, dev, gi)
            parts.append((it, lt, Tg, mel_g, z_g, a, ws))
        side.wait_stream(cur)
        for gi, (it, lt, Tg, mel_g, z_g, a, ws) in enumerate(parts):
            with torch.cuda.stream(side if gi else cur):
                self._infer_launch(mel_g, lt, z_g, (seed + 0x9E3779B97F4A7C15 * gi) & 0x7FFFFFFFFFFFFFFF, sigma, a, ws)
        cur.wait_stream(side)
        for it, lt, Tg, mel_g, z_g, a, ws in parts:
            out[:, :Tg * hop].index_copy_(0, it, a)
        return out

    def _infer_workspace(self, B, T, dev, slot, handle=None):
        nbytes = _lib.load().facppg_wg_workspace_bytes(handle if handle is not None else self._handle(dev), B, T)
        wss = self.__dict__.setdefault("_facppg_ws", {})
        ws = wss.get(slot)
        if ws is None or ws.numel() < nbytes or ws.device != dev:
            ws = torch.empty(nbytes, dtype=torch.uint8, device=dev)
            wss[slot] = ws
        return ws

    def _infer_launch(self, spect, lt, zt, seed, sigma, audio, ws, handle=None):
        dev = spect.device
        B, _, T = spect.shape
        with torch.cuda.device(dev):
            _lib.check(_lib.load().facppg_wg_infer(handle if handle is not None else self._handle(dev), _lib.ptr(spect), _lib.ptr(lt), _lib.ptr(zt),
                                                   seed & 0xFFFFFFFFFFFFFFFF, float(sigma), B, T, _lib.ptr(audio),
                                                   _lib.ptr(ws), ws.numel(), _lib.current_stream(dev)))

    def seed_layout(self, T, device):
        c = _lib.ctypes
        tqp, mg, nb = c.c_int(), c.c_int(), c.c_size_t()
        _lib.check(_lib.load().facppg_wg_seed_layout(self._handle(device), int(T), c.byref(tqp), c.byref(mg), c.byref(nb)))
        return tqp.value, mg.value, nb.value

    def mel_pad(self, mel, handle=None):
        dev = mel.device
        T = mel.shape[2]
        tqp, _, _ = self.seed_layout(T, dev)
        out = torch.empty(mel.shape[1], tqp, dtype=torch.float32, device=dev)
        m = mel[0]
        with torch.cuda.device(dev):
            _lib.check(_lib.load().facppg_wg_mel_pad(self._handle(dev), _lib.ptr(m), T, m.stride(0), _lib.ptr(out), _lib.current_stream(dev)))
        return out

    def cond_seed(self, melp, T, frame0, nframes, seeds, block_tiles=1, layers_per_workgroup=4, skip=None, handle=None, flows=None,
                  max_workgroups=0, counter=None):
        dev = melp.device
        f0, nf = flows if flows is not None else (0, 0)
        with torch.cuda.device(dev):
            _lib.check(_lib.load().facppg_wg_cond_seed(handle if handle is not None else self._handle(dev), _lib.ptr(melp), int(T), int(frame0),
                                                       int(nframes), int(block_tiles), int(layers_per_workgroup), int(f0), int(nf), _lib.ptr(seeds),
                                                       seeds.numel() * seeds.element_size(), _lib.ptr(skip), int(max_workgroups), _lib.ptr(counter),
                                                       _lib.current_stream(dev)))

    def infer_seeded(self, melp, T, seeds, seeded_frames, sigma=1.0, z=None, seed=None, handle=None, T_layout=None, flow_events=None):
        T_layout = T if T_layout is None else int(T_layout)
        dev = melp.device
        hop = self.upsample.stride[0]
        zt = None
        if z is not None:
            if isinstance(z, (list, tuple)):
                z = torch.cat([t.to(dev).float().reshape(-1) for t in z])
            zt = z.to(dev).float().contiguous()
            if zt.numel() != self.n_group * (T * hop // self.n_group):
                raise _lib.FacppgError("z has %d values, expected n_group*L = %d" % (zt.numel(), self.n_group * (T * hop // self.n_group)))
        if seed is None:
            seed = int(torch.empty((), dtype=torch.int64).random_().item())
        h = handle if handle is not None else self._handle(dev)
        ws = self._infer_workspace(1, T_layout, dev, 0, h)
        audio = torch.empty(1, T * hop, dtype=torch.float32, device=dev)
        evs = None
# ... 137 lines not shown
```

Measured before the change: 4.344 million.

## Fuse split-K reduction into GEMM via tickets and fuse WaveGlow flow edge into last WN layer

Adds an optional in-launch split-K reduction where the last-arriving block per tile, found through atomic tickets, sums the partials, replacing the separate reduce kernel. It is gated by the FACPPG_GEMM_REDUCE=inlaunch environment variable, so it is off by default. Separately, WaveGlow's flow-end coupling kernel is fused into the last WN layer launch for batch-1 folded configurations, which is on by default, to remove one launch per flow. It also makes Python workspaces per-thread and merges memsets in the Tacotron encoder. The changes add code complexity and a need for atomic ordering correctness.

```diff
diff --git a/fac-via-ppg_amd/common/stft.py b/fac-via-ppg_amd/common/stft.py
--- a/fac-via-ppg_amd/common/stft.py
+++ b/fac-via-ppg_amd/common/stft.py
@@ -1,3 +1,5 @@
+import threading
+
 import numpy as np
 import torch
 from scipy.signal import get_window
@@ -80,10 +82,12 @@
 
     def _workspace(self, h, dev, B, N):
         nbytes = _lib.load().facppg_stft_workspace_bytes(h, B, N)
-        ws = self.__dict__.get("_facppg_ws")
+        wss = self.__dict__.setdefault("_facppg_ws", {})
+        key = threading.get_ident()
+        ws = wss.get(key)
         if ws is None or ws.numel() < nbytes or ws.device != dev:
             ws = torch.empty(nbytes, dtype=torch.uint8, device=dev)
-            self.__dict__["_facppg_ws"] = ws
+            wss[key] = ws
         return ws
 
     @staticmethod
diff --git a/fac-via-ppg_amd/csrc/facppg_dsp.hip b/fac-via-ppg_amd/csrc/facppg_dsp.hip
--- a/fac-via-ppg_amd/csrc/facppg_dsp.hip
+++ b/fac-via-ppg_amd/csrc/facppg_dsp.hip
@@ -88,7 +88,7 @@
 
 struct Ws {
   int F;
-  size_t X, S, Z, fv, sk, sk_bytes, total;
+  size_t X, S, Z, fv, tk, tk_bytes, sk, sk_bytes, total;
 };
 Ws ws_layout(const facppg_stft* h, int B, int N) {
   Ws w;
@@ -99,13 +99,15 @@
   w.S = take((size_t)B * (h->fl + 2) * w.F * 4);
   w.Z = take((size_t)B * w.F * h->fl * 4);
   w.fv = take((size_t)B * 4);
+  w.tk_bytes = (gemm_ticket_words(B, h->fl + 2, w.F) + gemm_ticket_words(B, h->fl, w.F)) * sizeof(unsigned);
+  w.tk = take(w.tk_bytes);
   w.sk_bytes = (size_t)4 * B * (h->fl + 2) * w.F * 4;
   w.sk = take(w.sk_bytes);
   w.total = off;
   return w;
 }
 
-int run_forward(facppg_stft* h, const float* audio, const int* n_valid, int B, int N, char* ws, const Ws& w, hipStream_t s) {
+int run_forward(facppg_stft* h, const float* audio, const int* n_valid, int B, int N, char* ws, const Ws& w, GemmTickets& tk, hipStream_t s) {
   float* X = (float*)(ws + w.X);
   float* S = (float*)(ws + w.S);
   int* fv = (int*)(ws + w.fv);
@@ -115,15 +117,17 @@
   a.A = h->fwd; a.M = 2 * h->cutoff; a.Cin = h->fl; a.X = X; a.x_bs = (long)h->fl * w.F; a.ldx = w.F; a.N = w.F;
   a.n_valid = fv; a.C = S; a.c_bs = (long)2 * h->cutoff * w.F; a.ldc = w.F; a.B = B;
   a.splitk_ws = (float*)(ws + w.sk); a.splitk_ws_bytes = w.sk_bytes;
+  a.tickets = tk.take(B, a.M, w.F);
   return gemm_launch(a, s);
 }
 
-int run_inverse(facppg_stft* h, const float* R, int B, char* ws, const Ws& w, const int* fv, float* out, long out_bs, hipStream_t s) {
+int run_inverse(facppg_stft* h, const float* R, int B, char* ws, const Ws& w, const int* fv, float* out, long out_bs, GemmTickets& tk, hipStream_t s) {
   float* Z = (float*)(ws + w.Z);
   GemmArgs a;
   a.A = h->inv_t; a.M = h->fl; a.Cin = 2 * h->cutoff; a.X = R; a.x_bs = (long)2 * h->cutoff * w.F; a.ldx = w.F; a.N = w.F;
   a.n_valid = fv; a.C = Z; a.c_bs = (long)w.F * h->fl; a.ldc = h->fl; a.c_transposed = 1; a.B = B;
   a.splitk_ws = (float*)(ws + w.sk); a.splitk_ws_bytes = w.sk_bytes;
+  a.tickets = tk.take(B, a.M, w.F);
   if (int rc = gemm_launch(a, s)) return rc;
   const int n_out = h->hop * (w.F - 1);
   if (n_out > 0) {
@@ -200,7 +204,8 @@
   if (int rc = check_common(h, audio_dev, mag_dev, ws_, B, N, ws_bytes, &w)) return rc;
   hipStream_t s = (hipStream_t)stream_;
   char* ws = (char*)ws_;
-  if (int rc = run_forward(h, audio_dev, n_valid_dev, B, N, ws, w, s)) return rc;
+  GemmTickets tk(ws + w.tk, w.tk_bytes, s);
+  if (int rc = run_forward(h, audio_dev, n_valid_dev, B, N, ws, w, tk, s)) return rc;
   dim3 g((w.F + 255) / 256, h->cutoff, B);
   k_magphase<<<g, 256, 0, s>>>((float*)(ws + w.S), mag_dev, phase_dev, (int*)(ws + w.fv), h->cutoff, w.F);
   FACPPG_HIP_CHECK(hipGetLastError());
@@ -217,9 +222,10 @@
   hipStream_t s = (hipStream_t)stream_;
   char* ws = (char*)ws_;
   float* R = (float*)(ws + w.X);
+  GemmTickets tk(ws + w.tk, w.tk_bytes, s);
   dim3 g((F + 255) / 256, h->cutoff, B);
   k_recombine<<<g, 256, 0, s>>>(mag_dev, phase_dev, R, nullptr, h->cutoff, F);
-  return run_inverse(h, R, B, ws, w, nullptr, out_dev, (long)h->hop * (F - 1), s);
+  return run_inverse(h, R, B, ws, w, nullptr, out_dev, (long)h->hop * (F - 1), tk, s);
 }
 
 extern "C" int facppg_stft_mel(facppg_stft* h, const float* audio_dev, const int32_t* n_valid_dev, int B, int N, float* mel_dev,
@@ -229,7 +235,8 @@
   FACPPG_REQUIRE(h->n_mel > 0, FACPPG_EINVAL, "handle was created without a mel basis");
   hipStream_t s = (hipStream_t)stream_;
   char* ws = (char*)ws_;
-  if (int rc = run_forward(h, audio_dev, n_valid_dev, B, N, ws, w, s)) return rc;
+  GemmTickets tk(ws + w.tk, w.tk_bytes, s);
+  if (int rc = run_forward(h, audio_dev, n_valid_dev, B, N, ws, w, tk, s)) return rc;
   float* mag = (float*)(ws + w.X);
   int* fv = (int*)(ws + w.fv);
   dim3 g((w.F + 255) / 256, h->cutoff, B);
@@ -247,10 +254,11 @@
   FACPPG_REQUIRE(bias_spec_dev, FACPPG_EINVAL, "bias_spec is NULL");
   hipStream_t s = (hipStream_t)stream_;
   char* ws = (char*)ws_;
-  if (int rc = run_forward(h, audio_dev, n_valid_dev, B, N, ws, w, s)) return rc;
+  GemmTickets tk(ws + w.tk, w.tk_bytes, s);
+  if (int rc = run_forward(h, audio_dev, n_valid_dev, B, N, ws, w, tk, s)) return rc;
   float* S = (float*)(ws + w.S);
   int* fv = (int*)(ws + w.fv);
   dim3 g((w.F + 255) / 256, h->cutoff, B);
   k_spectral_subtract<<<g, 256, 0, s>>>(S, bias_spec_dev, strength, fv, h->cutoff, w.F);
-  return run_inverse(h, S, B, ws, w, fv, out_dev, (long)h->hop * (w.F - 1), s);
-}
+  return run_inverse(h, S, B, ws, w, fv, out_dev, (long)h->hop * (w.F - 1), tk, s);
+}
diff --git a/fac-via-ppg_amd/csrc/facppg_gemm.h b/fac-via-ppg_amd/csrc/facppg_gemm.h
--- a/fac-via-ppg_amd/csrc/facppg_gemm.h
+++ b/fac-via-ppg_amd/csrc/facppg_gemm.h
@@ -45,6 +45,29 @@
   int B = 1;
   float* splitk_ws = nullptr;
   size_t splitk_ws_bytes = 0;
+  unsigned* tickets = nullptr;
+};
+
+inline size_t gemm_ticket_words(int B, int M, int N) { return (size_t)B * ((round_up(M, 32) / 32 + 3) / 4) * ((N + 63) / 64); }
+
+bool gemm_inlaunch_enabled();
+
+struct GemmTickets {
+  unsigned* next = nullptr;
+  unsigned* end = nullptr;
+  GemmTickets() = default;
+  GemmTickets(void* base, size_t bytes, hipStream_t s, bool zeroed_by_caller = false) {
+    if (!gemm_inlaunch_enabled()) return;
+    if (!zeroed_by_caller && hipMemsetAsync(base, 0, bytes, s) != hipSuccess) return;
+    next = (unsigned*)base; end = (unsigned*)base + bytes / sizeof(unsigned);
+  }
+  unsigned* take(int B, int M, int N) {
+    const size_t n = gemm_ticket_words(B, M, N);
+    if (!next || (size_t)(end - next) < n) return nullptr;
+    unsigned* t = next;
+    next += n;
+    return t;
+  }
 };
 
 int gemm_launch(const GemmArgs& a, hipStream_t s);
diff --git a/fac-via-ppg_amd/csrc/facppg_gemm.hip b/fac-via-ppg_amd/csrc/facppg_gemm.hip
--- a/fac-via-ppg_amd/csrc/facppg_gemm.hip
+++ b/fac-via-ppg_amd/csrc/facppg_gemm.hip
@@ -1,4 +1,7 @@
 #include "facppg_gemm.h"
+
+#include <cstdlib>
+#include <cstring>
 
 namespace facppg {
 namespace {
@@ -109,18 +112,94 @@
     stage_write((c + 1) & 1);
     __syncthreads();
   }
-  if (!active) return;
-#pragma unroll
-  for (int cb = 0; cb < 2; ++cb) {
-    const int n = n0 + cb * 32 + li;
-    if (n >= Nb) continue;
-#pragma unroll
-    for (int r = 0; r < 16; ++r) {
-      const int m = mb * 32 + 8 * (r >> 2) + (r & 3) + 4 * kh;
-      if (m >= p.M) continue;
-      if (ka.sk > 1) p.splitk_ws[(((size_t)ks * p.B + b) * p.M + m) * p.N + n] = acc[cb][r];
-      else gemm_epilogue(p, b, m, n, acc[cb][r]);
-    }
+  const bool inlaunch = ka.sk > 1 && p.tickets;
+  if (!active && !inlaunch) return;
+  if (active) {
+#pragma unroll
+    for (int cb = 0; cb < 2; ++cb) {
+      const int n = n0 + cb * 32 + li;
+      if (n >= Nb) continue;
+#pragma unroll
+      for (int r = 0; r < 16; ++r) {
+        const int m = mb * 32 + 8 * (r >> 2) + (r & 3) + 4 * kh;
+        if (m >= p.M) continue;
+        if (ka.sk > 1) p.splitk_ws[(((size_t)ks * p.B + b) * p.M + m) * p.N + n] = acc[cb][r];
+        else gemm_epilogue(p, b, m, n, acc[cb][r]);
+      }
+    }
+  }
+  if (!inlaunch) return;
+  asm volatile("s_waitcnt vmcnt(0)" ::: "memory");
+  __syncthreads();
+  unsigned* const am_last = reinterpret_cast<unsigned*>(smem);
+  if (tid == 0) {
+    __builtin_amdgcn_fence(__ATOMIC_RELEASE, "agent");
+    asm volatile("s_waitcnt vmcnt(0)" ::: "memory");
+    const unsigned tile = ((unsigned)b * gridDim.y + blockIdx.y) * gridDim.x + blockIdx.x;
+    const unsigned t = __hip_atomic_fetch_add(p.tickets + tile, 1u, __ATOMIC_RELAXED, __HIP_MEMORY_SCOPE_AGENT);
+    const bool last = t == (unsigned)ka.sk - 1u;
+    if (last) {
+      __builtin_amdgcn_fence(__ATOMIC_ACQUIRE, "agent");
+      asm volatile("s_waitcnt vmcnt(0)" ::: "memory");
+    }
+    *am_last = last ? 1u : 0u;
+  }
+  __syncthreads();
+  if (!*am_last) return;
+  const size_t slab = (size_t)p.B * p.M * p.N;
+  const float* part = p.splitk_ws + (size_t)b * p.M * p.N;
+  const int mt = blockIdx.y * 128;
+  if ((p.N & 3) == 0 && (n0 & 3) == 0) {
+    const int c4 = n0 + 4 * (tid & 15), rq = tid >> 4;
+    if (c4 >= Nb) return;
+    for (int r0 = rq; r0 < 128 && mt + r0 < p.M; r0 += 32) {
+      const int ma = mt + r0, mb2 = min(ma + 16, p.M - 1);
+      float v[2][4] = {{0.0f, 0.0f, 0.0f, 0.0f}, {0.0f, 0.0f, 0.0f, 0.0f}};
+      for (int sb = 0; sb < ka.sk; sb += 4) {
+        float4 x[2][4];
+#pragma unroll
+        for (int s = 0; s < 4; ++s) {
+          if (sb + s < ka.sk) {
+            x[0][s] = *reinterpret_cast<const float4*>(part + (size_t)(sb + s) * slab + (size_t)ma * p.N + c4);
+            x[1][s] = *reinterpret_cast<const float4*>(part + (size_t)(sb + s) * slab + (size_t)mb2 * p.N + c4);
+          }
+        }
+#pragma unroll
+        for (int s = 0; s < 4; ++s) {
+          if (sb + s < ka.sk) {
+#pragma unroll
+            for (int h = 0; h < 2; ++h) { v[h][0] += x[h][s].x; v[h][1] += x[h][s].y; v[h][2] += x[h][s].z; v[h][3] += x[h][s].w; }
+          }
+        }
+      }
+#pragma unroll
+      for (int h = 0; h < 2; ++h) {
+        const int m = ma + 16 * h;
+        if (m >= p.M) continue;
+#pragma unroll
+        for (int e = 0; e < 4; ++e)
+          if (c4 + e < Nb) gemm_epilogue(p, b, m, c4 + e, v[h][e]);
+      }
+    }
+    return;
+  }
+  const int n = n0 + lane;
+  if (n >= Nb) return;
+  part += n;
+  const int m0 = mt + w * 32;
+  for (int r0 = 0; r0 < 32 && m0 + r0 < p.M; r0 += 8) {
+    float v[8];
+    size_t row[8];
+#pragma unroll
+    for (int j = 0; j < 8; ++j) { v[j] = 0.0f; row[j] = (size_t)min(m0 + r0 + j, p.M - 1) * p.N; }
+    for (int s = 0; s < ka.sk; ++s) {
+      const float* ps = part + (size_t)s * slab;
+#pragma unroll
+      for (int j = 0; j < 8; ++j) v[j] += ps[row[j]];
+    }
+#pragma unroll
+    for (int j = 0; j < 8; ++j)
+      if (m0 + r0 + j < p.M) gemm_epilogue(p, b, m0 + r0 + j, n, v[j]);
   }
 }
 
@@ -135,6 +214,11 @@
   gemm_epilogue(p, b, m, n, v);
 }
 
+}
+
+bool gemm_inlaunch_enabled() {
+  const char* e = getenv("FACPPG_GEMM_REDUCE");
+  return e && !strcmp(e, "inlaunch");
 }
 
 int pack_a_strided(const float* src, int M, int Cin, int taps, long sm, long sc, long st, long off, float4* dst, hipStream_t s) {
@@ -165,9 +249,10 @@
                    a.splitk_ws_bytes, need);
     ka.sk = sk;
   }
+  if (ka.sk == 1 || !gemm_inlaunch_enabled()) ka.g.tickets = nullptr;
   grid.z = a.B * ka.sk;
   k_gemm<<<grid, 256, 0, s>>>(ka);
-  if (ka.sk > 1) k_gemm_reduce<<<dim3((a.N - a.col0 + 255) / 256, a.M, a.B), 256, 0, s>>>(ka);
+  if (ka.sk > 1 && !ka.g.tickets) k_gemm_reduce<<<dim3((a.N - a.col0 + 255) / 256, a.M, a.B), 256, 0, s>>>(ka);
   FACPPG_HIP_CHECK(hipGetLastError());
   return FACPPG_OK;
 }
diff --git a/fac-via-ppg_amd/csrc/facppg_taco.hip b/fac-via-ppg_amd/csrc/facppg_taco.hip
--- a/fac-via-ppg_amd/csrc/facppg_taco.hip
+++ b/fac-via-ppg_amd/csrc/facppg_taco.hip
@@ -1408,7 +1408,7 @@
 }
 
 struct TWs {
-  size_t a0, a1, xproj, mem_cm, mask, xchg, splitk, splitk_bytes, total;
+  size_t a0, a1, xproj, mem_cm, mask, xchg, tickets, tickets_bytes, splitk, splitk_bytes, total;
 };
 TWs tws_layout(const facppg_taco_config& c, int B, int Tin) {
   TWs w;
@@ -1421,6 +1421,9 @@
   w.mem_cm = take((size_t)B * c.encoder_embedding_dim * Tin * 4);
   w.mask = take((size_t)2 * B * c.symbols_embedding_dim * Tin);
   w.xchg = take((size_t)B * 2 * 2 * (c.encoder_embedding_dim / 2) * 8);
+  w.tickets_bytes = ((2 + c.encoder_n_convolutions) * gemm_ticket_words(B, (int)E, Tin) + gemm_ticket_words(B, 4 * c.encoder_embedding_dim, Tin) +
+                     gemm_ticket_words(B, c.attention_dim, Tin)) * sizeof(unsigned);
+  w.tickets = take(w.tickets_bytes);
   const size_t mx = c.encoder_embedding_dim > c.symbols_embedding_dim ? c.encoder_embedding_dim : c.symbols_embedding_dim;
   w.splitk_bytes = (size_t)16 * B * mx * Tin * 4;
   w.splitk = take(w.splitk_bytes);
@@ -1709,13 +1712,22 @@
     k_random_mask<<<(unsigned)((n + 255) / 256), 256, 0, s>>>(m, n, seed);
     masks = m;
   }
+  const char* bilstm_mode = getenv("FACPPG_BILSTM_MODE");
+  const bool no_coop = bilstm_mode && !strcmp(bilstm_mode, "single");
+  const bool fit32 = (long)B * 2 * ((H + 31) / 32) <= h->coop_limit && (H + 3) / 4 <= 96 && !(bilstm_mode && !strcmp(bilstm_mode, "wide"));
+  const bool fit64 = (long)B * 2 * ((H + 63) / 64) <= h->coop_limit && (H + 1) / 2 <= 152;
+  const bool coop = !no_coop && (fit32 || fit64);
+  if (coop) FACPPG_HIP_CHECK(hipMemsetAsync(ws + w.xchg, 0, w.tickets + w.tickets_bytes - w.xchg, s));
+  GemmTickets tk(ws + w.tickets, w.tickets_bytes, s, coop);
   GemmArgs g;
   g.B = B; g.N = Tin; g.n_valid = padded_batch ? nullptr : lengths_dev;
   g.splitk_ws = (float*)(ws + w.splitk); g.splitk_ws_bytes = w.splitk_bytes;
   g.A = h->pre0; g.M = S; g.Cin = c.n_symbols; g.X = ppg_dev; g.x_bs = (long)c.n_symbols * Tin; g.ldx = Tin; g.act = ACT_RELU;
   g.mask = masks; g.mask_bs = (long)S * Tin; g.ldmask = Tin; g.C = a0; g.c_bs = (long)S * Tin; g.ldc = Tin;
+  g.tickets = tk.take(B, g.M, Tin);
   if (int rc = gemm_launch(g, s)) return rc;
   g.A = h->pre1; g.Cin = S; g.X = a0; g.x_bs = (long)S * Tin; g.mask = masks + (size_t)B * S * Tin; g.C = a1;
+  g.tickets = tk.take(B, g.M, Tin);
   if (int rc = gemm_launch(g, s)) return rc;
   float* cur = a1;
   float* nxt = a0;
@@ -1724,6 +1736,7 @@
     g.A = h->conv[j]; g.M = E; g.Cin = E; g.taps = c.encoder_kernel_size; g.pad = (c.encoder_kernel_size - 1) / 2; g.X = cur;
     g.x_bs = (long)E * Tin; g.bias = h->conv_b[j]; g.scale = h->conv_scale[j]; g.shift = h->conv_shift[j]; g.C = nxt;
     g.c_bs = (long)E * Tin;
+    g.tickets = tk.take(B, g.M, Tin);
     if (int rc = gemm_launch(g, s)) return rc;
     float* t = cur; cur = nxt; nxt = t;
   }
@@ -1731,14 +1744,10 @@
   p.splitk_ws = g.splitk_ws; p.splitk_ws_bytes = g.splitk_ws_bytes;
   p.B = B; p.N = Tin; p.n_valid = lengths_dev; p.A = h->wih; p.M = 8 * H; p.Cin = E; p.X = cur; p.x_bs = (long)E * Tin; p.ldx = Tin;
   p.bias = h->lstm_b; p.C = xproj; p.c_bs = (long)Tin * 8 * H; p.ldc = 8 * H; p.c_transposed = 1;
+  p.tickets = tk.take(B, p.M, Tin);
   if (int rc = gemm_launch(p, s)) return rc;
-  const char* bilstm_mode = getenv("FACPPG_BILSTM_MODE");
-  const bool no_coop = bilstm_mode && !strcmp(bilstm_mode, "single");
-  const bool fit32 = (long)B * 2 * ((H + 31) / 32) <= h->coop_limit && (H + 3) / 4 <= 96 && !(bilstm_mode && !strcmp(bilstm_mode, "wide"));
-  const bool fit64 = (long)B * 2 * ((H + 63) / 64) <= h->coop_limit && (H + 1) / 2 <= 152;
-  if (!no_coop && (fit32 || fit64)) {
+  if (coop) {
     unsigned long long* xchg = (unsigned long long*)(ws + w.xchg);
-    FACPPG_HIP_CHECK(hipMemsetAsync(xchg, 0, (size_t)B * 2 * 2 * H * 8, s));
     const float *w0 = h->whh_t[0], *w1 = h->whh_t[1];
     const float* xp = xproj;
     int Tin_ = Tin, H_ = H;
@@ -1755,6 +1764,7 @@
   m.splitk_ws = g.splitk_ws; m.splitk_ws_bytes = g.splitk_ws_bytes;
   m.B = B; m.N = Tin; m.n_valid = lengths_dev; m.A = h->mem_w; m.M = c.attention_dim; m.Cin = E; m.X = mem_cm; m.x_bs = (long)E * Tin;
   m.ldx = Tin; m.C = pm_dev; m.c_bs = (long)Tin * c.attention_dim; m.ldc = Tin;
+  m.tickets = tk.take(B, m.M, Tin);
   if (int rc = gemm_launch(m, s)) return rc;
   FACPPG_HIP_CHECK(hipGetLastError());
   return FACPPG_OK;
@@ -1959,7 +1969,7 @@
 }
 
 namespace {
-struct ForcedWs { size_t x0, p1, p2, xa, hc, mg, mask, xchg, prof, splitk, splitk_bytes, total; };
+struct ForcedWs { size_t x0, p1, p2, xa, hc, mg, mask, xchg, prof, tickets, tickets_bytes, splitk, splitk_bytes, total; };
 ForcedWs forced_ws(const facppg_taco_config& c, int B, int T) {
   ForcedWs w;
   size_t off = 0;
@@ -1974,6 +1984,8 @@
   w.mask = take(2 * BT * c.prenet_dim);
   w.xchg = take(BT * (c.attention_rnn_dim + c.encoder_embedding_dim + c.decoder_rnn_dim) * 8);
   w.prof = take(32 * 8);
+  w.tickets_bytes = gemm_ticket_words(B, c.n_acoustic_feat_dims + 1, T) * sizeof(unsigned);
+  w.tickets = take(w.tickets_bytes);
   w.splitk_bytes = 16 * BT * (c.n_acoustic_feat_dims + 1) * 4;
   w.splitk = take(w.splitk_bytes);
   w.total = off;
@@ -2063,7 +2075,7 @@
     vc = vd = 4; chunk = wg_limit / (2 * h->coop_nwg[4]);
   }
   unsigned long long* xw = (unsigned long long*)(ws + w.xchg);
-  FACPPG_HIP_CHECK(hipMemsetAsync(xw, 0, w.prof + 32 * 8 - w.xchg, s));
+  FACPPG_HIP_CHECK(hipMemsetAsync(xw, 0, w.tickets + w.tickets_bytes - w.xchg, s));
   a.prof = getenv("FACPPG_DECODER_PROF") ? (long long*)(ws + w.prof) : nullptr;
   const void* fn = regw ? (const void*)k_decoder_forced<true> : (const void*)k_decoder_forced<false>;
   FACPPG_HIP_CHECK(hipFuncSetAttribute(fn, hipFuncAttributeMaxDynamicSharedMemorySize, (int)smem));
@@ -2091,6 +2103,7 @@
   q.splitk_ws = (float*)(ws + w.splitk); q.splitk_ws_bytes = w.splitk_bytes;
   q.B = B; q.N = T; q.A = h->tf_proj; q.M = NF + 1; q.Cin = KP; q.X = hc; q.x_bs = (long)KP * T; q.ldx = T; q.bias = h->proj_b;
   q.C = mg; q.c_bs = (long)(NF + 1) * T; q.ldc = T;
+  q.tickets = GemmTickets(ws + w.tickets, w.tickets_bytes, s, true).take(B, q.M, T);
   if (int rc = gemm_launch(q, s)) return rc;
   {
     const size_t n = (size_t)B * (NF + 1) * T;
@@ -2151,7 +2164,9 @@
   hipStream_t s = (hipStream_t)stream_;
   float* buf[2] = {(float*)ws_, (float*)ws_ + (size_t)B * PE * T};
   float* skws = (float*)ws_ + (size_t)2 * B * PE * T;
-  const size_t skws_bytes = need - (size_t)2 * B * PE * T * 4;
+  const size_t skws_bytes = (size_t)16 * B * PE * T * 4;
+  const size_t tk_bytes = n * gemm_ticket_words(B, PE, T) * sizeof(unsigned);
+  GemmTickets tk((char*)skws + skws_bytes, tk_bytes, s);
   const float* cur = mel_dev;
   long cur_bs = (long)NF * ld;
   int cur_ld = ld;
@@ -2167,6 +2182,7 @@
     } else {
       g.res = mel_dev; g.res_bs = (long)NF * ld; g.ldres = ld; g.C = mel_post_dev; g.c_bs = (long)NF * ld; g.ldc = ld;
     }
+    g.tickets = tk.take(B, co, T);
     if (int rc = gemm_launch(g, s)) return rc;
     cur = g.C; cur_bs = g.c_bs; cur_ld = g.ldc;
   }
@@ -2176,7 +2192,8 @@
 extern "C" size_t facppg_taco_postnet_workspace_bytes(const facppg_taco* h, int B, int T) {
   if (!h || B <= 0 || T <= 0) return 0;
   const size_t sk = (size_t)16 * B * h->c.postnet_embedding_dim * T * 4;
-  return (size_t)2 * B * h->c.postnet_embedding_dim * T * 4 + sk;
+  const size_t tk = h->c.postnet_n_convolutions * gemm_ticket_words(B, h->c.postnet_embedding_dim, T) * sizeof(unsigned);
+  return (size_t)2 * B * h->c.postnet_embedding_dim * T * 4 + sk + tk;
 }
 
 namespace {
@@ -2235,7 +2252,8 @@
 extern "C" size_t facppg_taco_postnet_stream_workspace_bytes(const facppg_taco* h, int max_frames) {
   if (!h || max_frames <= 0) return 0;
   const size_t PE = h->c.postnet_embedding_dim, n = h->c.postnet_n_convolutions;
-  return (n - 1) * PE * max_frames * 4 + (size_t)16 * PE * max_frames * 4;
+  const size_t tk = n * gemm_ticket_words(1, (int)PE, max_frames) * sizeof(unsigned);
+  return (n - 1) * PE * max_frames * 4 + (size_t)16 * PE * max_frames * 4 + tk;
 }
 
 extern "C" int facppg_taco_postnet_range(const facppg_taco* h, const float* mel_dev, int ld, int f_prev, int f_new, int final_T,
@@ -2253,6 +2271,8 @@
   float* bufs = (float*)ws_;
   float* skws = bufs + (size_t)(n - 1) * PE * max_frames;
   const size_t skws_bytes = (size_t)16 * PE * max_frames * 4;
+  const size_t tk_bytes = n * gemm_ticket_words(1, PE, max_frames) * sizeof(unsigned);
+  GemmTickets tk((char*)skws + skws_bytes, tk_bytes, s);
   int src_hi = f_new;
   for (int j = 0; j < n; ++j) {
     const int lag = pad * (j + 1);
@@ -2268,6 +2288,7 @@
       g.bias = h->post_b[j]; g.scale = h->post_scale[j]; g.shift = h->post_shift[j];
       if (j < n - 1) { g.act = ACT_TANH; g.C = bufs + (size_t)j * PE * max_frames; g.ldc = max_frames; }
       else { g.res = mel_dev; g.ldres = ld; g.C = mel_post_dev; g.ldc = ld_post; }
+      g.tickets = tk.take(1, co, hi);
       if (int rc = gemm_launch(g, s)) return rc;
     }
     src_hi = hi > 0 ? hi : 0;
diff --git a/fac-via-ppg_amd/csrc/facppg_tdnn.hip b/fac-via-ppg_amd/csrc/facppg_tdnn.hip
--- a/fac-via-ppg_amd/csrc/facppg_tdnn.hip
+++ b/fac-via-ppg_amd/csrc/facppg_tdnn.hip
@@ -49,7 +49,7 @@
   }
 }
 
-struct TdnnWs { size_t x[2], splitk, splitk_bytes, total; int Tp; };
+struct TdnnWs { size_t x[2], tickets, tickets_bytes, splitk, splitk_bytes, total; int Tp; };
 TdnnWs tdnn_ws(const facppg_tdnn* h, int T) {
   TdnnWs w;
   w.Tp = h->left + T + h->right;
@@ -57,6 +57,8 @@
   auto take = [&](size_t bytes) { size_t o = off; off += (bytes + 255) / 256 * 256; return o; };
   w.x[0] = take((size_t)h->max_dim * w.Tp * 4);
   w.x[1] = take((size_t)h->max_dim * w.Tp * 4);
+  w.tickets_bytes = h->n_layers * gemm_ticket_words(1, h->max_dim, w.Tp) * sizeof(unsigned);
+  w.tickets = take(w.tickets_bytes);
   w.splitk_bytes = (size_t)16 * h->max_dim * w.Tp * 4;
   w.splitk = take(w.splitk_bytes);
   w.total = off;
@@ -169,6 +171,7 @@
   char* ws = (char*)ws_;
   float* x[2] = {(float*)(ws + w.x[0]), (float*)(ws + w.x[1])};
   const int Tp = w.Tp;
+  GemmTickets tk(ws + w.tickets, w.tickets_bytes, s);
   k_tdnn_input<<<dim3((Tp + 255) / 256, h->in_dim), 256, 0, s>>>(feats_dev, x[0], T, h->in_dim, h->left, Tp);
   int cur = 0;
   for (int i = 0; i < h->n_layers; ++i) {
@@ -178,6 +181,7 @@
     g.X = x[cur]; g.ldx = Tp; g.N = Tp; g.bias = h->bias[i]; g.act = l.relu ? ACT_RELU : ACT_NONE;
     g.C = x[cur ^ 1]; g.ldc = Tp; g.B = 1;
     g.splitk_ws = (float*)(ws + w.splitk); g.splitk_ws_bytes = w.splitk_bytes;
+    g.tickets = tk.take(1, l.out_dim, Tp);
     const int rc = gemm_launch(g, s);
     if (rc != FACPPG_OK) return rc;
     cur ^= 1;
diff --git a/fac-via-ppg_amd/csrc/facppg_wg.hip b/fac-via-ppg_amd/csrc/facppg_wg.hip
--- a/fac-via-ppg_amd/csrc/facppg_wg.hip
+++ b/fac-via-ppg_amd/csrc/facppg_wg.hip
@@ -247,6 +247,29 @@
   }
   table[g] = e;
 }
+
+struct EdgeArgs {
+  const float* skip;
+  const float* aud_in;
+  float* aud_out;
+  float* h_out;
+  float* final_audio;
+  const float* z0;
+  const float* z_early;
+  const float* end_w;
+  const float* end_b;
+  const float* winv;
+  const float* start_w;
+  const float* start_b;
+  const int* t_valid;
+  float sigma;
+  int T, hop8, Lp, Lr, L, n_early, final_flow;
+  int swap, swap_next;
+  int La;
+  int P, Tr, Tqp;
+  int folded;
+  float* xa_out;
+};
 
 struct WnArgs {
   const float* h_in;
@@ -272,6 +295,8 @@
   int nconv;
   const float4* seed;
   int seed_nt;
+  EdgeArgs edge;
+  int edge_fuse, edge_h, edge_early;
 };
 
 typedef float f4u __attribute__((ext_vector_type(4), aligned(4)));
@@ -736,6 +761,128 @@
 }
 __device__ __forceinline__ void store_f1(float* g, const float v) { *(__attribute__((address_space(1))) float*)g = v; }
 
+template <int HN>
+__device__ __forceinline__ void write_xa(const EdgeArgs& p, int b, int h_off, const float* a0) {
+  float* dst = p.xa_out + (size_t)b * 8 * p.Lp + h_off;
+#pragma unroll
+  for (int j = 0; j < 8; ++j) dst[(size_t)j * p.Lp] = j < HN ? a0[j] : j == HN ? 1.0f : 0.0f;
+}
+
+__device__ __forceinline__ bool edge_pos(const EdgeArgs& p, int b, int x, int& pos, int& h_off, int& sk_off) {
+  const int Tb = p.t_valid ? p.t_valid[b] : p.T;
+  if (p.P > 0) {
+    const int ph = blockIdx.z;
+    if (x >= Tb) return false;
+    pos = x * p.P + ph; h_off = ph * p.Tqp + HQ + x; sk_off = ph * p.Tr + x;
+  } else {
+    if (x >= Tb * p.hop8) return false;
+    pos = x; h_off = HALO + x; sk_off = x;
+  }
+  return true;
+}
+
+template <int HN>
+__device__ __forceinline__ void start_conv(const EdgeArgs& p, int b, int h_off, const float* a0, int ch0 = 0, int nch = C) {
+  float* dst = p.h_out + (size_t)b * C * p.Lp + h_off;
+  for (int ch = ch0; ch < ch0 + nch; ++ch) {
+    float v = p.start_b[ch];
+#pragma unroll
+    for (int j = 0; j < HN; ++j) v = fmaf(p.start_w[ch * HN + j], a0[j], v);
+    dst[(size_t)ch * p.Lp] = v;
+  }
+}
+
+template <int H, bool EARLY>
+__device__ __forceinline__ void edge_fetch(const EdgeArgs& p, int b, int pos, float (&a)[2 * H], float (&z)[2]) {
+#pragma unroll
+  for (int j = 0; j < 2 * H; ++j) a[j] = p.aud_in[((size_t)b * 8 + j) * p.La + pos];
+  if constexpr (EARLY) {
+#pragma unroll
+    for (int j = 0; j < 2; ++j) z[j] = p.z_early[((size_t)b * 2 + j) * p.L + pos];
+  }
+}
+
+template <int H, bool EARLY>
+__device__ __forceinline__ void edge_couple(const EdgeArgs& p, const float (&o)[2 * H], float (&a)[2 * H], const float (&z)[2],
+                                            float (&y)[EARLY ? 2 * H + 2 : 2 * H]) {
+  constexpr int CC = 2 * H;
+  {
+    const int tr = p.swap ? 0 : H;
+#pragma unroll
+    for (int j = 0; j < H; ++j) a[tr + j] = (a[tr + j] - o[j]) / expf(o[H + j]);
+  }
+  if constexpr (EARLY) {
+#pragma unroll
+    for (int j = 0; j < 2; ++j) y[j] = p.sigma * z[j];
+  }
+#pragma unroll
+  for (int i = 0; i < CC; ++i) {
+    float v = 0.0f;
+#pragma unroll
+    for (int j = 0; j < CC; ++j) v = fmaf(p.winv[i * CC + j], a[j], v);
+    y[(EARLY ? 2 : 0) + i] = v;
+  }
+}
+
+template <int CN>
+__device__ __forceinline__ void edge_emit(const EdgeArgs& p, int b, int pos, int h_off, const float (&y)[CN], bool writer, int ch0, int nch) {
+  if (p.final_flow) {
+    if (writer) {
+      float* dst = p.final_audio + (size_t)b * p.T * p.hop8 * 8 + (size_t)pos * CN;
+#pragma unroll
+      for (int j = 0; j < CN; ++j) dst[j] = y[j];
+    }
+  } else {
+    if (writer) {
+#pragma unroll
+      for (int j = 0; j < CN; ++j) p.aud_out[((size_t)b * 8 + j) * p.La + pos] = y[j];
+    }
+    start_conv<CN / 2>(p, b, h_off, y + (p.swap_next ? CN / 2 : 0), ch0, nch);
+    if (p.folded && writer) write_xa<CN / 2>(p, b, h_off, y + (p.swap_next ? CN / 2 : 0));
+  }
+}
+
+template <int H, bool EARLY>
+__device__ __forceinline__ void flow_edge_position(const EdgeArgs& p, int b, int pos, int h_off, const float (&o)[2 * H], bool writer,
+                                                   int ch0, int nch) {
+  float a[2 * H], z[2] = {0.0f, 0.0f}, y[EARLY ? 2 * H + 2 : 2 * H];
+  edge_fetch<H, EARLY>(p, b, pos, a, z);
+  edge_couple<H, EARLY>(p, o, a, z, y);
+  edge_emit<EARLY ? 2 * H + 2 : 2 * H>(p, b, pos, h_off, y, writer, ch0, nch);
+}
+
+struct EdgePre { float a[8], z[2]; };
+__device__ __forceinline__ void wn_edge_prefetch(const EdgeArgs& e, int n_half, bool early, int pos, EdgePre& pre) {
+#pragma unroll
+  for (int j = 0; j < 8; ++j) pre.a[j] = j < 2 * n_half ? e.aud_in[(size_t)j * e.La + pos] : 0.0f;
+#pragma unroll
+  for (int j = 0; j < 2; ++j) pre.z[j] = early ? e.z_early[(size_t)j * e.L + pos] : 0.0f;
+}
+template <int H, bool EARLY>
+__device__ __forceinline__ void wn_fused_edge_t(const EdgeArgs& e, int pos, int h_off, const float* fin, int pitch, const EdgePre& pre,
+                                                bool writer, int ch0, int nch) {
+  float o[2 * H], a[2 * H], y[EARLY ? 2 * H + 2 : 2 * H];
+#pragma unroll
+  for (int j = 0; j < 2 * H; ++j) { o[j] = fin[j * pitch]; a[j] = pre.a[j]; }
+  edge_couple<H, EARLY>(e, o, a, pre.z, y);
+  edge_emit<EARLY ? 2 * H + 2 : 2 * H>(e, 0, pos, h_off, y, writer, ch0, nch);
+}
+__device__ __forceinline__ void wn_fused_edge(const EdgeArgs& e, int n_half, bool early, int pos, int h_off, const float* fin, int pitch,
+                                              const EdgePre& pre, bool writer, int ch0, int nch) {
+#define FACPPG_EDGE_CASE(HH)                                                                     \
+  case HH:                                                                                       \
+    if (early) wn_fused_edge_t<HH, true>(e, pos, h_off, fin, pitch, pre, writer, ch0, nch);      \
+    else wn_fused_edge_t<HH, false>(e, pos, h_off, fin, pitch, pre, writer, ch0, nch);           \
+    break;
+  switch (n_half) {
+    FACPPG_EDGE_CASE(1)
+    FACPPG_EDGE_CASE(2)
+    FACPPG_EDGE_CASE(3)
+    FACPPG_EDGE_CASE(4)
+  }
+#undef FACPPG_EDGE_CASE
+}
+
 template <bool LAST, int NCB, bool EF, bool SEED = false>
 __device__ __forceinline__ void wn_layer8_tile(const WnArgs& p, const int lin, float* __restrict__ smem) {
   static_assert(!SEED || NCB == 1, "seeded tiles: 32 frames");
@@ -885,6 +1032,17 @@
     const float4* wimg = reinterpret_cast<const float4*>(p.we) + w8 * 128 + lane * 2;
     es0 = gld(wimg); es1 = gld(wimg + 1);
   }
+  constexpr bool EDGE = LAST && ESPLIT;
+  [[maybe_unused]] bool fuse = false;
+  [[maybe_unused]] int ex = 0;
+  [[maybe_unused]] EdgePre epre;
+  if constexpr (EDGE) {
+    fuse = p.edge_fuse != 0;
+    if (fuse) {
+      ex = (p.flat_cols > 0 ? tile : tile % p.ntq) * TNt + li;
+      if (ex < p.T) wn_edge_prefetch(p.edge, p.edge_h, p.edge_early != 0, ex * p.P + ph, epre);
+    }
+  }
   constexpr bool HPRE = !LAST && NCB == 1;
   float4 hpre[HPRE ? 32 / RPL4 : 1];
   if constexpr (HPRE) {
@@ -981,13 +1139,31 @@
       float* g = p.skip + ((size_t)b * 8 + row) * p.Lr + sk_off;
       const float bias = p.endb[row];
       const float vv[4] = {v4.x, v4.y, v4.z, v4.w};
-      if (nvalid >= 4) {
+      if (EDGE && fuse) {
+        float fin[4] = {0.0f, 0.0f, 0.0f, 0.0f};
+        if (nvalid >= 4) {
+          float4 x = make_float4(bias, bias, bias, bias);
+          if (!p.first) x = *reinterpret_cast<const float4*>(g);
+          fin[0] = x.x + vv[0]; fin[1] = x.y + vv[1]; fin[2] = x.z + vv[2]; fin[3] = x.w + vv[3];
+        } else {
+          for (int k = 0; k < nvalid; ++k) fin[k] = (p.first ? bias : g[k]) + vv[k];
+        }
+        *reinterpret_cast<float4*>(smem + row * TNt + scol4) = make_float4(fin[0], fin[1], fin[2], fin[3]);
+      } else if (nvalid >= 4) {
         float4 x = make_float4(bias, bias, bias, bias);
         if (!p.first) x = *reinterpret_cast<const float4*>(g);
         store_f4(g, make_float4(x.x + vv[0], x.y + vv[1], x.z + vv[2], x.w + vv[3]));
       } else {
         for (int k = 0; k < nvalid; ++k) store_f1(g + k, (p.first ? bias : g[k]) + vv[k]);
       }
+    }
+  }
+  if constexpr (EDGE) {
+    if (fuse) {
+      __syncthreads();
+      if (ex < p.T)
+        wn_fused_edge(p.edge, p.edge_h, p.edge_early != 0, ex * p.P + ph, ph * p.Tqp + HQ + ex, smem + li, TNt, epre, w8 == 0 && kh == 0,
+                      w8 * 32 + kh * 16, 16);
     }
   }
   float* slab = smem + w8 * (32 * TNt);
@@ -1325,6 +1501,13 @@
       }
     }
   }
+  constexpr bool EDGE = LAST && EF;
+  [[maybe_unused]] bool fuse = false;
+  [[maybe_unused]] EdgePre epre;
+  if constexpr (EDGE) {
+    fuse = p.edge_fuse != 0;
+    if (fuse && pl < nvalid) wn_edge_prefetch(p.edge, p.edge_h, p.edge_early != 0, (q0 + pl) * p.P + ph, epre);
+  }
   if constexpr (EF) {
     const float4* wimg = reinterpret_cast<const float4*>(p.we) + w8 * 128 + lane * 2;
     const float4 a0 = wimg[0], a1 = wimg[1];
@@ -1354,7 +1537,17 @@
         float* g = p.skip + ((size_t)b * 8 + row) * p.Lr + sk_off + c4;
         const float bias = p.endb[row];
         const float vv[4] = {t.x, t.y, t.z, t.w};
-        if (nv >= 4) {
+        if (EDGE && fuse) {
+          float fin[4] = {0.0f, 0.0f, 0.0f, 0.0f};
+          if (nv >= 4) {
+            float4 x = make_float4(bias, bias, bias, bias);
+            if (!p.first) x = *reinterpret_cast<const float4*>(g);
+            fin[0] = x.x + vv[0]; fin[1] = x.y + vv[1]; fin[2] = x.z + vv[2]; fin[3] = x.w + vv[3];
+          } else {
+            for (int k = 0; k < nv; ++k) fin[k] = (p.first ? bias : g[k]) + vv[k];
+          }
+          *reinterpret_cast<float4*>(smem + row * TN16 + c4) = make_float4(fin[0], fin[1], fin[2], fin[3]);
+        } else if (nv >= 4) {
           float4 x = make_float4(bias, bias, bias, bias);
           if (!p.first) x = *reinterpret_cast<const float4*>(g);
           *reinterpret_cast<float4*>(g) = make_float4(x.x + vv[0], x.y + vv[1], x.z + vv[2], x.w + vv[3]);
@@ -1362,6 +1555,14 @@
           for (int k = 0; k < nv; ++k) g[k] = (p.first ? bias : g[k]) + vv[k];
         }
       }
+    }
+  }
+  if constexpr (EDGE) {
+    if (fuse) {
+      __syncthreads();
+      if (pl < nvalid)
+        wn_fused_edge(p.edge, p.edge_h, p.edge_early != 0, (q0 + pl) * p.P + ph, ph * p.Tqp + HQ + q0 + pl, smem + pl, TN16, epre,
+                      w8 == 0 && kq == 0, w8 * 32 + kq * 8, 8);
     }
   }
   float* slab = smem + w8 * (32 * TN16);
@@ -1524,60 +1725,6 @@
   }
 }
 
-struct EdgeArgs {
-  const float* skip;
-  const float* aud_in;
-  float* aud_out;
-  float* h_out;
-  float* final_audio;
-  const float* z0;
-  const float* z_early;
-  const float* end_w;
-  const float* end_b;
-  const float* winv;
-  const float* start_w;
-  const float* start_b;
-  const int* t_valid;
-  float sigma;
-  int T, hop8, Lp, Lr, L, n_early, final_flow;
-  int swap, swap_next;
-  int La;
-  int P, Tr, Tqp;
-  int folded;
-  float* xa_out;
-};
-
-template <int HN>
-__device__ __forceinline__ void write_xa(const EdgeArgs& p, int b, int h_off, const float* a0) {
-  float* dst = p.xa_out + (size_t)b * 8 * p.Lp + h_off;
-#pragma unroll
-  for (int j = 0; j < 8; ++j) dst[(size_t)j * p.Lp] = j < HN ? a0[j] : j == HN ? 1.0f : 0.0f;
-}
-
-__device__ __forceinline__ bool edge_pos(const EdgeArgs& p, int b, int x, int& pos, int& h_off, int& sk_off) {
-  const int Tb = p.t_valid ? p.t_valid[b] : p.T;
-  if (p.P > 0) {
-    const int ph = blockIdx.z;
-    if (x >= Tb) return false;
-    pos = x * p.P + ph; h_off = ph * p.Tqp + HQ + x; sk_off = ph * p.Tr + x;
-  } else {
-    if (x >= Tb * p.hop8) return false;
-    pos = x; h_off = HALO + x; sk_off = x;
-  }
-  return true;
-}
-
-template <int HN>
-__device__ __forceinline__ void start_conv(const EdgeArgs& p, int b, int h_off, const float* a0, int ch0 = 0, int nch = C) {
-  float* dst = p.h_out + (size_t)b * C * p.Lp + h_off;
-  for (int ch = ch0; ch < ch0 + nch; ++ch) {
-    float v = p.start_b[ch];
-#pragma unroll
-    for (int j = 0; j < HN; ++j) v = fmaf(p.start_w[ch * HN + j], a0[j], v);
-    dst[(size_t)ch * p.Lp] = v;
-  }
-}
-
 template <int HN, bool QS = false>
 __global__ __launch_bounds__(256) void k_begin(EdgeArgs p) {
   const int b = blockIdx.y;
@@ -1643,41 +1790,7 @@
       for (int j = 0; j < CC; ++j) o[j] += acc[j];
     }
   }
-  float a[CC];
-#pragma unroll
-  for (int j = 0; j < CC; ++j) a[j] = p.aud_in[((size_t)b * 8 + j) * p.La + pos];
-  {
-    const int tr = p.swap ? 0 : H;
-#pragma unroll
-    for (int j = 0; j < H; ++j) a[tr + j] = (a[tr + j] - o[j]) / expf(o[H + j]);
-  }
-  constexpr int CN = EARLY ? CC + 2 : CC;
-  float y[CN];
-  if (EARLY) {
-#pragma unroll
-    for (int j = 0; j < 2; ++j) y[j] = p.sigma * p.z_early[((size_t)b * 2 + j) * p.L + pos];
-  }
-#pragma unroll
-  for (int i = 0; i < CC; ++i) {
-    float v = 0.0f;
-#pragma unroll
-    for (int j = 0; j < CC; ++j) v = fmaf(p.winv[i * CC + j], a[j], v);
-    y[(EARLY ? 2 : 0) + i] = v;
-  }
-  if (p.final_flow) {
-    if (qtr == 0) {
-      float* dst = p.final_audio + (size_t)b * p.T * p.hop8 * 8 + (size_t)pos * CN;
-#pragma unroll
-      for (int j = 0; j < CN; ++j) dst[j] = y[j];
-    }
-  } else {
-    if (qtr == 0) {
-#pragma unroll
-      for (int j = 0; j < CN; ++j) p.aud_out[((size_t)b * 8 + j) * p.La + pos] = y[j];
-    }
-    start_conv<CN / 2>(p, b, h_off, y + (p.swap_next ? CN / 2 : 0), qtr * CQ, CQ);
-    if (p.folded && qtr == 0) write_xa<CN / 2>(p, b, h_off, y + (p.swap_next ? CN / 2 : 0));
-  }
+  flow_edge_position<H, EARLY>(p, b, pos, h_off, o, qtr == 0, qtr * CQ, CQ);
 }
 
 
@@ -1730,23 +1843,9 @@
 #pragma unroll
   for (int e = 0; e < 4; ++e) {
     const int pos = (x0 + (e < nv ? e : 0)) * p.P + ph;
-    float a[CC];
-#pragma unroll
-    for (int j = 0; j < CC; ++j) a[j] = p.aud_in[((size_t)b * 8 + j) * p.La + pos];
-    const int tr = p.swap ? 0 : H;
-#pragma unroll
-    for (int j = 0; j < H; ++j) a[tr + j] = (a[tr + j] - o[e][j]) / expf(o[e][H + j]);
-    if (EARLY) {
-#pragma unroll
-      for (int j = 0; j < 2; ++j) y[e][j] = p.sigma * p.z_early[((size_t)b * 2 + j) * p.L + pos];
-    }
-#pragma unroll
-    for (int i = 0; i < CC; ++i) {
-      float v = 0.0f;
-#pragma unroll
-      for (int j = 0; j < CC; ++j) v = fmaf(p.winv[i * CC + j], a[j], v);
-      y[e][(EARLY ? 2 : 0) + i] = v;
-    }
+    float a[CC], z[2] = {0.0f, 0.0f};
+    edge_fetch<H, EARLY>(p, b, pos, a, z);
+    edge_couple<H, EARLY>(p, o[e], a, z, y[e]);
     if (e < nv) {
       if (p.final_flow) {
         float* dst = p.final_audio + (size_t)b * p.T * p.hop8 * 8 + (size_t)pos * CN;
@@ -2406,8 +2505,25 @@
   h->last_tile = tn; h->last_tiles = (int)lgrid;
   h->last_waves = (wide128 || tile16 || (narrow && w8mode != 0) || (!narrow && w8mode == 2)) ? 8 : 4;
   h->ev_layers = c.wn_layers;
+  const char* fuse_env = getenv("FACPPG_WG_EDGE_FUSE");
+  const bool fuse_edge = (!fuse_env || atoi(fuse_env) != 0) && fold && B == 1 && !T_valid_dev && !c.alternate_halves && c.wn_layers > 1 &&
+                         (tile16 || (narrow && (seeds || w8mode != 0)));
   for (int k = nf - 1; k >= 0; --k) {
     if (flow_events && flow_events[k]) FACPPG_HIP_CHECK(hipStreamWaitEvent(s, (hipEvent_t)flow_events[k], 0));
+    e.aud_in = aud[ai]; e.aud_out = aud[ai ^ 1];
+    e.end_w = h->end_w[k]; e.end_b = h->end_b[k]; e.winv = h->winv[k];
+    e.final_flow = (k == 0);
+    e.swap = c.alternate_halves && (k & 1);
+    e.swap_next = c.alternate_halves && k > 0 && ((k - 1) & 1);
+    e.z_early = nullptr;
+    if (h->early[k]) { e.z_early = z + z_off; z_off += (size_t)B * c.n_early_size * w.L; }
+    if (k > 0) { e.start_w = h->start_w[k - 1]; e.start_b = h->start_b[k - 1]; }
+    {
+      const int cn = 2 * h->n_half[k] + (h->early[k] ? 2 : 0);
+      if (k > 0) FACPPG_REQUIRE(cn == 2 * h->n_half[k - 1], FACPPG_EUNSUPPORTED, "flow %d channel mismatch", k);
+      else FACPPG_REQUIRE(cn == 8, FACPPG_EUNSUPPORTED, "final flow must yield n_group channels");
+      FACPPG_REQUIRE(h->n_half[k] >= 1 && h->n_half[k] <= 4, FACPPG_EUNSUPPORTED, "n_half %d", h->n_half[k]);
+    }
     for (int i = 0; i < c.wn_layers; ++i) {
       a.h_in = hbuf[hi]; a.h_out = hbuf[hi ^ 1];
       a.w1 = h->w1pm[k][i]; a.wc = h->wcpm[k][i]; a.b1 = h->b1pm[k][i]; a.w2 = h->w2[k][i]; a.b2 = h->b2[k][i];
@@ -2421,6 +2537,11 @@
         if (i == 0) { a.nconv = 1; a.w1 = tile16 ? h->w1f_16[k] : h->w1f[k]; }
       }
       a.nch = a.nconv + h->kcp / KCH;
+      a.edge_fuse = 0;
+      if (last && fuse_edge) {
+        e.h_out = hbuf[hi ^ 1];
+        a.edge = e; a.edge_fuse = 1; a.edge_h = h->n_half[k]; a.edge_early = h->early[k] ? 1 : 0;
+      }
       if (h->profiling && i == 0) FACPPG_HIP_CHECK(hipEventRecord(h->ev[h->ev_used++], s));
 #define WN_LAUNCH(KERNEL_LAST, KERNEL_MID, THREADS, LDS)              \
   do {                                                                 \
@@ -2456,23 +2577,16 @@
       if (!last) hi ^= 1;
       if (h->profiling && last) FACPPG_HIP_CHECK(hipEventRecord(h->ev[h->ev_used++], s));
     }
-    e.aud_in = aud[ai]; e.aud_out = aud[ai ^ 1]; e.h_out = hbuf[hi];
-    e.end_w = h->end_w[k]; e.end_b = h->end_b[k]; e.winv = h->winv[k];
-    e.final_flow = (k == 0);
-    e.swap = c.alternate_halves && (k & 1);
-    e.swap_next = c.alternate_halves && k > 0 && ((k - 1) & 1);
-    e.z_early = nullptr;
-    if (h->early[k]) { e.z_early = z + z_off; z_off += (size_t)B * c.n_early_size * w.L; }
-    if (k > 0) { e.start_w = h->start_w[k - 1]; e.start_b = h->start_b[k - 1]; }
-    const int cn = 2 * h->n_half[k] + (h->early[k] ? 2 : 0);
-    if (k > 0) FACPPG_REQUIRE(cn == 2 * h->n_half[k - 1], FACPPG_EUNSUPPORTED, "flow %d channel mismatch", k);
-    else FACPPG_REQUIRE(cn == 8, FACPPG_EUNSUPPORTED, "final flow must yield n_group channels");
-    switch (h->n_half[k]) {
-      case 1: launch_flow_end<1>(h->early[k], fqs, fgrid, s, e); break;
-      case 2: launch_flow_end<2>(h->early[k], fqs, fgrid, s, e); break;
-      case 3: launch_flow_end<3>(h->early[k], fqs, fgrid, s, e); break;
-      case 4: launch_flow_end<4>(h->early[k], fqs, fgrid, s, e); break;
-      default: FACPPG_REQUIRE(false, FACPPG_EUNSUPPORTED, "n_half %d", h->n_half[k]);
+    if (fuse_edge) hi ^= 1;
+    else {
+      e.h_out = hbuf[hi];
+      switch (h->n_half[k]) {
+        case 1: launch_flow_end<1>(h->early[k], fqs, fgrid, s, e); break;
+        case 2: launch_flow_end<2>(h->early[k], fqs, fgrid, s, e); break;
+        case 3: launch_flow_end<3>(h->early[k], fqs, fgrid, s, e); break;
+        case 4: launch_flow_end<4>(h->early[k], fqs, fgrid, s, e); break;
+        default: FACPPG_REQUIRE(false, FACPPG_EUNSUPPORTED, "n_half %d", h->n_half[k]);
+      }
     }
     ai ^= 1;
   }
diff --git a/fac-via-ppg_amd/waveglow/glow.py b/fac-via-ppg_amd/waveglow/glow.py
--- a/fac-via-ppg_amd/waveglow/glow.py
+++ b/fac-via-ppg_amd/waveglow/glow.py
@@ -1,4 +1,5 @@
 import os
+import threading
 
 import torch
 
@@ -1028,10 +1029,11 @@
     def _infer_workspace(self, B, T, dev, slot, handle=None):
         nbytes = _lib.load().facppg_wg_workspace_bytes(handle if handle is not None else self._handle(dev), B, T)
         wss = self.__dict__.setdefault("_facppg_ws", {})
-        ws = wss.get(slot)
+        key = (slot, threading.get_ident())
+        ws = wss.get(key)
         if ws is None or ws.numel() < nbytes or ws.device != dev:
             ws = torch.empty(nbytes, dtype=torch.uint8, device=dev)
-            wss[slot] = ws
+            wss[key] = ws
         return ws
 
     def _infer_launch(self, spect, lt, zt, seed, sigma, audio, ws, handle=None):
```

After: 4.382 million, median of 4. No clear change (+0.9%).
